# OSU-NLP-Group/saev

Measured on AMD Instinct MI355X. Metric: activations/sec (train step), d_in=1024 x32 k=32, higher is better.
Workload: dtype f32 (encoder: fp16 MFMA first pass with a rigorous error margin, survivors recomputed exactly in fp32; all else fp32)

## Files before the change

include/saev_amd.h:

```cpp
#ifndef SAEV_AMD_H
#define SAEV_AMD_H

#include <stdint.h>

#ifdef __cplusplus
extern "C" {
#endif

#define SAEV_AMD_ABI_VERSION 12

typedef enum {
    SAEV_OK = 0,
    SAEV_INVALID_ARG = -1,
    SAEV_HIP_ERROR = -2,
    SAEV_UNSUPPORTED = -3,
    SAEV_NOT_BOUND = -4,
    SAEV_RCCL_ERROR = -5,
    SAEV_STALE_PARAMS = -6,
    SAEV_ROW_OVERFLOW = -7
} saev_status;

typedef struct {
    int32_t d_model;
    int32_t d_sae;
// ... 377 lines not shown
#define SAEV_L1_STATE_BETA 3
#define SAEV_L1_STATE_F 4
#define SAEV_L1_STATE_FY 5
#define SAEV_L1_STATE_KKT 6
#define SAEV_L1_STATE_OBJ 7
#define SAEV_L1_STATE_DONE 8
#define SAEV_L1_STATE_NEED_GRAD 9
#define SAEV_L1_STATE_CUR 10
#define SAEV_L1_STATE_PREV 11
#define SAEV_L1_STATE_NEXT 12
#define SAEV_L1_STATE_REJECTS 13
#define SAEV_L1_STATE_RESTARTS 14
typedef struct {
    int32_t struct_size;
    int32_t coef_rows;
    int64_t chunk_rows, n_chunks;
    int64_t col_blocks;
    int64_t total_bytes;
    int64_t off_err, off_state, off_w, off_z, off_g, off_part, off_r, off_loss, off_bp;
} saev_l1_logistic_layout;
int64_t saev_pool_images_range(void);
int saev_pool_images(const int64_t* indptr, const int32_t* indices, const float* data, int64_t nnz, int64_t n_images,
                     int64_t tokens_per_image, int64_t n_latents, int32_t agg, float* out, int32_t* err, void* stream);
int64_t saev_l1_logistic_workspace_bytes(int64_t n, int64_t S, int64_t K);
int saev_l1_logistic_layout_of(int64_t n, int64_t S, int64_t K, saev_l1_logistic_layout* out);
int saev_l1_logistic_init(const float* X, const int32_t* y, int64_t n, int64_t S, int64_t K, double C, double kkt_tol, void* workspace,
                          int64_t workspace_bytes, void* stream);
int saev_l1_logistic_iterate(const float* X, const int32_t* y, int64_t n, int64_t S, int64_t K, double C, double kkt_tol, int32_t n_iters,
                             void* workspace, int64_t workspace_bytes, void* stream);
int saev_l1_logistic_result(const float* X, const int32_t* y, int64_t n, int64_t S, int64_t K, double C, double kkt_tol, double* coef,
                            double* intercept, double* scalars, void* workspace, int64_t workspace_bytes, void* stream);
#define SAEV_COACT_JACCARD 0
#define SAEV_COACT_CONTAINMENT 1
#define SAEV_COACT_ERR_COLUMN 1
#define SAEV_COACT_ERR_VALUE 2
#define SAEV_COACT_ERR_INDPTR 3
int64_t saev_coactivation_chunk_rows(void);
int64_t saev_coactivation_window(void);
int64_t saev_coactivation_slots(void);
int64_t saev_coactivation_workspace_bytes(int64_t N, int64_t Sa, int64_t Sb, int64_t nnz_a, int64_t nnz_b);
int saev_coactivation(const int64_t* a_indptr, const int32_t* a_indices, const float* a_data, int64_t nnz_a, int64_t Sa,
                      const int64_t* b_indptr, const int32_t* b_indices, const float* b_data, int64_t nnz_b, int64_t Sb, int64_t N,
                      float thr_a, float thr_b, int32_t measure, int32_t top_m, int32_t* n_a, int32_t* n_b, int32_t* out_index,
                      int32_t* out_inter, int32_t* err, void* workspace, int64_t workspace_bytes, void* stream);
int saev_params_touched(saev_ctx* ctx);

const int32_t* saev_last_idx(saev_ctx* ctx);
const float* saev_last_val(saev_ctx* ctx);
const float* saev_last_x_hat(saev_ctx* ctx);

int saev_copy_last(saev_ctx* ctx, int32_t n_rows, int32_t* idx_out, float* val_out, float* x_hat_out, void* stream);

int saev_bound_state(saev_ctx* ctx, float* z, int64_t* launches, int64_t* repeats, float* mean_candidates, void* stream);

int saev_enable_kernel_timing(saev_ctx* ctx, int32_t enable);
float saev_last_encoder_ms(saev_ctx* ctx);

#ifdef __cplusplus
}
#endif
#endif
```

saev_amd/_lib.py:

```python

from __future__ import annotations

import ctypes as C
import os
import pathlib

_HERE = pathlib.Path(__file__).resolve().parent
LIB_PATH = pathlib.Path(os.environ.get("SAEV_AMD_LIB", _HERE / "libsaev_amd.so"))

ABI_VERSION = 12


class SaevCfg(C.Structure):
    _fields_ = [
        ("d_model", C.c_int32), ("d_sae", C.c_int32), ("top_k", C.c_int32), ("k_aux", C.c_int32),
        ("alpha", C.c_float), ("dead_threshold_tokens", C.c_int64),
        ("normalize_w_dec", C.c_int32), ("remove_parallel_grads", C.c_int32),
        ("max_batch", C.c_int32), ("encoder_mode", C.c_int32), ("aux_dead_cap", C.c_int32),
        ("shard_world", C.c_int32), ("bound_mode", C.c_int32), ("max_backward_rows", C.c_int32),
        ("activation", C.c_int32),
    ]


class SaevDebugCfg(C.Structure):
# ... 183 lines not shown
    "saev_kmeans_collapsed": (C.c_int, [P, C.c_int64, C.c_int64, C.c_float, P, C.c_int32, P, C.c_int64, P, P, P]),
    "saev_batch_stats_workspace_bytes": (C.c_int64, [C.c_int64, C.c_int64]),
    "saev_batch_stats": (C.c_int, [P, P, P, P, P, P, C.c_int64, C.c_int64, C.c_int64, C.c_int64, C.POINTER(SaevBatchAcc), P, C.c_int64, P]),
    "saev_row_norm_mean": (C.c_int, [P, C.c_int64, C.c_int64, P, P, C.c_int64, P]),
    "saev_latent_topk_workspace_bytes": (C.c_int64, [C.c_int64, C.c_int64]),
    "saev_latent_topk_update": (C.c_int, [P, P, P, C.c_int64, P, P, P, C.c_int64, P, C.c_int64, C.c_int64, C.c_int64,
                                          C.POINTER(SaevLatentTopKState), P, C.c_int64, P]),
    "saev_latent_hist_workspace_bytes": (C.c_int64, [C.c_int64, C.c_int64]),
    "saev_latent_hist_update": (C.c_int, [P, P, P, C.c_int64, P, P, P, C.c_int64, P, C.c_int64, C.c_int64, C.POINTER(SaevLatentHistState), P,
                                          C.c_int64, P]),
    "saev_latent_hist_locate": (C.c_int, [C.POINTER(SaevLatentHistState), C.POINTER(SaevLatentHistTargets), C.c_int64, P]),
    "saev_probe1d_workspace_bytes": (C.c_int64, [C.c_int64] * 4),
    "saev_probe1d_layout_of": (C.c_int, [C.c_int64] * 4 + [C.POINTER(SaevProbe1DLayout)]),
    "saev_probe1d_prepare": (C.c_int, [P, P, P, C.c_int64, C.c_int64, C.c_int64, C.c_int64, P, P, P, P, C.c_int64, P]),
    "saev_probe1d_stats": (C.c_int, [C.c_int64] * 4 + [P, P, P, P, C.c_int64, P]),
    "saev_probe1d_init": (C.c_int, [C.c_int64] * 4 + [C.POINTER(SaevProbe1DCfg), P, C.c_int64, P]),
    "saev_probe1d_update": (C.c_int, [C.c_int64] * 4 + [C.POINTER(SaevProbe1DCfg), P, P, P, P, C.c_int64, P]),
    "saev_probe1d_fit": (C.c_int, [C.c_int64] * 4 + [C.POINTER(SaevProbe1DCfg), P, P, P, P, C.c_int64, P]),
    "saev_probe1d_evaluate": (C.c_int, [C.c_int64] * 4 + [P, P, C.c_double, C.c_int32, P, P, P, P, P, P, C.c_int64, P]),
    "saev_latent_ap_workspace_bytes": (C.c_int64, [C.c_int64] * 4),
    "saev_latent_ap_layout_of": (C.c_int, [C.c_int64] * 4 + [C.POINTER(SaevLatentAPLayout)]),
    "saev_latent_ap": (C.c_int, [P, P, P, C.c_int64, C.c_int64, C.c_int64, C.c_int64, P, P, P, P, P, P, P, P, C.c_int64, P]),
    "saev_probe_ap": (C.c_int, [P, P, P, C.c_int64, C.c_int64, C.c_int64, C.c_int64, P, P, P, P, P, C.c_int32, P, P, P, P, C.c_int32, P, P, C.c_int64, P]),
    "saev_latent_auroc_workspace_bytes": (C.c_int64, [C.c_int64] * 5),
    "saev_latent_auroc": (C.c_int, [P, P, P, C.c_int64, C.c_int64, C.c_int64, C.c_int64, P, P, P, P, C.c_int64, P, P, P, P, P, P, P, P, P, P, C.c_int64, P]),
    "saev_pool_images_range": (C.c_int64, []),
    "saev_pool_images": (C.c_int, [P, P, P, C.c_int64, C.c_int64, C.c_int64, C.c_int64, C.c_int32, P, P, P]),
    "saev_l1_logistic_workspace_bytes": (C.c_int64, [C.c_int64] * 3),
    "saev_l1_logistic_layout_of": (C.c_int, [C.c_int64] * 3 + [C.POINTER(SaevL1LogisticLayout)]),
    "saev_l1_logistic_init": (C.c_int, [P, P, C.c_int64, C.c_int64, C.c_int64, C.c_double, C.c_double, P, C.c_int64, P]),
    "saev_l1_logistic_iterate": (C.c_int, [P, P, C.c_int64, C.c_int64, C.c_int64, C.c_double, C.c_double, C.c_int32, P, C.c_int64, P]),
    "saev_l1_logistic_result": (C.c_int, [P, P, C.c_int64, C.c_int64, C.c_int64, C.c_double, C.c_double, P, P, P, P, C.c_int64, P]),
    "saev_coactivation_chunk_rows": (C.c_int64, []),
    "saev_coactivation_window": (C.c_int64, []),
    "saev_coactivation_slots": (C.c_int64, []),
    "saev_coactivation_workspace_bytes": (C.c_int64, [C.c_int64] * 5),
    "saev_coactivation": (C.c_int, [P, P, P, C.c_int64, C.c_int64, P, P, P, C.c_int64, C.c_int64, C.c_int64, C.c_float, C.c_float, C.c_int32,
                                    C.c_int32, P, P, P, P, P, P, C.c_int64, P]),
    "saev_edit_plan_bytes": (C.c_int64, [C.c_int64, C.c_int64]),
    "saev_edit_plan_build": (C.c_int, [C.POINTER(SaevEdit), C.c_int64, C.c_int64, C.c_int64, P, C.c_int64, P]),
    "saev_intervene_rows": (C.c_int, [P, C.c_int64, C.c_int64, P, C.c_int64, P, P, P, C.c_int64, P, C.c_int64, C.c_int64, P, P, P, P, P]),
    "saev_class_fire_counts": (C.c_int, [P, P, P, C.c_int64, C.c_int64, P, P, C.c_int64, C.c_int64, C.POINTER(C.c_float), C.c_int32, P, P, P, P]),
    "saev_class_fire_f1": (C.c_int, [P, P, P, C.c_int64, C.c_int64, C.c_int32, P, P, P, P]),
    "saev_comm_unique_id": (C.c_int, [P]),
    "saev_comm_init": (C.c_int, [P, P, C.c_int32, C.c_int32]),
    "saev_comm_world": (C.c_int, [P]),
    "saev_comm_destroy": (C.c_int, [P]),
    "saev_train_step_dp": (C.c_int, [P, P, C.c_int32, C.c_float, C.c_float, C.c_int64, P]),
    "saev_last_idx": (P, [P]),
    "saev_last_val": (P, [P]),
    "saev_last_x_hat": (P, [P]),
    "saev_copy_last": (C.c_int, [P, C.c_int32, P, P, P, P]),
    "saev_bound_state": (C.c_int, [P, C.POINTER(C.c_float), C.POINTER(C.c_int64), C.POINTER(C.c_int64), C.POINTER(C.c_float), P]),
    "saev_enable_kernel_timing": (C.c_int, [P, C.c_int32]),
    "saev_last_encoder_ms": (C.c_float, [P]),
}

EXPORTED_SYMBOLS = tuple(_SIGNATURES)

_lib = None


def load() -> C.CDLL:
    global _lib
    if _lib is None:
        if not LIB_PATH.exists():
            raise SaevError(
                f"{LIB_PATH} not found: build the HIP extension first (`make` in the repo root or "
                "`python -c 'import __graft_entry__ as g; g.build()'`). There is no CPU fallback."
            )
        import torch

        lib = C.CDLL(str(LIB_PATH))
        for name, (res, args) in _SIGNATURES.items():
            fn = getattr(lib, name)
            fn.restype = res
            fn.argtypes = args
        got = lib.saev_abi_version()
        if got != ABI_VERSION:
            raise SaevError(f"libsaev_amd.so ABI version {got} != expected {ABI_VERSION}")
        _lib = lib
    return _lib


def check(lib: C.CDLL, ctx, rc: int, what: str) -> None:
    if rc != 0:
        msg = lib.saev_last_error(ctx)
        raise SaevError(f"{what} failed (status {rc}): {msg.decode() if msg else '?'}")
```

saev_amd/csrc/ctx.h:

```cpp
#pragma once
#include <hip/hip_runtime.h>

#include <algorithm>
#include <cmath>
#include <cstdio>
#include <cstdlib>
#include <cstring>
#include <string>
#include <vector>

#include "kernels.h"

constexpr int AUX_KSPLIT_MAX = 16;
constexpr int CAND_CAP = 4096;
constexpr int CAND_STRIDE = CAND_CAP + 256;
constexpr int TIMING_RING = 512;
constexpr int DEAD_LAG = 4;
constexpr int DEAD_RING = 16;
enum { AUX_NONE = 0, AUX_SMALL_DEVICE = 1, AUX_SMALL_HOST = 2, AUX_DENSE = 3 };

struct saev_ctx {
    saev_cfg cfg{};
    saev_debug_cfg dbg{};
    int device = 0;
// ... 64 lines not shown
    bool fused_forward = false;
    bool g_rows_valid = true;
    bool fwd_slices = false;
    bool fwd_step = false;
    float* rs_part = nullptr;
    float* xS_c = nullptr;
    int2 *pv = nullptr, *pv2 = nullptr;
    int32_t *plat = nullptr, *cut_lat = nullptr, *cut_list = nullptr;
    int32_t* lat_unused = nullptr;
    bool fused_step = false;
    bool unused_valid = false;
    int P = 1;
    int32_t cuts[MAX_PREFIXES] = {0};
    float* G = nullptr;
    float* GS = nullptr;
    int P_cap = 0;
    int n_dead_host = 0, k_use_host = 0;
    int64_t tokens_seen = 0;
    bool tracker_dirty = false;
    int nd_cap = 0;
    DeadRecord* rec_host = nullptr;
    DeadRecord* rec_dev = nullptr;
    hipEvent_t dead_ev[DEAD_RING];
    bool dead_ev_created = false;
    int64_t dead_steps = 0;
    int64_t rec_valid_from = 1;
    int aux_route = AUX_NONE;
    int64_t n_readbacks = 0;
    std::vector<void*> aux_allocs;
    int32_t* dead_list = nullptr;
    float *Wenc_dead = nullptr, *Wdec_dead = nullptr, *H_dead = nullptr, *A_dead = nullptr, *dWd = nullptr, *dWe = nullptr,
          *dbe = nullptr, *aux_partials = nullptr, *WencT_dead = nullptr, *aux_small_part = nullptr, *aux_small_part2 = nullptr, *aux_small_partbe = nullptr;
    bool aux_dev_count = false;
    bool aux_small = false;
    int aux_mfma_bound = 0;
    int aux_ndp = AUX_SMALL_MAX;
    int aux_mfma_cap = AUX_SMALL_MAX;
    bool aux_mfma = false;
    bool aux_fused = false;
    bool aux_all = false;
    uint8_t* A_mask = nullptr;
    _Float16 *aux_ws1 = nullptr, *aux_ws2 = nullptr, *aux_xsA = nullptr, *aux_xsg = nullptr, *aux_kA = nullptr, *aux_kD = nullptr, *aux_kX = nullptr;
    bool aux_both = false;
    float* aux_parts = nullptr;
    int aux_kpad = 0;
    float *bias_dead = nullptr, *zero_bias = nullptr, *aux_scales = nullptr;
    float* aux_sync = nullptr;
    int aux_Dp2 = 0;
    float *row_margin = nullptr, *wnorm_scratch = nullptr, *surv_val = nullptr;
    int32_t *surv_idx = nullptr, *surv_cnt = nullptr, *surv_rng = nullptr;
    int rs_lat_range = 0, rs_n_ranges = 0;
    int32_t* tau_max = nullptr;
    float* heur_state = nullptr;
    float *f16r_scales = nullptr, *mu = nullptr, *xnorm = nullptr, *b_shift = nullptr, *dot_part = nullptr, *xabs_part = nullptr,
          *sq_part = nullptr, *wmax_prev = nullptr;
    bool wmax_known = false;
    bool mu_ready = false;
    bool stream_ok = false;
    float *WeS = nullptr;
    float *xn_part = nullptr, *amax_part = nullptr, *cmax_part = nullptr;
    float* b_seen = nullptr;
    int32_t *stale_host = nullptr, *stale_dev = nullptr;
    uint32_t* wchk = nullptr;
    float *mu_keep = nullptr, *xside_keep = nullptr;
    bool fwd_streamed = false;
    bool fwd_moves_mu = false;
    int64_t fwd_mu_serial = -1;
    bool borrow_streamed = false;
    bool follow_stream = false;
    bool wchk_valid = false;
    bool fwd_reused_wimg = false;
    uint32_t stale_salt = 0;
    int scale_par = 0;
    bool prep_valid = false;
    bool wimg_fresh = false;
    int64_t mu_serial = 0, wimg_mu_serial = -1;
    bool wimg_bf16_fresh = false;
    bool stream_step = false;
    bool stats_pending = false, stats_lists = false;
    bool aux_stats_pending = false;
    bool dead_list_ready = false;
    bool train_fused = false;
    const float* gather_pool = nullptr;
    const int64_t* gather_rows = nullptr;
    float *upper_c = nullptr, *mu_c = nullptr, *xnorm_c = nullptr, *xabs_c = nullptr;
    _Float16* xs_c = nullptr;
    saev_ctx* leader = nullptr;
    void* comm = nullptr;
    int comm_rank = 0, comm_world = 0;
    std::vector<saev_ctx*> followers;
    const float* xprep_x = nullptr;
    int xprep_n = 0;
    int64_t xprep_serial = 0;
    int64_t leader_serial_seen = 0;
    _Float16 *xs = nullptr, *ws = nullptr;
    int Dp = 0, S_pad = 0, MB_pad = 0;
    int max_work = 0, max_part = 0;
    float* upper = nullptr;
    saev_step_stats* stats = nullptr;
    double* stats_scratch = nullptr;
    int* tickets = nullptr;
    const float *ov_x = nullptr, *ov_g = nullptr, *ov_val = nullptr;
    const int32_t* ov_idx = nullptr;
    int ov_n = 0;
    float* db_aux = nullptr;
    bool trust_grads = false;
// ... 115 lines not shown
```

saev_amd/csrc/ctx.hip:

```cpp
#include "ctx.h"

int muon_cfg_check(const saev_muon_cfg& m, std::string* why) {
    if (m.ns_steps < 0 || m.ns_steps >= 100) { *why = "ns_steps must be in [0, 100)"; return SAEV_INVALID_ARG; }
    if (m.adjust_lr < 0 || m.adjust_lr > 2) { *why = "adjust_lr must be 0 (original), 1 (match_rms_adamw) or 2 (none)"; return SAEV_INVALID_ARG; }
    if (!(m.momentum >= 0.f) || !(m.weight_decay >= 0.f)) { *why = "momentum and weight_decay must be >= 0"; return SAEV_INVALID_ARG; }
    return SAEV_OK;
}

extern "C" {

int saev_abi_version(void) { return SAEV_AMD_ABI_VERSION; }

int saev_layout(const saev_cfg* cfg, saev_layout_t* out) {
    if (!cfg || !out || cfg->d_model <= 0 || cfg->d_sae <= 0) return SAEV_INVALID_ARG;
    const int64_t S = cfg->d_sae, D = cfg->d_model, N = std::max(1, cfg->shard_world);
    out->chunk_a = (S + 1 + N - 1) / N * D;
    out->chunk_b = ((D * S + S + N - 1) / N + 3) / 4 * 4;
    out->off_W_dec = 0;
    out->off_b_dec = S * D;
    out->off_W_enc = N * out->chunk_a;
    out->off_b_enc = out->off_W_enc + D * S;
    out->n_total = N * out->chunk_a + N * out->chunk_b;
    return SAEV_OK;
}
// ... 92 lines not shown
    A(cand_cnt, MB); A(gmax, (size_t)64 * c->gmax_stride); A(cand_idx, MB * CAND_STRIDE); A(cand_val, MB * CAND_STRIDE);
    A(h_dense, MB * S);
    A(idx, MB * K); A(val, MB * K);
    if (KA > 0) { A(aux_idx, MB * KA); A(aux_val, MB * KA); A(g_aux, MB * D); A(dead_list, S); }
    A(x_hat, MB * D); A(g, MB * D);
    A(rowstats, MB);
    c->bitmap_words = (int)(((MBB + 31) / 32 + 7) / 8 * 8);
    A(bitmap, S * c->bitmap_words);
    A(grp_prefix, S * (c->bitmap_words / 8));
    A(scan_totals, ((S + 1023) / 1024) * 4);
    A(counts, S); A(starts, S + 1); A(pairs, MBB * K); A(dval_pairs, MBB * (size_t)cfg->top_k);
    {
        const long max_pairs = MBB * K;
        c->max_work = (int)(S + (max_pairs + DW_CHUNK - 1) / DW_CHUNK);
        c->max_part = (int)(2 * ((max_pairs + DW_CHUNK - 1) / DW_CHUNK) + 2);
    }
    A(chunk_starts, S + 1); A(part_starts, S); A(work_latent, c->max_work);
    A(dW_encT, S * D); A(partials, (size_t)c->max_part * 2 * D); A(db_partials, c->max_part); A(row_proj, S); A(enc_sq, S);
    {
        const bool rows_only = c->dbg.dw_route == 1;
        c->dws_ok = !rows_only && !btk && D % DWS_SLICE == 0 && (uint64_t)S * D * 4ull < (1ull << 32) && MBB < (1l << 24) &&
                    (uint64_t)MBB * K < (1ull << 31);
    }
    c->fwd_slices = !btk && c->cfg.encoder_mode == SAEV_ENCODER_F16R && c->dbg.fwd_route == 0 && D % RS_SLICE == 0 &&
                    (uint64_t)S * 128ull < (1ull << 32) - 256ull && fused_supported(c->cfg);
    if (c->fwd_slices) {
        A(rs_part, (size_t)(D / RS_SLICE) * MB * REFINE_CAP); A(surv_rng, MB * RS_MAX_RANGES);
        c->rs_lat_range = (int)std::max<long>(RS_LAT_RANGE, ((S + RS_MAX_RANGES - 1) / RS_MAX_RANGES + 255) / 256 * 256);
        c->rs_n_ranges = (int)((S + c->rs_lat_range - 1) / c->rs_lat_range);
    }
    if (c->fwd_slices && !c->dws_ok) A(xS, MBB * D);
    if (c->dws_ok) {
        A(gS, MBB * D); A(xS, MBB * D); A(dvp, (size_t)(D / DWS_SLICE) * MBB * K);
        if (c->dbg.dw_route != 2 && decode_forms_dval((int)D, (int)K)) A(dval_rows, MB * K);
        A(pv, MBB * K); A(pv2, MBB * K); A(plat, MBB * K); A(cut_lat, (MBB * K + DWS_RUN - 1) / DWS_RUN); A(cut_list, 4 * (1 + (MBB * K + DWS_RUN - 1) / DWS_RUN)); A(lat_unused, S);
        if (c->dval_rows != nullptr && c->dbg.fin_route == 0) { A(wn2, S); A(sq_wave, (size_t)2 * dw_slices_waves((int)D, (int)(MBB * K))); }
    }
    A(colsum_partials, ((MBB + 63) / 64) * D);
    A(sumsq_partials, 2 * 1024 + (S + 3) / 4 + 8 + transpose_blocks((int)S, (int)D)); A(sumsq_total, 1);
    if (c->cfg.encoder_mode != SAEV_ENCODER_F32 || KA > 0 || c->relu_train) {
        c->Dp = (int)((D + 31) / 32 * 32);
        c->S_pad = (int)((S + 255) / 256 * 256);
        c->MB_pad = (int)((MB + 255) / 256 * 256);
        A(zero_bias, std::max(S, D)); A(aux_scales, 16); A(aux_sync, absmax_parts_max((int)MB));
    }
    if (c->cfg.encoder_mode != SAEV_ENCODER_F32) {
        A(xs, (size_t)c->MB_pad * 2 * c->Dp);
        A(ws, (size_t)c->S_pad * 2 * c->Dp);
        A(row_margin, MB); A(wnorm_scratch, std::max((S + 3) / 4, 3 * ((S + 255) / 256))); A(f16r_scales, 16); A(mu, D); A(xnorm, 2 * MB); A(b_shift, S);
        A(xabs_part, (MB + 3) / 4);
        if (c->cfg.encoder_mode == SAEV_ENCODER_F16R) { A(dot_part, (size_t)2 * (c->Dp / 32) * c->S_pad); A(sq_part, (size_t)2 * (c->Dp / 32) * c->S_pad); A(wmax_prev, 1); }
        if (c->cfg.encoder_mode == SAEV_ENCODER_F16R) { A(surv_idx, MB * REFINE_CAP); A(surv_val, MB * REFINE_CAP); A(surv_cnt, MB); }
    }
    c->stream_ok = c->fwd_slices && c->cfg.bound_mode == 0 && c->dbg.prep_route == 0 && D % 32 == 0 && c->Dp == (int)D;
    if (c->stream_ok) {
        A(WeS, S * D); A(xn_part, (size_t)(D / 32) * c->MB_pad * 2);
        A(amax_part, (size_t)(c->MB_pad / 256) * (D / 32)); A(cmax_part, (size_t)(c->MB_pad / 256) * (D / 32)); A(b_seen, S);
        A(mu_keep, D); A(xside_keep, 4);
    }
    if (c->stream_ok || c->cfg.encoder_mode == SAEV_ENCODER_BF16) A(wchk, (size_t)2 * ((S + 255) / 256) * ((D + 31) / 32));
    A(toks, S); A(fired, S); A(dead, S); A(flags, 16); A(upper, 1); A(stats, 1);
    A(tau_max, MB); A(heur_state, 8); A(stats_scratch, STATS_SCRATCH_DOUBLES); A(tickets, 8); A(db_aux, D);
    if (btk) { A(btk_ws, btk_workspace_words((int)MB)); A(row_nnz, MB); A(btk_over, 1); A(threshold_own, 1); }
#undef A
    if (rc == SAEV_OK && c->relu_train) rc = relu_train_alloc(c);
    if (rc != SAEV_OK) {
        for (void* p : c->allocs) hipFree(p);
        delete c;
        return rc;
    }
    hipMemset(c->toks, 0, S * sizeof(int64_t));
    hipMemset(c->fired, 0, S * sizeof(int32_t));
    hipMemset(c->dead, 0, S * sizeof(int32_t));
    hipMemset(c->flags, 0, 16 * sizeof(int32_t));
    if (btk) {
        hipMemset(c->threshold_own, 0, sizeof(float));
        hipMemset(c->btk_ws, 0, BTK_ST_WORDS * sizeof(uint32_t));
        hipMemset(c->btk_over, 0, sizeof(int32_t));
        c->threshold = c->threshold_own;
    }
    if (c->stream_ok || c->cfg.encoder_mode == SAEV_ENCODER_BF16) {
        void* hp = nullptr;
        if (hipHostMalloc(&hp, 64, hipHostMallocMapped) == hipSuccess &&
            hipHostGetDevicePointer(reinterpret_cast<void**>(&c->stale_dev), hp, 0) == hipSuccess) {
            c->stale_host = static_cast<int32_t*>(hp);
            c->stale_host[0] = 0; c->stale_host[1] = 0;
        } else {
            if (hp) hipHostFree(hp);
            c->stale_host = nullptr; c->stale_dev = nullptr;
        }
    }
    hipMemset(c->scan_totals, 0, ((S + 1023) / 1024) * 4 * sizeof(int32_t));
    hipMemset(c->stats, 0, sizeof(saev_step_stats));
    hipMemset(c->stats_scratch, 0, STATS_SCRATCH_DOUBLES * sizeof(double));
    hipMemset(c->tickets, 0, 8 * sizeof(int));
    {
        const float init[8] = {2.6f, 0.f, 0.f, 0.f, 0.f, 0.f, 0.f, 0.f};
        hipMemcpy(c->heur_state, init, sizeof(init), hipMemcpyHostToDevice);
    }
    hipMemset(c->rowstats, 0, MB * sizeof(RowStats));
    if (c->xs) hipMemset(c->xs, 0, (size_t)c->MB_pad * 2 * c->Dp * sizeof(_Float16));
    if (c->zero_bias) hipMemset(c->zero_bias, 0, std::max(S, D) * sizeof(float));
    if (c->f16r_scales) hipMemset(c->f16r_scales, 0, 16 * sizeof(float));
    if (KA > 0) {
        const int s4 = (int)((S + 3) / 4 * 4);
        const int want = cfg->aux_dead_cap > 0 ? cfg->aux_dead_cap : std::max(4096, 8 * (int)KA);
        const int cap = std::min((want + 3) / 4 * 4, s4);
        rc = alloc_aux_buffers(c, cap);
        if (rc == SAEV_OK) {
            void* h = nullptr;
            if (hipHostMalloc(&h, DEAD_RING * sizeof(DeadRecord), hipHostMallocMapped) != hipSuccess ||
                hipHostGetDevicePointer(reinterpret_cast<void**>(&c->rec_dev), h, 0) != hipSuccess) {
                rc = SAEV_HIP_ERROR;
            } else {
                c->rec_host = static_cast<DeadRecord*>(h);
                std::memset(h, 0, DEAD_RING * sizeof(DeadRecord));
                for (int i = 0; i < DEAD_RING && rc == SAEV_OK; ++i)
                    if (hipEventCreateWithFlags(&c->dead_ev[i], hipEventDisableTiming) != hipSuccess) rc = SAEV_HIP_ERROR;
                c->dead_ev_created = rc == SAEV_OK;
            }
        }
        if (rc != SAEV_OK) {
            for (void* q : c->allocs) hipFree(q);
            for (void* q : c->aux_allocs) hipFree(q);
            if (c->rec_host) hipHostFree(c->rec_host);
            delete c;
            return rc;
        }
    }
    hipDeviceSynchronize();
    *out = c;
    return SAEV_OK;
}

extern "C" {

static void detach_follower(saev_ctx* c) {
    c->leader = nullptr;
    centre_owner_changed(c);
    c->borrow_streamed = false;
    c->follow_stream = false;
}

static void unlink_from_leader(saev_ctx* c) {
    if (c->leader != nullptr) {
        auto& f = c->leader->followers;
        f.erase(std::remove(f.begin(), f.end(), c), f.end());
        detach_follower(c);
    }
}

// ... 133 lines not shown

int saev_copy_last_row_nnz(saev_ctx* c, int32_t n_rows, int32_t* row_nnz_out, void* stream) {
    if (!c) return SAEV_INVALID_ARG;
    REQUIRE(c, c->btk, SAEV_UNSUPPORTED, "saev_copy_last_row_nnz: the context is not a BatchTopK context");
    REQUIRE(c, c->n_last > 0 && n_rows == c->n_last && row_nnz_out, SAEV_INVALID_ARG,
            "saev_copy_last_row_nnz: n_rows differs from the batch of the last forward (or none has run)");
    HIPCHK(c, hipMemcpyAsync(row_nnz_out, c->row_nnz, (size_t)n_rows * sizeof(int32_t), hipMemcpyDeviceToDevice, (hipStream_t)stream));
    return SAEV_OK;
}

int saev_bind_threshold(saev_ctx* c, float* threshold) {
    if (!c) return SAEV_INVALID_ARG;
    REQUIRE(c, c->btk, SAEV_UNSUPPORTED, "saev_bind_threshold: the context is not a BatchTopK context");
    c->threshold = threshold != nullptr ? threshold : c->threshold_own;
    return SAEV_OK;
}
float* saev_threshold_device(saev_ctx* c) { return c ? c->threshold : nullptr; }
int32_t saev_row_cap(const saev_ctx* c) { return c && c->btk ? c->cfg.top_k : 0; }
int32_t saev_row_overflow_need(const saev_ctx* c) { return c ? c->btk_need : 0; }

int saev_batch_topk_state(saev_ctx* c, float* cut, int64_t* n_above, int64_t* tie_quota, int64_t* n_ties, void* stream) {
    if (!c) return SAEV_INVALID_ARG;
    REQUIRE(c, c->btk, SAEV_UNSUPPORTED, "saev_batch_topk_state: the context is not a BatchTopK context");
    uint32_t h[BTK_ST_WORDS];
    hipStream_t s = (hipStream_t)stream;
    HIPCHK(c, hipMemcpyAsync(h, c->btk_ws, sizeof(h), hipMemcpyDeviceToHost, s));
    HIPCHK(c, hipStreamSynchronize(s));
    if (cut) std::memcpy(cut, &h[BTK_ST_CUT], sizeof(float));
    if (n_above) *n_above = h[BTK_ST_ABOVE];
    if (tie_quota) *tie_quota = h[BTK_ST_RANK];
    if (n_ties) *n_ties = h[BTK_ST_TIES];
    return SAEV_OK;
}

int64_t* saev_toks_since_active(saev_ctx* c) { return c ? c->toks : nullptr; }
int32_t* saev_fired_flags(saev_ctx* c) { return c ? c->fired : nullptr; }
const saev_step_stats* saev_stats_device(saev_ctx* c) { return c ? c->stats : nullptr; }
const int32_t* saev_last_idx(saev_ctx* c) { return c ? c->idx : nullptr; }
const float* saev_last_val(saev_ctx* c) { return c ? c->val : nullptr; }
const float* saev_last_x_hat(saev_ctx* c) { return c ? c->x_hat : nullptr; }

int saev_read_stats(saev_ctx* c, saev_step_stats* out_host, void* stream) {
    if (!c || !out_host) return SAEV_INVALID_ARG;
    hipStream_t s = (hipStream_t)stream;
    HIPCHK(c, hipMemcpyAsync(out_host, c->stats, sizeof(saev_step_stats), hipMemcpyDeviceToHost, s));
    HIPCHK(c, hipStreamSynchronize(s));
    return SAEV_OK;
}

int saev_bound_state(saev_ctx* c, float* z, int64_t* launches, int64_t* repeats, float* mean_candidates, void* stream) {
    if (!c) return SAEV_INVALID_ARG;
    float h[4] = {0.f, 0.f, 0.f, 0.f};
    hipStream_t s = (hipStream_t)stream;
    HIPCHK(c, hipMemcpyAsync(h, c->heur_state, sizeof(h), hipMemcpyDeviceToHost, s));
    HIPCHK(c, hipStreamSynchronize(s));
    if (z) *z = h[0];
    if (repeats) *repeats = (int64_t)h[1];
    if (launches) *launches = (int64_t)h[2];
    if (mean_candidates) *mean_candidates = h[3];
    return SAEV_OK;
}

int saev_enable_kernel_timing(saev_ctx* c, int32_t enable) {
    if (!c) return SAEV_INVALID_ARG;
    if (enable && !c->ev_created) {
        for (int i = 0; i < TIMING_RING; ++i) {
            HIPCHK(c, hipEventCreate(&c->ev_start[i]));
            HIPCHK(c, hipEventCreate(&c->ev_stop[i]));
        }
        c->ev_created = true;
    }
    c->timing = enable != 0;
    c->ev_count = 0;
    return SAEV_OK;
}

float saev_last_encoder_ms(saev_ctx* c) {
    if (!c || !c->ev_created || c->ev_count == 0) return -1.f;
    const long n = std::min<long>(c->ev_count, TIMING_RING);
    double tot = 0;
    for (long i = 0; i < n; ++i) {
        float ms = 0.f;
        if (hipEventElapsedTime(&ms, c->ev_start[i], c->ev_stop[i]) != hipSuccess) return -1.f;
        tot += ms;
    }
    return (float)(tot / n);
}

int saev_params_touched(saev_ctx* c) {
    if (!c) return SAEV_INVALID_ARG;
    params_moved(c);
    return SAEV_OK;
}

void saev_muon_default_cfg(saev_muon_cfg* out) {
    if (!out) return;
    *out = saev_muon_cfg{0.95f, 0.1f, 3.4445f, -4.7750f, 2.0315f, 1e-7f, 1, 5, 0};
}

int64_t saev_muon_workspace_bytes(int64_t rows, int64_t cols) {
    if (rows <= 0 || cols <= 0 || rows > cols || cols > (int64_t)1 << 30) return -1;
    return (int64_t)muon_layout((int)rows, (int)cols).bytes;
}

int saev_muon_newton_schulz(const void* x_in, int64_t rows, int64_t cols, void* x_out, const saev_muon_cfg* cfg, int32_t normalize,
                            void* workspace, int64_t workspace_bytes, void* stream) {
    if (!x_in || !x_out || !workspace) return SAEV_INVALID_ARG;
    const int64_t need = saev_muon_workspace_bytes(rows, cols);
    if (need < 0 || workspace_bytes < need || ((uintptr_t)workspace & 255) != 0) return SAEV_INVALID_ARG;
    saev_muon_cfg m;
    saev_muon_default_cfg(&m);
    if (cfg) m = *cfg;
// ... 59 lines not shown
```

saev_amd/csrc/ctx_auxk.hip:

```cpp
#include "ctx.h"

int alloc_aux_buffers(saev_ctx* c, int cap) {
    const size_t MB = c->cfg.max_batch, D = c->cfg.d_model;
    const size_t capA = std::max(cap, AUX_SMALL_MAX);
    auto grab = [&](size_t bytes) -> void* {
        void* q = nullptr;
        if (hipMalloc(&q, bytes) != hipSuccess) return nullptr;
        c->aux_allocs.push_back(q);
        c->aux_bytes += bytes;
        return q;
    };
    c->Wenc_dead = (float*)grab(D * capA * 4);
    c->Wdec_dead = (float*)grab(capA * D * 4);
    c->H_dead = (float*)grab(MB * capA * 4);
    c->A_dead = (float*)grab(MB * capA * 4);
    c->A_mask = (uint8_t*)grab(MB * capA);
    c->dWd = (float*)grab(capA * D * 4);
    c->dWe = (float*)grab(capA * D * 4);
    c->dbe = (float*)grab(capA * 4);
    c->aux_partials = (float*)grab(((MB + 63) / 64) * capA * 4);
    const size_t mcap = (aux_mfma_supported((int)D) && capA >= (size_t)AUX_MFMA_MAX && c->cfg.max_backward_rows == 0 && c->dbg.aux_wide_route == 0)
                            ? (size_t)AUX_MFMA_MAX : (size_t)AUX_SMALL_MAX;
    c->aux_mfma_cap = (int)mcap;
    c->WencT_dead = (float*)grab(mcap * D * 4);
// ... 208 lines not shown
            HIPCHK(c, launch_colsum(c->g_aux, n, D, c->colsum_partials, c->grads + c->off_b_dec, 1, nd_dev, s));
        }
        return SAEV_OK;
    }
    {
        if (c->aux_both) {
            int ns, Kp;
            ksplit_shape(ndp, D, n, &ns, &Kp);
            HIPCHK(c, launch_split_both(c->g_aux, n, D, 1.0f, c->aux_scales + 4, c->aux_xsg, c->Dp, c->aux_kD, Kp, s));
        } else {
        HIPCHK(c, launch_split_rows(c->g_aux, n, D, c->Dp, c->aux_xsg, 0, s, 1.0f, c->aux_scales + 4));
        HIPCHK(c, launch_split_rows(c->Wdec_dead, ndp, D, c->Dp, c->aux_ws1, 0, s, 256.0f));
        }
        rc = dense_f16x3(c, c->aux_xsg, c->aux_ws1, c->zero_bias, n, c->Dp, ndp, 256.0f, dA, s, c->aux_scales + 4);
    }
    if (rc != SAEV_OK) return rc;
    if (!c->aux_all) HIPCHK(c, launch_mask_apply_absmax(dA, c->A_mask, (long)n * ndp, c->aux_sync, c->aux_scales + 10, s));
    else HIPCHK(c, launch_absmax_pow2(dA, (long)n * ndp, c->aux_sync, c->aux_scales + 10, s));
    {
        rc = ksplit_f16x3(c, c->A_dead, c->aux_scales + 2, ndp, c->g_aux, c->aux_scales + 4, D, n, c->dWd, s,
                          c->aux_both ? c->aux_kA : nullptr, c->aux_both ? c->aux_kD : nullptr);
        if (rc != SAEV_OK) return rc;
        if (c->cfg.encoder_mode == SAEV_ENCODER_F16X3) HIPCHK(c, launch_pow2_scale(c->upper_c, c->aux_scales + 6, s));
        rc = ksplit_f16x3(c, dA, c->aux_scales + 10, ndp, c->x_last, c->aux_scales + 6, D, n, c->dWe, s, nullptr,
                          c->aux_both ? c->aux_kX : nullptr);
        if (rc != SAEV_OK) return rc;
    }
    HIPCHK(c, launch_colsum(dA, n, ndp, c->aux_partials, c->dbe, 0, nullptr, s));
    HIPCHK(c, launch_colsum(c->g_aux, n, D, c->colsum_partials, c->ov_x != nullptr ? c->db_aux : c->grads + c->off_b_dec,
                            c->ov_x != nullptr ? 0 : 1, nullptr, s));
    return SAEV_OK;
}

extern "C" {

int saev_step_dead(saev_ctx* c, int64_t n_rows_global, void* stream) {
    if (!c) return SAEV_INVALID_ARG;
    REQUIRE(c, c->x_last && c->training_last, SAEV_INVALID_ARG, "saev_step_dead: no training forward in flight");
    hipStream_t s = (hipStream_t)stream;
    const int S = c->cfg.d_sae;
    const int64_t step = ++c->dead_steps;
    c->tokens_seen += n_rows_global;
    DeadArgs d{};
    d.toks = c->toks; d.fired = c->fired; d.dead = c->dead; d.S = S;
    d.add_tokens = n_rows_global; d.threshold = c->cfg.dead_threshold_tokens; d.k_aux = c->cfg.k_aux;
    d.n_dead = c->flags + 4; d.k_use = c->flags + 5; d.stats = c->stats; d.scratch = c->flags + 6;
    d.horizon_tokens = (int64_t)DEAD_LAG * n_rows_global;
    d.step = step; d.cum_tokens = c->tokens_seen;
    d.rec = c->rec_dev ? c->rec_dev + step % DEAD_RING : nullptr;
    c->dead_list_ready = false;
    if (c->stats_pending) {
        c->stats_pending = false;
        d.dead_list = c->cfg.k_aux > 0 ? c->dead_list : nullptr;
        HIPCHK(c, launch_stats_dead(c->rowstats, c->n_last, c->cfg.d_model, c->P_last, c->cfg.alpha, c->upper_c, c->flags + 2, c->stats,
                                    c->stats_scratch, c->stats_lists ? c->cand_cnt : nullptr, CAND_CAP, d, s));
        c->dead_list_ready = d.dead_list != nullptr;
    } else {
        HIPCHK(c, launch_dead_update(d, s));
    }
    c->n_dead_host = 0;
    c->k_use_host = 0;
    c->aux_route = AUX_NONE;
    c->aux_small = false;
    c->aux_dev_count = false;
    if (c->cfg.k_aux <= 0) return SAEV_OK;
    HIPCHK(c, hipEventRecord(c->dead_ev[step % DEAD_RING], s));
    if (!c->tracker_dirty && c->tokens_seen < c->cfg.dead_threshold_tokens) return SAEV_OK;
    const bool mfma_route = aux_mfma_supported(c->cfg.d_model) && c->dbg.aux_small_route == 0;
    const int small_default = mfma_route ? std::max((int)AUX_SMALL_MAX, c->aux_mfma_cap) : (int)AUX_SMALL_DEFAULT;
    const int small_cap = c->dbg.aux_small_max < 0 ? 0 : (c->dbg.aux_small_max == 0 ? small_default : std::min(c->dbg.aux_small_max, (int)AUX_SMALL_MAX));
    const int small_max = std::min(small_cap, c->cfg.k_aux);
    const int64_t s0 = step - DEAD_LAG;
    if (s0 >= c->rec_valid_from) {
        HIPCHK(c, hipEventSynchronize(c->dead_ev[s0 % DEAD_RING]));
        const volatile DeadRecord* r = c->rec_host + s0 % DEAD_RING;
        if (r->step == s0 && c->tokens_seen - r->cum_tokens <= r->horizon_tokens) {
            const int bound = r->n_near;
            if (bound == 0) return SAEV_OK;
            if (bound <= small_max && c->cfg.d_model <= 2048) {
                c->aux_route = AUX_SMALL_DEVICE;
                return auxk_small_forward(c, s, bound);
            }
            if ((bound + 3) / 4 * 4 <= c->nd_cap) {
                c->aux_route = AUX_DENSE;
                c->aux_dev_count = true;
                c->n_dead_host = bound;
                c->k_use_host = std::min(c->cfg.k_aux, bound);
                return auxk_forward(c, s);
            }
        }
    }
    int32_t host[2] = {0, 0};
    HIPCHK(c, hipMemcpyAsync(host, c->flags + 4, 2 * sizeof(int32_t), hipMemcpyDeviceToHost, s));
    HIPCHK(c, hipStreamSynchronize(s));
    c->n_readbacks++;
    c->n_dead_host = host[0];
    c->k_use_host = host[1];
    if (c->n_dead_host <= 0) return SAEV_OK;
    if ((c->n_dead_host + 3) / 4 * 4 > c->nd_cap && !(c->n_dead_host <= small_max && c->cfg.d_model <= 2048)) {
        const int s4 = (S + 3) / 4 * 4;
        const int cap = std::min(s4, std::max(2 * c->nd_cap, (2 * c->n_dead_host + 1023) / 1024 * 1024));
        for (void* q : c->aux_allocs) hipFree(q);
        c->aux_allocs.clear();
        c->aux_bytes = 0;
        c->nd_cap = 0;
        int rcg = alloc_aux_buffers(c, cap);
        if (rcg != SAEV_OK) {
            c->err = "AuxK: " + std::to_string(c->n_dead_host) + " dead latents exceed saev_cfg.aux_dead_cap and the buffers could not be grown to " +
// ... 16 lines not shown
```

saev_amd/csrc/ctx_forward.hip:

```cpp
#include "ctx.h"

extern "C" {


int saev_normalize_w_dec(saev_ctx* c, void* stream) {
    if (!c) return SAEV_INVALID_ARG;
    REQUIRE(c, c->params, SAEV_NOT_BOUND, "parameters not bound");
    if (!c->cfg.normalize_w_dec) return SAEV_OK;
    HIPCHK(c, launch_normalize_rows(c->params + c->off_W_dec, c->cfg.d_sae, c->cfg.d_model, (hipStream_t)stream));
    return SAEV_OK;
}

static bool bind_x_sources(saev_ctx* c, const float* x, int n, bool allow_borrow) {
    saev_ctx* l = c->leader;
    const bool borrow = allow_borrow && l != nullptr && l->xprep_x == x && l->xprep_n == n && l->xprep_serial != c->leader_serial_seen;
    saev_ctx* src = borrow ? l : c;
    c->upper_c = src->upper; c->mu_c = src->mu; c->xnorm_c = src->xnorm; c->xabs_c = src->xabs_part; c->xs_c = src->xs;
    c->borrow_streamed = borrow && l->fwd_streamed && l->mu_keep != nullptr;
    if (c->borrow_streamed) c->mu_c = l->mu_keep;
    c->fwd_step = c->fwd_slices && (src == c || src->fwd_slices);
    c->xS_c = c->fwd_step ? src->xS : nullptr;
    if (borrow) c->leader_serial_seen = l->xprep_serial;
    return borrow;
}
// ... 16 lines not shown
        if (!c->wmax_known) {
            { int rcw = wait_wenc(c, s); if (rcw != SAEV_OK) return rcw; }
            HIPCHK(c, launch_transpose(c->params + c->off_W_enc, c->dW_encT, D, S, s));
            HIPCHK(c, launch_wnorm_max(c->dW_encT, S, D, c->wnorm_scratch, c->wmax_prev, s));
            c->wmax_known = true;
        }
        if (!x_borrowed) {
            if (!c->mu_ready) { HIPCHK(c, launch_colsum(x, n, D, c->colsum_partials, c->mu, 0, nullptr, s, 0, 1.0f / (float)n)); c->mu_serial++; }
            HIPCHK(c, launch_center_stats(x, c->mu, n, D, c->xnorm, c->xabs_part, s, xmax_dev));
        }
        c->mu_ready = false;
        if (c->borrow_streamed)
            HIPCHK(c, launch_follower_scales(c->leader->xside_keep, c->wmax_prev, scl(c), pre_flag != nullptr ? pre_flag : c->flags, 0, s));
        else
        HIPCHK(c, launch_f16r_scales(c->xabs_c, (n + 3) / 4, c->wmax_prev, scl(c), s));
        float* const wt_out = (c->fwd_step && c->stream_ok) ? c->WeS : c->dW_encT;
        if (!x_borrowed && c->wenc_ready == nullptr) {
            HIPCHK(c, launch_split_f16r(x, n, D, c->Dp, c->xs, scl(c), c->mu, c->params + c->off_W_enc, S, c->S_pad, c->ws,
                                        reinterpret_cast<double*>(c->dot_part), c->sq_part, wt_out, s, c->fwd_step ? c->xS : nullptr,
                                        c->fwd_step ? 1 : 0));
        } else {
            if (!x_borrowed) HIPCHK(c, launch_split_rows(x, n, D, c->Dp, c->xs, 2, s, 1.0f, scl(c), c->mu, c->fwd_step ? c->xS : nullptr));
            { int rcw = wait_wenc(c, s); if (rcw != SAEV_OK) return rcw; }
            HIPCHK(c, launch_split_wT(c->params + c->off_W_enc, D, S, c->S_pad, c->Dp, 1.0f, c->ws, 2, s, scl(c) + 1,
                                      c->mu_c, reinterpret_cast<double*>(c->dot_part), c->sq_part, wt_out, c->fwd_step ? 1 : 0));
        }
        c->wimg_fresh = c->stream_ok && c->fwd_step && !x_borrowed && c->leader == nullptr;
        c->wimg_mu_serial = c->mu_serial;
        HIPCHK(c, launch_bias_finish(reinterpret_cast<const double*>(c->dot_part), c->sq_part, c->Dp, S, c->S_pad,
                                     scl(c) + 1, c->params + c->off_b_enc, c->b_shift, c->wnorm_scratch, s, c->b_seen));
        if (!defer_margins)
            HIPCHK(c, launch_row_margins(c->xnorm_c, n, D, c->wnorm_scratch, (S + 255) / 256, scl(c), pre_flag,
                                         c->wmax_prev, c->row_margin, s));
        return SAEV_OK;
    }
    if (!x_borrowed) HIPCHK(c, launch_split_rows(x, n, D, c->Dp, c->xs, bf ? 1 : 0, s));
    { int rcw = wait_wenc(c, s); if (rcw != SAEV_OK) return rcw; }
    c->fwd_reused_wimg = bf && c->wimg_bf16_fresh;
    if (!(bf && c->wimg_bf16_fresh))
        HIPCHK(c, launch_split_wT(c->params + c->off_W_enc, D, S, c->S_pad, c->Dp, bf ? 1.0f : 256.0f, c->ws, bf ? 1 : 0, s));
    if (bf && c->dbg.prep_route == 0 && c->Dp == D && D % 32 == 0) c->wimg_bf16_fresh = true;
    return SAEV_OK;
}

static int prepare_dense_scaled(saev_ctx* c, const float* x, int n, const float* absmax_dev, float* pair, hipStream_t s) {
    HIPCHK(c, launch_pow2_scale(absmax_dev, pair, s));
    HIPCHK(c, launch_split_rows(x, n, c->cfg.d_model, c->Dp, c->xs, 0, s, 1.0f, pair));
    { int rcw = wait_wenc(c, s); if (rcw != SAEV_OK) return rcw; }
    HIPCHK(c, launch_split_wT(c->params + c->off_W_enc, c->cfg.d_model, c->cfg.d_sae, c->S_pad, c->Dp, 256.0f, c->ws, 0, s));
    return SAEV_OK;
}

static int run_encoder(saev_ctx* c, const float* x, int n, int epi, float* h_out, const int32_t* flag, int when,
                       hipStream_t s, bool predicted = false, const float* x_scale = nullptr) {
    const bool f16r = c->cfg.encoder_mode == SAEV_ENCODER_F16R;
    if (c->cfg.encoder_mode != SAEV_ENCODER_F32 && !(f16r && epi == EPI_DENSE)) {
        const bool bf = c->cfg.encoder_mode == SAEV_ENCODER_BF16;
        EncodeF16Args a{};
        a.xs = c->xs_c; a.ws = c->ws;
        a.b_enc = f16r ? c->b_shift : c->params + c->off_b_enc;
        a.n_rows = n; a.Dp = c->Dp; a.S = c->cfg.d_sae; a.w_scale = (bf || f16r) ? 1.0f : 256.0f;
        a.scale_dev = f16r ? scl(c) : x_scale;
        a.arith = bf ? 1 : (f16r ? 2 : 0);
        a.row_margin = f16r ? c->row_margin : nullptr;
        a.s_splits = encoder_splits(n, a.S, encode_f16x3_tile_rows(), encode_f16x3_tile_latents(), 256);
        a.h_out = h_out;
        a.ngroups = f16_ngroups(c); a.top_k = c->cfg.top_k;
        a.gmax = c->gmax; a.gmax_stride = c->gmax_stride; a.cand_cnt = c->cand_cnt; a.cand_val = c->cand_val; a.cand_idx = c->cand_idx;
        a.cand_cap = CAND_CAP; a.cand_stride = CAND_STRIDE;
        a.enable_flag = flag; a.enable_when = when;
        if (predicted) { a.heur_z = c->heur_state; a.tau_max = c->tau_max; }
        a.refresh_first = 8;
        a.refresh_every = a.ngroups > 32 ? 1 : 2;
        HIPCHK(c, launch_encode_f16x3(a, epi, s));
        return SAEV_OK;
    }
    EncodeArgs a{};
    a.x = x;
    a.W_enc = c->params + c->off_W_enc;
    a.b_enc = c->params + c->off_b_enc;
    a.n_rows = n;
    a.D = c->cfg.d_model;
    a.S = c->cfg.d_sae;
    a.s_splits = encoder_splits(n, a.S, encode_gemm_tile_rows(), encode_gemm_tile_latents(), 512);
    a.h_out = h_out;
    a.ngroups = c->cfg.top_k <= 32 ? 32 : 64;
    a.gmax = c->gmax;
    a.gmax_stride = c->gmax_stride;
    a.cand_cnt = c->cand_cnt;
    a.cand_val = c->cand_val;
    a.cand_idx = c->cand_idx;
    a.cand_cap = CAND_CAP; a.cand_stride = CAND_STRIDE;
    a.enable_flag = flag;
    a.enable_when = when;
    HIPCHK(c, launch_encode_gemm(a, epi, s));
    return SAEV_OK;
}

int saev_encode_dense(saev_ctx* c, const float* x, int32_t n, float* h_out, void* stream) {
    if (!c) return SAEV_INVALID_ARG;
    REQUIRE(c, c->params, SAEV_NOT_BOUND, "parameters not bound");
    REQUIRE(c, x && h_out && n > 0, SAEV_INVALID_ARG, "saev_encode_dense: bad arguments");
    REQUIRE(c, n <= c->cfg.max_batch || c->cfg.encoder_mode == SAEV_ENCODER_F32, SAEV_INVALID_ARG,
            "saev_encode_dense: n_rows > max_batch");
    bind_x_sources(c, x, n, false);
    c->xprep_x = nullptr;
    if (c->relu_train && c->cfg.encoder_mode == SAEV_ENCODER_F16X3) {
        hipStream_t s = (hipStream_t)stream;
        HIPCHK(c, hipMemsetAsync(c->rt_scales + 8, 0, sizeof(float), s));
        HIPCHK(c, launch_absmax(x, (long)n * c->cfg.d_model, c->rt_scales + 8, s));
        int rc = prepare_dense_scaled(c, x, n, c->rt_scales + 8, c->rt_scales + 10, s);
        if (rc != SAEV_OK) return rc;
        return run_encoder(c, x, n, EPI_DENSE, h_out, nullptr, 0, s, false, c->rt_scales + 10);
    }
    if (c->cfg.encoder_mode != SAEV_ENCODER_F16R) {
        int rc = prepare_encoder(c, x, n, nullptr, (hipStream_t)stream);
        if (rc != SAEV_OK) return rc;
    }
    return run_encoder(c, x, n, EPI_DENSE, h_out, nullptr, 0, (hipStream_t)stream);
}

int saev_topk_dense(saev_ctx* c, const float* h, int32_t n, int32_t k, const int32_t* mask, int32_t* idx_out,
                    float* val_out, void* stream) {
    if (!c) return SAEV_INVALID_ARG;
    REQUIRE(c, h && idx_out && val_out && n > 0 && k > 0, SAEV_INVALID_ARG, "saev_topk_dense: bad arguments");
    REQUIRE(c, k <= c->cfg.d_sae, SAEV_INVALID_ARG, "saev_topk_dense: k > d_sae");
    SelectDenseArgs a{};
    a.h = h; a.n_rows = n; a.S = c->cfg.d_sae; a.k = k; a.mask = mask;
    a.idx_out = idx_out; a.val_out = val_out; a.out_stride = k;
    HIPCHK(c, launch_select_dense(a, (hipStream_t)stream));
    return SAEV_OK;
}

static int encode_topk_impl(saev_ctx* c, const float* x, int n, int32_t* idx_out, float* val_out,
                            const int32_t* pre_flag, hipStream_t s, const float* xmax_dev = nullptr, bool x_borrowed = false) {
    const int K = c->cfg.top_k;
    int32_t* need_dense = c->flags + 1;
    const bool f16r_mode = c->cfg.encoder_mode == SAEV_ENCODER_F16R;
    const bool predict_mode = fused_supported(c->cfg) && c->cfg.bound_mode != 0 && c->cfg.encoder_mode != SAEV_ENCODER_F32 &&
                              f16_ngroups(c) == 32;
    const bool one_launch_pre = fused_supported(c->cfg) && !predict_mode;
    if (c->follow_stream) {
        HIPCHK(c, launch_follower_scales(c->leader->xside_keep, c->wmax_prev, scl(c), const_cast<int32_t*>(pre_flag), 1, s));
    } else if (!c->stream_step) {
        int rc0 = prepare_encoder(c, x, n, const_cast<int32_t*>(pre_flag), s, xmax_dev, x_borrowed, one_launch_pre);
        if (rc0 != SAEV_OK) return rc0;
        rc0 = wait_wenc(c, s);
        if (rc0 != SAEV_OK) return rc0;
    }
    if (fused_supported(c->cfg)) {
        const int ng = c->cfg.encoder_mode == SAEV_ENCODER_F32 ? (c->cfg.top_k <= 32 ? 32 : 64) : f16_ngroups(c);
        const bool f16r = c->cfg.encoder_mode == SAEV_ENCODER_F16R;
        auto select_stage = [&](const int32_t* flag, int when, int32_t* bad, const int32_t* tau_max, int32_t* ovf = nullptr,
                                const int32_t* first_flag = nullptr) -> int {
            SelectCandArgs sc{};
            sc.cand_cnt = c->cand_cnt; sc.cand_val = c->cand_val; sc.cand_idx = c->cand_idx;
            sc.cand_cap = CAND_CAP; sc.cand_stride = CAND_STRIDE; sc.n_rows = n; sc.k = K;
            sc.idx_out = idx_out; sc.val_out = val_out; sc.out_stride = K;
            sc.enable_flag = first_flag ? first_flag : flag; sc.enable_when = when;
            sc.tau_max = tau_max; sc.invalid = bad; sc.ovf = ovf;
            if (f16r) {
                sc.row_margin = c->row_margin; sc.x = x; sc.W_encT = c->dW_encT; sc.b_enc = c->params + c->off_b_enc;
                sc.D = c->cfg.d_model; sc.refine_overflow = bad;
                sc.surv_idx = c->surv_idx; sc.surv_val = c->surv_val; sc.surv_cnt = c->surv_cnt;
                if (c->fwd_step) { sc.surv_rng = c->surv_rng; sc.lat_range = c->rs_lat_range; sc.n_ranges = c->rs_n_ranges; }
                HIPCHK(c, launch_select_cand(sc, s));
                sc.enable_flag = flag; sc.ovf = nullptr;
                if (c->fwd_step) {
                    RefineSlicesArgs rs{};
                    rs.surv_idx = c->surv_idx; rs.surv_cnt = c->surv_cnt; rs.surv_val = c->surv_val; rs.surv_rng = c->surv_rng;
                    rs.xS = c->xS_c; rs.WeS = c->stream_ok ? c->WeS : c->dW_encT; rs.b_enc = sc.b_enc; rs.part = c->rs_part;
                    rs.n_rows = n; rs.S = c->cfg.d_sae; rs.D = c->cfg.d_model;
                    rs.lat_range = c->rs_lat_range; rs.n_ranges = c->rs_n_ranges;
                    rs.enable_flag = flag; rs.enable_when = when;
                    HIPCHK(c, launch_refine_slices(rs, s));
                    sc.sum_part = c->rs_part; sc.sum_bias = sc.b_enc; sc.sum_n = c->cfg.d_model / RS_SLICE; sc.sum_plane = (size_t)n * REFINE_CAP;
                } else {
                    HIPCHK(c, launch_refine_exact(sc, s));
                }
                sc.row_margin = nullptr; sc.tau_max = nullptr;
                sc.cand_cnt = c->surv_cnt; sc.cand_val = c->surv_val; sc.cand_idx = c->surv_idx; sc.cand_cap = REFINE_CAP; sc.cand_stride = REFINE_CAP;
            }
            HIPCHK(c, launch_select_cand(sc, s));
            return SAEV_OK;
        };
        const bool predict = c->cfg.bound_mode != 0 && ng == 32 && c->cfg.encoder_mode != SAEV_ENCODER_F32;
        int32_t *bad1 = c->flags + 9, *run2 = c->flags + 10, *gate = c->flags + 11;
        if (predict) {
            HIPCHK(c, launch_heur_gate(c->heur_state, pre_flag, gate, s));
            HIPCHK(c, launch_encoder_init(c->cand_cnt, n, c->gmax, 0, s, c->tau_max));
            timing_begin(c, s);
            int rc = run_encoder(c, x, n, EPI_TOPK, nullptr, gate, 0, s, true);
            if (rc != SAEV_OK) return rc;
            timing_end(c, s);
            HIPCHK(c, launch_overflow_check(c->cand_cnt, n, CAND_CAP, gate, bad1, c->flags + 2, c->flags + 3, s, need_dense,
                                            nullptr, c->heur_state + 3, nullptr, pre_flag));
            rc = select_stage(bad1, 0, bad1, c->tau_max);
            if (rc != SAEV_OK) return rc;
            HIPCHK(c, launch_heur_update(c->heur_state, bad1, c->heur_state + 3, K, gate, s));
            HIPCHK(c, launch_encoder_init(c->cand_cnt, n, c->gmax, ng * c->gmax_stride, s, nullptr, bad1, 1));
            rc = run_encoder(c, x, n, EPI_TOPK, nullptr, bad1, 1, s);
            if (rc != SAEV_OK) return rc;
            HIPCHK(c, launch_overflow_check(c->cand_cnt, n, CAND_CAP, pre_flag, need_dense, c->flags + 2, c->flags + 3, s, need_dense,
                                            run2, nullptr, bad1));
            rc = select_stage(run2, 1, need_dense, nullptr);
            if (rc != SAEV_OK) return rc;
        } else {
            const int S_ = c->cfg.d_sae;
            if (c->stream_step) {
                const int D_ = c->cfg.d_model;
                XprepArgs xp{};
                xp.x = c->gather_pool != nullptr ? c->gather_pool : x; xp.rows = c->gather_rows; xp.x_out = c->gather_pool != nullptr ? const_cast<float*>(x) : nullptr;
                xp.n = n; xp.D = D_; xp.nks = D_ / 32; xp.n_pad = c->MB_pad; xp.scales = scl(c); xp.mu = c->mu; xp.xs = c->xs; xp.xS = c->xS;
                xp.xn_part = c->xn_part; xp.col_part = c->colsum_partials; xp.amax_part = c->amax_part; xp.cmax_part = c->cmax_part;
                xp.W_enc = c->params + c->off_W_enc; xp.WeS = c->WeS; xp.b_enc = c->params + c->off_b_enc; xp.b_seen = c->b_seen;
                xp.S = S_; xp.salt = ++c->stale_salt; xp.stale = c->flags + 12;
                if (!c->followers.empty()) { xp.mu_keep = c->mu_keep; xp.xside_keep = c->xside_keep; }
                HIPCHK(c, launch_xprep(xp, s));
                PreEncode2Args pe{};
                pe.cand_cnt = c->cand_cnt; pe.n_rows = n; pe.gmax = c->gmax; pe.n_gmax = ng * c->gmax_stride;
                pe.xn_part = c->xn_part; pe.nks = D_ / 32; pe.n_pad = c->MB_pad; pe.D = D_;
                pe.wg_part = c->wnorm_scratch; pe.n_part = (S_ + 255) / 256; pe.scales = scl(c); pe.scales_next = scl_next(c);
                pe.pre_flag = const_cast<int32_t*>(pre_flag); pe.wmax_prev = c->wmax_prev; pe.margin = c->row_margin; pe.xnorm = c->xnorm;
                pe.flags1 = c->flags + 1; pe.col_part = c->colsum_partials; pe.n_rowblk = (n + 255) / 256; pe.mu = c->mu;
                pe.inv_n = 1.0f / (float)n; pe.update_mu = c->train_fused ? 1 : 0;
                pe.amax_part = c->amax_part; pe.cmax_part = c->cmax_part; pe.n_img = ((n + 255) / 256) * (D_ / 32);
                pe.upper = c->upper; pe.stats = c->stats; pe.stale = c->flags + 12; pe.stale_host = c->stale_dev;
                pe.xside_keep = c->followers.empty() ? nullptr : c->xside_keep;
                HIPCHK(c, launch_pre_encode2(pe, s));
                if (c->train_fused) c->mu_serial++;
            } else
            HIPCHK(c, launch_pre_encode(c->cand_cnt, n, c->gmax, ng * c->gmax_stride, f16r_mode ? c->xnorm_c : nullptr, c->cfg.d_model,
                                        c->wnorm_scratch, (S_ + 255) / 256, f16r_mode ? scl(c) : nullptr, const_cast<int32_t*>(pre_flag),
                                        c->wmax_prev, c->row_margin, c->flags + 1, s));
            timing_begin(c, s);
            int rc = run_encoder(c, x, n, EPI_TOPK, nullptr, pre_flag, 0, s);
            if (rc != SAEV_OK) return rc;
            timing_end(c, s);
            rc = select_stage(need_dense, 0, need_dense, nullptr, c->flags + 1, pre_flag);
            if (rc != SAEV_OK) return rc;
        }
    } else {
        HIPCHK(c, launch_init_i32(need_dense, 1, 1, s));
        HIPCHK(c, hipMemsetAsync(c->flags + 2, 0, 2 * sizeof(int32_t), s));
        timing_begin(c, s);
        timing_end(c, s);
    }
    int rc = run_encoder(c, x, n, EPI_DENSE, c->h_dense, need_dense, 1, s);
    if (rc != SAEV_OK) return rc;
    SelectDenseArgs sd{};
    sd.h = c->h_dense; sd.n_rows = n; sd.S = c->cfg.d_sae; sd.k = K;
    sd.idx_out = idx_out; sd.val_out = val_out; sd.out_stride = K;
    sd.enable_flag = need_dense; sd.enable_when = 1;
    if (fused_supported(c->cfg)) sd.walk_grid = 4 * 256;
    HIPCHK(c, launch_select_dense(sd, s));
    return SAEV_OK;
}

int saev_encode_topk(saev_ctx* c, const float* x, int32_t n, int32_t* idx_out, float* val_out, void* stream) {
    if (!c) return SAEV_INVALID_ARG;
    REQUIRE(c, c->cfg.activation == SAEV_ACT_TOPK, SAEV_UNSUPPORTED,
            "saev_encode_topk: a TopK context only (ReLU: saev_encode_relu, BatchTopK: saev_encode_batch_topk)");
    REQUIRE(c, c->params, SAEV_NOT_BOUND, "parameters not bound");
    REQUIRE(c, x && idx_out && val_out && n > 0 && n <= c->cfg.max_batch, SAEV_INVALID_ARG,
            "saev_encode_topk: bad arguments (n_rows must be in 1..max_batch)");
    hipStream_t s = (hipStream_t)stream;
    HIPCHK(c, hipMemsetAsync(c->flags, 0, sizeof(int32_t), s));
    bind_x_sources(c, x, n, false);
    c->xprep_x = nullptr;
    c->stream_step = false;
    c->follow_stream = false;
    return encode_topk_impl(c, x, n, idx_out, val_out, c->flags, s);
}

int saev_scatter_dense(saev_ctx* c, const int32_t* idx, const float* val, int32_t n, int32_t k, float* f_out,
                       void* stream) {
    if (!c) return SAEV_INVALID_ARG;
    REQUIRE(c, idx && val && f_out && n > 0 && k > 0, SAEV_INVALID_ARG, "saev_scatter_dense: bad arguments");
    HIPCHK(c, launch_scatter_dense(idx, val, n, k, k, c->cfg.d_sae, f_out, (hipStream_t)stream));
    return SAEV_OK;
}

int saev_decode_sparse(saev_ctx* c, const int32_t* idx, const float* val, int32_t n, int32_t k,
                       const int64_t* prefixes_host, int32_t n_prefixes, float* x_hats_out, void* stream) {
    if (!c) return SAEV_INVALID_ARG;
    REQUIRE(c, c->params, SAEV_NOT_BOUND, "parameters not bound");
    REQUIRE(c, idx && val && x_hats_out && n > 0 && k > 0, SAEV_INVALID_ARG, "saev_decode_sparse: bad arguments");
    const int S = c->cfg.d_sae, D = c->cfg.d_model;
    int64_t single = S;
    if (!prefixes_host) { prefixes_host = &single; n_prefixes = 1; }
    REQUIRE(c, n_prefixes >= 1 && prefixes_host[n_prefixes - 1] == S && prefixes_host[0] >= 1, SAEV_INVALID_ARG,
            "prefixes must end at d_sae and start at >= 1");
    for (int p = 1; p < n_prefixes; ++p)
        REQUIRE(c, prefixes_host[p] > prefixes_host[p - 1], SAEV_INVALID_ARG, "prefixes must be strictly increasing");
    REQUIRE(c, n <= c->cfg.max_batch || n_prefixes == 1, SAEV_INVALID_ARG, "n_rows > max_batch");
    hipStream_t s = (hipStream_t)stream;
    for (int p = 0; p < n_prefixes; ++p) {
        DecodeArgs a{};
        a.x = nullptr;
        a.idx = idx; a.val = val; a.code_stride = k; a.k = k;
        a.W_dec = c->params + c->off_W_dec; a.b_dec = c->params + c->off_b_dec;
        a.n_rows = n; a.D = D; a.S = S; a.idx_limit = (int)prefixes_host[p];
        a.x_hat = (n_prefixes == 1) ? x_hats_out : c->g;
        HIPCHK(c, launch_decode(a, s));
        if (n_prefixes > 1)
            HIPCHK(c, hipMemcpy2DAsync(x_hats_out + (size_t)p * D, (size_t)n_prefixes * D * sizeof(float), c->g,
                                       (size_t)D * sizeof(float), (size_t)D * sizeof(float), n,
                                       hipMemcpyDeviceToDevice, s));
    }
    return SAEV_OK;
}


namespace {
int btk_codes(saev_ctx* c, const float* h, int n, int training, int32_t* row_nnz_out, int32_t* idx_out, float* val_out,
              int32_t* overflow_out, hipStream_t s) {
    BtkArgs a{};
    a.h = h; a.n_rows = n; a.S = c->cfg.d_sae; a.top_k = c->btk_k; a.row_cap = c->cfg.top_k; a.training = training ? 1 : 0;
    a.update_threshold = a.training; a.momentum = c->btk_momentum; a.threshold = c->threshold;
    a.idx_out = idx_out; a.val_out = val_out; a.row_nnz_out = row_nnz_out; a.overflow = overflow_out;
    a.ws = c->btk_ws; a.max_rows = c->cfg.max_batch; a.list_cap = c->btk_list_cap;
    HIPCHK(c, launch_batch_topk(a, s));
    return SAEV_OK;
}
// ... 111 lines not shown
    if (!c) return SAEV_INVALID_ARG;
    REQUIRE(c, pool && rows && out && n > 0, SAEV_INVALID_ARG, "saev_gather_rows: bad arguments");
    HIPCHK(c, launch_gather_rows(pool, rows, n, c->cfg.d_model, out, (hipStream_t)stream));
    return SAEV_OK;
}


int saev_step_forward(saev_ctx* c, const float* x, int32_t n, int64_t n_rows_global, int32_t training,
                      void* stream) {
    if (!c) return SAEV_INVALID_ARG;
    if (c->relu_train) return relu_train_forward(c, x, n, n_rows_global, training, (hipStream_t)stream);
    REQUIRE(c, c->cfg.activation != SAEV_ACT_RELU, SAEV_UNSUPPORTED, "saev_step_forward: a ReLU context runs the forward entries only");
    REQUIRE(c, c->params, SAEV_NOT_BOUND, "parameters not bound");
    REQUIRE(c, x && n > 0 && n <= c->cfg.max_batch, SAEV_INVALID_ARG,
            "saev_step_forward: n_rows must be in 1..max_batch");
    REQUIRE(c, ((uintptr_t)x % 16) == 0, SAEV_INVALID_ARG, "x must be 16-byte aligned");
    REQUIRE(c, n_rows_global >= n, SAEV_INVALID_ARG, "n_rows_global < n_rows");
    hipStream_t s = (hipStream_t)stream;
    const int S = c->cfg.d_sae, D = c->cfg.d_model, K = c->cfg.top_k;
    c->x_last = x;
    c->n_last = n;
    c->training_last = training;
    c->ov_x = nullptr; c->ov_n = 0;
    c->unused_valid = false;
    hipEvent_t wdec_ev = c->wdec_ready;
    c->wdec_ready = nullptr;
    const bool btk = c->btk;
    const bool borrowed = bind_x_sources(c, x, n, !btk);
    if (c->stale_host != nullptr && reinterpret_cast<volatile int32_t*>(c->stale_host)[1] != 0) {
        const int n_tiles = reinterpret_cast<volatile int32_t*>(c->stale_host)[1];
        reinterpret_cast<volatile int32_t*>(c->stale_host)[1] = 0;
        c->wimg_fresh = false; c->wimg_bf16_fresh = false; c->wn2_fresh = false;
        c->err = "W_enc was written outside the library without saev_params_touched (" + std::to_string(n_tiles) +
                 " 32 x 256 tiles changed between two optimizer steps): a recent step encoded with operand images of the OLD values. "
                 "Announce such writes (saev_params_touched / SaeEngine.params_touched) or make them through torch in-place "
                 "operations on the parameter tensors; the context prepares from scratch from here on";
        return SAEV_STALE_PARAMS;
    }
    if (c->stale_host != nullptr && *reinterpret_cast<volatile int32_t*>(c->stale_host) != 0) {
        *reinterpret_cast<volatile int32_t*>(c->stale_host) = 0;
        c->wimg_fresh = false;
        c->wn2_fresh = false;
    }
    c->stream_step = c->stream_ok && c->prep_valid && c->wimg_fresh && c->wimg_mu_serial == c->mu_serial && c->leader == nullptr &&
                     c->wenc_ready == nullptr && c->fwd_step && (c->followers.empty() || c->dbg.group_route == 0);
    if (!borrowed) {
        c->fwd_streamed = c->stream_step;
        c->fwd_moves_mu = c->stream_step && c->train_fused;
        c->fwd_mu_serial = c->mu_serial;
    }
    c->follow_stream = borrowed && c->borrow_streamed && c->stream_ok && c->wimg_fresh && c->wimg_mu_serial == c->leader->fwd_mu_serial &&
                       c->wenc_ready == nullptr && c->fwd_step && c->cfg.encoder_mode == SAEV_ENCODER_F16R;
    c->fwd_reused_wimg = c->stream_step || c->follow_stream;
    if (c->gather_pool != nullptr && !c->stream_step)
        HIPCHK(c, launch_gather_rows(c->gather_pool, c->gather_rows, n, D, const_cast<float*>(x), s));
    if (c->stream_step) {
        c->xprep_x = nullptr;
    } else if (!borrowed && !btk && c->cfg.encoder_mode == SAEV_ENCODER_F16R) {
        c->xprep_x = nullptr;
        HIPCHK(c, launch_colsum_absmax(x, n, D, c->colsum_partials, c->mu, c->xabs_part, c->upper, s, 1.0f / (float)n, c->stats, c->flags));
        c->mu_ready = true;
        c->mu_serial++;
    } else {
        HIPCHK(c, launch_step_zero(c->stats, c->upper, c->flags, s));
        if (!borrowed) {
            c->xprep_x = nullptr;
            HIPCHK(c, launch_absmax(x, (long)n * D, c->upper, s));
        }
    }
    (void)n_rows_global;
    int rc;
    if (btk) {
        rc = encode_dense_h(c, x, n, s);
        if (rc == SAEV_OK) rc = btk_codes(c, c->h_dense, n, training, c->row_nnz, c->idx, c->val, c->btk_over, s);
        if (rc == SAEV_OK) {
            int32_t need = 0;
            HIPCHK(c, hipMemcpyAsync(&need, c->btk_over, sizeof(int32_t), hipMemcpyDeviceToHost, s));
            HIPCHK(c, hipStreamSynchronize(s));
            if (need > 0) {
                c->btk_need = need;
                c->x_last = nullptr; c->n_last = 0; c->training_last = 0;
                c->err = "BatchTopK: a row holds " + std::to_string(need) + " codes, the context's row_cap is " + std::to_string(K) +
                         " (create a context with a larger saev_batch_topk_cfg.row_cap and repeat the forward; the threshold has not moved)";
                return SAEV_ROW_OVERFLOW;
            }
        }
    } else {
        rc = encode_topk_impl(c, x, n, c->idx, c->val, c->flags, s, c->upper_c, borrowed);
    }
    if (rc != SAEV_OK) return rc;
    if (!borrowed) { c->xprep_x = x; c->xprep_n = n; c->xprep_serial++; }
    if (!borrowed && c->stream_ok && !c->stream_step && c->fwd_step) {
        HIPCHK(c, hipMemcpyAsync(scl(c) + 4, c->upper, sizeof(float), hipMemcpyDeviceToDevice, s));
        c->prep_valid = true;
    }
    if (wdec_ev != nullptr) HIPCHK(c, hipStreamWaitEvent(s, wdec_ev, 0));
    if (training) {
        c->wn2_fresh = false;
        if (c->cfg.normalize_w_dec) {
            HIPCHK(c, launch_normalize_rows(c->params + c->off_W_dec, S, D, s, c->wn2));
            c->wn2_fresh = c->wn2 != nullptr;
        }
    }

    DecodeArgs a{};
    a.x = x; a.idx = c->idx; a.val = c->val; a.code_stride = K; a.k = K;
    a.W_dec = c->params + c->off_W_dec; a.b_dec = c->params + c->off_b_dec;
    a.n_rows = n; a.D = D; a.S = S; a.idx_limit = S;
    a.upper = c->upper_c;
    a.gscale = 2.0f / ((float)n * (float)D * (float)c->P);
    a.training = training ? 1 : 0;
    a.g = c->g; a.x_hat = c->x_hat; a.fired = c->fired; a.rowstats = c->rowstats;
    c->dws_rows = 0;
    c->dval_fwd = false;
    if (training && c->dws_ok && (c->P == 1 || c->GS != nullptr)) { a.gS = c->P == 1 ? c->gS : c->GS; a.xS = c->fwd_step ? nullptr : c->xS; c->dws_rows = n; }
    if (c->dws_rows == n && c->dval_rows != nullptr && (c->P == 1 || decode_matry_forms_dval(D, K))) { a.dval_out = c->dval_rows; c->dval_fwd = true; }
    c->g_rows_valid = !(c->train_fused && training && c->P == 1 && c->dws_rows == n);
    if (!c->g_rows_valid) a.g = nullptr;
    c->bitmap_prefill_words = 0;
    if (training && c->dbg.csc_route == 0 && c->bitmap != nullptr && c->bitmap_clean && !c->last_backward_gathered) {
        const int words = ((n + 31) / 32 + 7) / 8 * 8;
        if (words <= c->bitmap_clean_words) {
            a.csc_bitmap = c->bitmap; a.csc_words = words;
            c->bitmap_prefill_words = words; c->bitmap_prefill_rows = n;
            c->bitmap_clean = false;
        }
    }
    if (c->P > 1) {
        MatryArgs m{};
        m.P = c->P;
        for (int p = 0; p < c->P; ++p) m.cuts[p] = c->cuts[p];
        m.G = c->G;
        m.g_rows_all = c->fused_forward ? 0 : 1;
        HIPCHK(c, launch_decode_matry(a, m, s));
    } else {
        HIPCHK(c, launch_decode(a, s));
    }
    c->P_last = c->P;
    for (int p = 0; p < c->P; ++p) c->cuts_last[p] = c->cuts[p];
    const bool lists = !btk && fused_supported(c->cfg) && !(c->cfg.bound_mode != 0 && c->cfg.encoder_mode != SAEV_ENCODER_F32 && f16_ngroups(c) == 32);
    c->stats_pending = false;
    if (c->train_fused && training) {
        c->stats_pending = true;
        c->stats_lists = lists;
        return SAEV_OK;
    }
    HIPCHK(c, launch_stats_reduce(c->rowstats, n, D, c->P, c->cfg.alpha, 0, c->upper_c, c->flags + 2, c->stats, s, nullptr, c->stats_scratch,
                                  lists ? c->cand_cnt : nullptr, CAND_CAP));
    return SAEV_OK;
}

}
```

saev_amd/csrc/gemm_encode_f16x3.hip:

```cpp
#include "common.h"
#include "kernels.h"

namespace {

typedef _Float16 half8 __attribute__((ext_vector_type(8)));

constexpr int HTS = 256;
constexpr int HTB = 256;
constexpr int HTHREADS = 512;
constexpr int NSLOTS = 4;

struct __attribute__((aligned(16))) KSlot {
    _Float16 a[HTS][32];
    _Float16 b[HTB][32];
};
struct __attribute__((aligned(16))) HSmem {
    union {
        KSlot slot[NSLOTS];
        struct {
            KSlot keep[2];
            int32_t slots32[2][32][HTB];
        } e32;
    };
    int32_t tau_key[HTB];
// ... 549 lines not shown
    const int l15 = lane & 15;
    const int kg = lane >> 4;

    const int Dp = a.Dp, S = a.S, B = a.n_rows;
    const int n_stiles = (S + HTS - 1) / HTS;
    int bb, sp;
    {
        const int id = blockIdx.x;
        const int nbb = (B + HTB - 1) / HTB;
        const int full = (nbb / 8) * 8 * a.s_splits;
        if (id < full) {
            const int xcd = id & 7, j = id >> 3;
            sp = j % a.s_splits;
            bb = (j / a.s_splits) * 8 + xcd;
        } else {
            const int r = id - full;
            bb = (nbb / 8) * 8 + r / a.s_splits;
            sp = r % a.s_splits;
        }
    }
    const int st_begin = (int)((long)n_stiles * sp / a.s_splits);
    const int st_end = (int)((long)n_stiles * (sp + 1) / a.s_splits);
    const int b0 = bb * HTB;

    const int nks = Dp / 32;
    const int rot = (bb & 7) % nks;
    auto kmap = [&](int t) { const int k = t + rot; return k >= nks ? k - nks : k; };

    const size_t img = (size_t)256 * 32;
    const int blk_imgs = a.blk_imgs > 0 ? a.blk_imgs : nks;
    const _Float16* x_imgs = a.xs + (size_t)bb * blk_imgs * img;
    const uint32_t lane_off = (uint32_t)lane * 16u;
    const uint32_t lds_w = (uint32_t)(size_t)(__attribute__((address_space(3))) char*)&sm.slot[0].a[wid * 32][0];
    auto stage_kstep = [&](int slot, int s0, int ks) {
        const char* wsrc = reinterpret_cast<const char*>(a.ws + ((size_t)(s0 / HTS) * blk_imgs + ks) * img) + wid * 2048;
        const char* xsrc = reinterpret_cast<const char*>(x_imgs + (size_t)ks * img) + wid * 2048;
        const uint32_t lds_a = lds_w + (uint32_t)slot * (uint32_t)sizeof(KSlot);
        asm volatile(
            "s_mov_b32 m0, %0\n\ts_nop 0\n\t"
            "global_load_lds_dwordx4 %2, %3" SAEV_ENC_W_POLICY "\n\tglobal_load_lds_dwordx4 %2, %3 offset:1024" SAEV_ENC_W_POLICY "\n\t"
            "s_mov_b32 m0, %1\n\ts_nop 0\n\t"
            "global_load_lds_dwordx4 %2, %4" SAEV_ENC_X_POLICY "\n\tglobal_load_lds_dwordx4 %2, %4 offset:1024" SAEV_ENC_X_POLICY
            ::"s"(lds_a), "s"(lds_a + (uint32_t)sizeof(_Float16) * HTS * 32), "v"(lane_off), "s"(wsrc), "s"(xsrc)
            : "memory");
    };

    const int arow0 = ws * 128 + l15;
    const int brow0 = wb * 64 + l15;
    const int coff = 8 * (kg ^ ((4 - (l15 >> 2)) & 3));

    if (st_begin < st_end) {
        stage_kstep(0, st_begin * HTS, kmap(0));
        if (nks > 1) stage_kstep(1, st_begin * HTS, kmap(1));
    }

    for (int st = st_begin; st < st_end; ++st) {
        const int s0 = st * HTS;
        f32x4 acc[8][4];
#pragma unroll
        for (int i = 0; i < 8; ++i)
#pragma unroll
            for (int j = 0; j < 4; ++j) acc[i][j] = f32x4{0.f, 0.f, 0.f, 0.f};

        float* const bias_t = sm.bias[st & 1];
        if (tid < HTS) bias_t[tid] = (s0 + tid < S) ? a.b_enc[s0 + tid] : NEG_INF;
        asm volatile("s_waitcnt vmcnt(0)" ::: "memory");
        __syncthreads();
        if (nks > 2) stage_kstep(2, s0, kmap(2));
        const char* const w_tile = reinterpret_cast<const char*>(a.ws + (size_t)(s0 / HTS) * blk_imgs * img) + wid * 2048;
        const char* const x_blk = reinterpret_cast<const char*>(x_imgs) + wid * 2048;
        const uint32_t run_bytes = (uint32_t)nks * (uint32_t)(img * sizeof(_Float16));
        uint32_t koff = (uint32_t)kmap(nks > 3 ? 3 : 0) * (uint32_t)(img * sizeof(_Float16));
        auto stage_next = [&](int slot) {
            const uint32_t lds_a = lds_w + (uint32_t)slot * (uint32_t)sizeof(KSlot);
            asm volatile(
                "s_mov_b32 m0, %0\n\ts_nop 0\n\t"
                "global_load_lds_dwordx4 %2, %3" SAEV_ENC_W_POLICY "\n\tglobal_load_lds_dwordx4 %2, %3 offset:1024" SAEV_ENC_W_POLICY "\n\t"
                "s_mov_b32 m0, %1\n\ts_nop 0\n\t"
                "global_load_lds_dwordx4 %2, %4" SAEV_ENC_X_POLICY "\n\tglobal_load_lds_dwordx4 %2, %4 offset:1024" SAEV_ENC_X_POLICY
                ::"s"(lds_a), "s"(lds_a + (uint32_t)sizeof(_Float16) * HTS * 32), "v"(lane_off), "s"(w_tile + koff), "s"(x_blk + koff)
                : "memory");
            koff += (uint32_t)(img * sizeof(_Float16));
            koff = koff == run_bytes ? 0u : koff;
        };

        auto kstep = [&](int t, auto WAIT_, auto SLOT_) {
            constexpr int WAIT = decltype(WAIT_)::value;
            constexpr int SLOT = decltype(SLOT_)::value;
            if constexpr (WAIT == 8) stage_next(SLOT >= 0 ? (SLOT + 3) & 3 : (t + 3) & 3);
            const KSlot& cs = sm.slot[SLOT >= 0 ? SLOT : t & 3];
            half8 fa[3], fb[4];
            auto load_a = [&](int set, int sb) { fa[set] = *reinterpret_cast<const half8*>(&cs.a[arow0 + 16 * sb][coff]); };
#pragma unroll
            for (int jb = 0; jb < 4; ++jb) fb[jb] = *reinterpret_cast<const half8*>(&cs.b[brow0 + 16 * jb][coff]);
            load_a(0, 0);
            load_a(1, 1);
            static_for<8>([&](auto G) {
                constexpr int sb = decltype(G)::value;
                constexpr int as = sb % 3;
                constexpr int j0 = (sb & 1) ? 3 : 0, j1 = (sb & 1) ? 2 : 1, j2 = (sb & 1) ? 1 : 2, j3 = (sb & 1) ? 0 : 3;
                acc[sb][j0] = mfma16<AR>(fa[as], fb[j0], acc[sb][j0]);
                __builtin_amdgcn_sched_barrier(0);
                if constexpr (sb + 2 < 8) load_a((sb + 2) % 3, sb + 2);
                __builtin_amdgcn_sched_barrier(0);
                acc[sb][j1] = mfma16<AR>(fa[as], fb[j1], acc[sb][j1]);
                acc[sb][j2] = mfma16<AR>(fa[as], fb[j2], acc[sb][j2]);
// ... 71 lines not shown
                }
                __syncthreads();
                {
                    int32_t old[32];
#pragma unroll
                    for (int i = 0; i < 32; ++i) {
                        old[i] = __hip_atomic_load(GPTR(i), __ATOMIC_RELAXED, __HIP_MEMORY_SCOPE_AGENT);
                    }
                    short2v mp[16];
                    uint32_t improved = 0;
#pragma unroll
                    for (int j = 0; j < 16; ++j) {
                        const int gp = 16 * tpart + j;
                        const short2v w0 = __builtin_bit_cast(short2v, sm.e32.slots32[0][gp][trow]);
                        const short2v w1 = __builtin_bit_cast(short2v, sm.e32.slots32[1][gp][trow]);
                        const short2v wm = __builtin_elementwise_max(w0, w1);
                        const short2v o = __builtin_bit_cast(
                            short2v, __builtin_amdgcn_perm((uint32_t)old[2 * j + 1], (uint32_t)old[2 * j], 0x07060302u));
                        mp[j] = __builtin_elementwise_max(wm, o);
                        improved |= __builtin_bit_cast(uint32_t, mp[j]) ^ __builtin_bit_cast(uint32_t, o);
                    }
                    if (share && improved != 0) {
#pragma unroll
                        for (int j = 0; j < 16; ++j) {
                            const int32_t a0 = (int32_t)mp[j][0], a1 = (int32_t)mp[j][1];
                            if (a0 > (old[2 * j] >> 16)) atomicMax(GPTR(2 * j), a0 << 16);
                            if (a1 > (old[2 * j + 1] >> 16)) atomicMax(GPTR(2 * j + 1), a1 << 16);
                        }
                    }
                    short2v mn = mp[0], mx = mp[0];
#pragma unroll
                    for (int j = 1; j < 16; ++j) { mn = __builtin_elementwise_min(mn, mp[j]); mx = __builtin_elementwise_max(mx, mp[j]); }
                    int32_t lo = min((int32_t)mn[0], (int32_t)mn[1]), hi = max((int32_t)mx[0], (int32_t)mx[1]);
                    lo = min(lo, __shfl_xor(lo, 32, 64));
                    hi = max(hi, __shfl_xor(hi, 32, 64));
                    const int K = a.top_k;
#pragma unroll 1
                    for (int it = 0; it < 4 && lo < hi && K < 64; ++it) {
                        const int32_t mid = lo + ((hi - lo + 1) >> 1);
                        const short2v midp = {(short)mid, (short)mid};
                        uint32_t lt = 0;
#pragma unroll
                        for (int j = 0; j < 16; ++j)
                            lt += (__builtin_bit_cast(uint32_t, __builtin_elementwise_sub_sat(mp[j], midp)) >> 15) & 0x00010001u;
                        int c = 32 - (int)((lt & 0xffffu) + (lt >> 16));
                        c += __shfl_xor(c, 32, 64);
                        if (c >= K) lo = mid; else hi = mid - 1;
                    }
                    if (tpart == 0) sm.tau_key[trow] = (int32_t)((uint32_t)lo << 16);
                }
#undef GPTR
                __syncthreads();
            }
        } else if (refresh) {
#pragma unroll
            for (int jb = 0; jb < 4; ++jb) {
                const int bl_ = wb * 64 + jb * 16 + l15;
#pragma unroll
                for (int p = 0; p < 2; ++p)
#pragma unroll
                    for (int e = 0; e < 4; ++e) {
                        const float m = fmaxf(fmaxf(acc[p][jb][e], acc[p + 2][jb][e]), fmaxf(acc[p + 4][jb][e], acc[p + 6][jb][e]));
                        sm.e32.slots32[ws][p * 16 + 4 * kg + e][bl_] = f2key(m);
                    }
            }
            __syncthreads();
            if (tid < HTB) sm.tau_key[tid] = INT32_MAX;
            __syncthreads();
            {
                const int row = tid % HTB;
                const int part = __builtin_amdgcn_readfirstlane(tid / HTB);
                constexpr int GPT = 16;
                const int b = b0 + row;
                const bool share = b < B;
                const uint32_t boff = (uint32_t)b * 4u;
                int32_t m = INT32_MAX;
                int32_t old[GPT];
#pragma unroll
                for (int i = 0; i < GPT; ++i) {
                    old[i] = INT32_MIN;
                    if (share)
                        old[i] = __hip_atomic_load(
                            reinterpret_cast<int32_t*>(reinterpret_cast<char*>(a.gmax + (size_t)(part * GPT + i) * a.gmax_stride) + boff),
                            __ATOMIC_RELAXED, __HIP_MEMORY_SCOPE_AGENT);
                }
#pragma unroll
                for (int i = 0; i < GPT; ++i) {
                    const int g = part * GPT + i;
                    const int32_t v = max(sm.e32.slots32[0][g][row], sm.e32.slots32[1][g][row]);
                    if (share && v > old[i])
                        atomicMax(reinterpret_cast<int32_t*>(reinterpret_cast<char*>(a.gmax + (size_t)g * a.gmax_stride) + boff), v);
                    m = min(m, max(v, old[i]));
                }
                atomicMin(&sm.tau_key[row], m);
            }
            __syncthreads();
        }
        if (NG == 32 && st == st_begin && a.top_k <= HTS / 4) {
            if (tid < HTB) { sm.ref[0][tid] = INT32_MIN; sm.ref[1][tid] = 0; sm.ref[2][tid] = 0; sm.ref[3][tid] = 0; }
            __syncthreads();
#pragma unroll
            for (int jb = 0; jb < 4; ++jb) {
                float m = NEG_INF;
#pragma unroll
                for (int sb = 0; sb < 8; ++sb)
#pragma unroll
                    for (int e = 0; e < 4; ++e) m = fmaxf(m, acc[sb][jb][e]);
                atomicMax(&sm.ref[0][wb * 64 + jb * 16 + l15], f2key(m));
            }
            __syncthreads();
            float tg[4][3];
#pragma unroll
            for (int jb = 0; jb < 4; ++jb) {
                const int row = wb * 64 + jb * 16 + l15;
                const float t0 = key2f(sm.tau_key[row]), M = key2f(sm.ref[0][row]);
                const bool usable = t0 > -3.0e38f && M > t0;
                const float span = usable ? (M - t0) : 0.f;
                tg[jb][0] = t0 + 0.25f * span; tg[jb][1] = t0 + 0.40f * span; tg[jb][2] = t0 + 0.55f * span;
                int c0 = 0, c1 = 0, c2 = 0;
#pragma unroll
                for (int sb = 0; sb < 8; ++sb)
#pragma unroll
                    for (int e = 0; e < 4; ++e) {
                        const float v = acc[sb][jb][e];
                        c0 += (v >= tg[jb][0]) ? 1 : 0; c1 += (v >= tg[jb][1]) ? 1 : 0; c2 += (v >= tg[jb][2]) ? 1 : 0;
                    }
                if (usable) { atomicAdd(&sm.ref[1][row], c0); atomicAdd(&sm.ref[2][row], c1); atomicAdd(&sm.ref[3][row], c2); }
            }
            __syncthreads();
            if (ws == 0 && kg == 0) {
#pragma unroll
                for (int jb = 0; jb < 4; ++jb) {
                    const int row = wb * 64 + jb * 16 + l15;
                    float best = key2f(sm.tau_key[row]);
                    if (sm.ref[1][row] >= a.top_k) best = fmaxf(best, tg[jb][0]);
                    if (sm.ref[2][row] >= a.top_k) best = fmaxf(best, tg[jb][1]);
                    if (sm.ref[3][row] >= a.top_k) best = fmaxf(best, tg[jb][2]);
                    sm.tau_key[row] = f2key(best);
                }
            }
            __syncthreads();
        }
        typedef unsigned u32x2 __attribute__((ext_vector_type(2)));
        uint32_t hit[4];
        int pos[4], rowtot[4], base[4];
#pragma unroll
        for (int jb = 0; jb < 4; ++jb) {
            const int b = b0 + wb * 64 + jb * 16 + l15;
            float tau = fmaxf(key2f(sm.tau_key[wb * 64 + jb * 16 + l15]), -3.0e38f);
            if (a.row_margin != nullptr) tau -= (b < B) ? a.row_margin[b] : 0.f;
            uint32_t m = 0;
#pragma unroll
            for (int sb = 0; sb < 8; ++sb)
#pragma unroll
                for (int e = 0; e < 4; ++e)
                    asm("v_cmp_ge_f32 vcc, %1, %2\n\tv_addc_co_u32 %0, vcc, %0, %0, vcc" : "+v"(m) : "v"(acc[sb][jb][e]), "v"(tau) : "vcc");
            m = (b < B) ? m : 0u;
            const int n = __builtin_popcount(m);
            const u32x2 r = __builtin_amdgcn_permlane16_swap((unsigned)n, (unsigned)n, false, false);
            const unsigned pair = r[0] + r[1];
            const u32x2 q = __builtin_amdgcn_permlane32_swap(pair, pair, false, false);
            rowtot[jb] = (int)(q[0] + q[1]);
            pos[jb] = (int)(((kg & 1) ? r[0] : 0u) + ((kg & 2) ? q[0] : 0u));
            base[jb] = 0;
            if (kg == 0 && rowtot[jb] > 0) base[jb] = atomicAdd(&a.cand_cnt[b], rowtot[jb]);
            hit[jb] = m;
        }
        asm volatile("s_waitcnt vmcnt(0)" ::: "memory");
        asm volatile("" : "+v"(base[0]), "+v"(base[1]), "+v"(base[2]), "+v"(base[3]));
        float* const park = reinterpret_cast<float*>(&sm.e32.slots32[0][0][0]) + wid * 2048 + lane * 4;
        const int lat0 = s0 + ws * 128 + 4 * kg;
#pragma unroll
        for (int jb = 0; jb < 4; ++jb) {
            const u32x2 h = __builtin_amdgcn_permlane32_swap((unsigned)base[jb], (unsigned)base[jb], false, false);
            const u32x2 f = __builtin_amdgcn_permlane16_swap(h[0], h[0], false, false);
            const int row_base = (int)f[0];
            uint32_t mm = (row_base + rowtot[jb] <= a.cand_cap) ? hit[jb] : 0u;
            if (__ballot(mm != 0u) == 0ull) continue;
            if (mm != 0u) {
#pragma unroll
                for (int sb = 0; sb < 8; ++sb) *reinterpret_cast<f32x4*>(park + 256 * sb) = acc[sb][jb];
            }
            uint32_t off = ((uint32_t)(b0 + wb * 64 + jb * 16 + l15) * (uint32_t)a.cand_stride + (uint32_t)(row_base + pos[jb])) * 4u;
            int i0 = 0;
            while (mm != 0u) {
                const int p = __builtin_clz(mm);
                const int i = i0 + p;
                mm = (mm << p) << 1;
                i0 = i + 1;
                const int c = i >> 2, e = i & 3;
                const float v = park[256 * c + e];
                *reinterpret_cast<float*>(reinterpret_cast<char*>(a.cand_val) + off) = v;
                *reinterpret_cast<int32_t*>(reinterpret_cast<char*>(a.cand_idx) + off) = lat0 + 16 * c + e;
                off += 4u;
            }
        }
        if (!prefetched && st + 1 < st_end) {
            __syncthreads();
            stage_kstep(0, s0 + HTS, kmap(0));
            if (nks > 1) stage_kstep(1, s0 + HTS, kmap(1));
        }
    }
}

}

hipError_t launch_encode_f16x3(const EncodeF16Args& a, int epi, hipStream_t stream) {
    const int n_bblocks = (a.n_rows + HTB - 1) / HTB;
    dim3 grid(n_bblocks * a.s_splits, (epi == EPI_DENSE && a.n_batches > 1) ? a.n_batches : 1), block(HTHREADS);
    const size_t smem = sizeof(HSmem);
    static bool attr_set = false;
    if (!attr_set) {
        const void* fns[12] = {reinterpret_cast<const void*>(&encode_m16_kernel<1>),
                              reinterpret_cast<const void*>(&encode_m16_kernel<2>),
                              reinterpret_cast<const void*>(&encode_m16_kernel<1, 64>),
                              reinterpret_cast<const void*>(&encode_m16_kernel<2, 64>),
                              reinterpret_cast<const void*>(&encode_f16x3_kernel<EPI_TOPK, 32, 0, true>),
                              reinterpret_cast<const void*>(&encode_f16x3_kernel<EPI_TOPK, 32, 1, true>),
                              reinterpret_cast<const void*>(&encode_f16x3_kernel<EPI_TOPK, 32, 2, true>),
                              reinterpret_cast<const void*>(&encode_f16x3_kernel<EPI_DENSE, 32, 0>),
                              reinterpret_cast<const void*>(&encode_f16x3_kernel<EPI_TOPK, 32, 0>),
                              reinterpret_cast<const void*>(&encode_f16x3_kernel<EPI_TOPK, 64, 0>),
                              reinterpret_cast<const void*>(&encode_f16x3_kernel<EPI_DENSE, 32, 1>),
                              reinterpret_cast<const void*>(&encode_f16x3_kernel<EPI_DENSE, 32, 2>)};
        for (const void* f : fns) {
            hipError_t e = hipFuncSetAttribute(f, hipFuncAttributeMaxDynamicSharedMemorySize, (int)smem);
            if (e != hipSuccess) return e;
        }
        attr_set = true;
    }
#define LAUNCH_ENC(...) hipLaunchKernelGGL((encode_f16x3_kernel<__VA_ARGS__>), grid, block, smem, stream, a)
#define LAUNCH_M16(...) hipLaunchKernelGGL((encode_m16_kernel<__VA_ARGS__>), grid, block, smem, stream, a)
    if (epi == EPI_DENSE) {
        if (a.arith == 1) LAUNCH_ENC(EPI_DENSE, 32, 1);
        else if (a.arith == 2) LAUNCH_ENC(EPI_DENSE, 32, 2);
        else LAUNCH_ENC(EPI_DENSE, 32, 0);
    } else if (a.ngroups <= 32 && a.heur_z != nullptr) {
        if (a.arith == 1) LAUNCH_ENC(EPI_TOPK, 32, 1, true);
        else if (a.arith == 2) LAUNCH_ENC(EPI_TOPK, 32, 2, true);
        else LAUNCH_ENC(EPI_TOPK, 32, 0, true);
    } else if (a.ngroups <= 32) {
        if (a.arith == 1) LAUNCH_M16(1);
        else if (a.arith == 2) LAUNCH_M16(2);
        else LAUNCH_ENC(EPI_TOPK, 32, 0);
    } else {
        if (a.arith == 1) LAUNCH_M16(1, 64);
        else if (a.arith == 2) LAUNCH_M16(2, 64);
        else LAUNCH_ENC(EPI_TOPK, 64, 0);
    }
#undef LAUNCH_M16
#undef LAUNCH_ENC
    return hipGetLastError();
}

int encode_f16x3_tile_rows() { return HTB; }
int encode_f16x3_tile_latents() { return HTS; }
```

saev_amd/csrc/kernels.h:

```cpp
#pragma once
#include <hip/hip_runtime.h>
#include <stdint.h>

#include <string>

#include "../../include/saev_amd.h"

enum { EPI_DENSE = 0, EPI_TOPK = 1 };

struct EncodeArgs {
    const float* x;
    const float* W_enc;
    const float* b_enc;
    int n_rows, D, S;
    int s_splits;
    float* h_out;
    int ngroups;
    int32_t* gmax;
    int gmax_stride;
    int32_t* cand_cnt;
    float* cand_val;
    int32_t* cand_idx;
    int cand_cap;
    int cand_stride;
    const int32_t* enable_flag;
    int enable_when;
};

size_t encode_gemm_smem_bytes();
hipError_t launch_encode_gemm(const EncodeArgs& a, int epi, hipStream_t stream);
int encode_gemm_tile_rows();
int encode_gemm_tile_latents();

struct SelectDenseArgs {
    const float* h;
    int n_rows, S;
    int k;
    const int32_t* k_dev;
    const int32_t* mask;
    int32_t* idx_out;
    float* val_out;
    int out_stride;
    const int32_t* enable_flag;
    int enable_when;
    int walk_grid;
};
hipError_t launch_select_dense(const SelectDenseArgs& a, hipStream_t stream);

struct SelectCandArgs {
    const int32_t* cand_cnt;
    const float* cand_val;
    const int32_t* cand_idx;
    int cand_cap, cand_stride, n_rows, k;
    int32_t* idx_out;
    float* val_out;
    int out_stride;
    const int32_t* enable_flag;
    int enable_when;
    const float* row_margin;
    const float* x;
    const float* W_encT;
    const float* b_enc;
    int D;
    int32_t* surv_idx;
    float* surv_val;
    int32_t* surv_cnt;
    int32_t* refine_overflow;
    const int32_t* tau_max;
    int32_t* invalid;
    int32_t* ovf;
    int32_t* surv_rng;
    int lat_range, n_ranges;
    const float* sum_part;
    const float* sum_bias;
    int sum_n;
    size_t sum_plane;
};
hipError_t launch_refine_exact(const SelectCandArgs& a, hipStream_t stream);
constexpr int REFINE_CAP = 512;
constexpr int RS_SLICE = 32;
constexpr int RS_ROWS_MAX = 8;
constexpr int RS_LAT_RANGE = 32768;
constexpr int RS_MAX_RANGES = 8;
struct RefineSlicesArgs {
    const int32_t* surv_idx; const int32_t* surv_cnt; float* surv_val; const int32_t* surv_rng;
    const float* xS; const float* WeS; const float* b_enc; float* part;
    int n_rows, S, D, lat_range, n_ranges;
    const int32_t* enable_flag; int enable_when;
};
hipError_t launch_refine_slices(const RefineSlicesArgs& a, hipStream_t stream);
hipError_t launch_select_cand(const SelectCandArgs& a, hipStream_t stream);
hipError_t launch_init_i32(int32_t* p, int32_t v, int n, hipStream_t stream);
hipError_t launch_encoder_init(int32_t* cand_cnt, int n_rows, int32_t* gmax, int n_gmax, hipStream_t stream,
                               int32_t* tau_max = nullptr, const int32_t* enable_flag = nullptr, int enable_when = 0);
hipError_t launch_pre_encode(int32_t* cand_cnt, int n_rows, int32_t* gmax, int n_gmax, const float* xnorm, int D,
                             const float* wg_part, int n_part, const float* scales, int32_t* pre_flag, float* wmax_prev,
                             float* margin, int32_t* flags1, hipStream_t stream);
hipError_t launch_heur_gate(float* state, const int32_t* pre_flag, int32_t* gate, hipStream_t stream);
hipError_t launch_heur_update(float* state, const int32_t* bad, const float* cand_mean, int k, const int32_t* gate,
                              hipStream_t stream);
hipError_t launch_step_zero(saev_step_stats* stats, float* upper, int32_t* flag0, hipStream_t stream);
hipError_t launch_wnorm_max(const float* W_encT, int S, int D, float* wg_scratch, float* wmax, hipStream_t stream);
hipError_t launch_f16r_scales(const float* xmax_part, int n_part, const float* wmax, float* scales, hipStream_t stream);
hipError_t launch_pow2_scale(const float* absmax, float* pair, hipStream_t stream);
hipError_t launch_center_stats(const float* x, const float* mu, int n, int D, float* xnorm, float* wg_absmax,
                               hipStream_t stream, const float* xmax = nullptr);
hipError_t launch_row_margins(const float* xnorm, int n, int D, const float* wg_part, int n_part, const float* scales,
                              int32_t* pre_flag, float* wmax_prev, float* margin, hipStream_t stream);
hipError_t launch_overflow_check(const int32_t* cand_cnt, int n_rows, int cap, const int32_t* pre_flag,
                                 int32_t* need_dense, int32_t* n_overflow, int32_t* cand_max, hipStream_t stream,
                                 int32_t* dense_out = nullptr, int32_t* run_out = nullptr, float* cand_mean = nullptr,
                                 const int32_t* enable_flag = nullptr, const int32_t* dense_src = nullptr);

struct __attribute__((aligned(8))) RowStats {
    float sse_scaled;
    float l0;
    float l1;
    float aux_sse;
    double sse64;
    double sumsq64;
};

struct DecodeArgs {
    const float* x;
    const int32_t* idx;
    const float* val;
    int code_stride, k;
    const float* W_dec;
    const float* b_dec;
// ... 143 lines not shown
    float* p; const float* g; float* m; float* v;
    long n;
    float lr, beta1, beta2, eps, bc1, bc2_sqrt;
    float omb1, omb2;
    float grad_scale;
    float max_norm;
    const double* sumsq;
    saev_step_stats* stats;
};
hipError_t launch_adam(const AdamArgs& a, hipStream_t stream);
hipError_t launch_adam_rows(const AdamArgs& a, const float2* row_proj, int S, int D, hipStream_t stream);
hipError_t launch_sumsq_final_ex(const double* partials, int nb, const float2* row_proj, int n_rows, const float* e1, long n1,
                                 const float* e2, long n2, double* total, double* blk_part, int* ticket, hipStream_t stream,
                                 const float* enc_sq = nullptr,
                                 const float* plain = nullptr, long n_plain = 0);
struct AdamImageArgs {
    _Float16* ws; float* WeS; double* dot_part; float* sq_part;
    const float* mu; const float* wmax_prev; float* scales_next;
    int nks, S_pad;
    int mode;
    uint32_t* chk; int32_t* late; int verify;
    const int32_t* early;
};
hipError_t launch_adam_fused(const AdamArgs& a, const float2* row_proj, const float* gT, int S, int D, long off_b_dec, long n_b_dec,
                             long off_W_enc, long off_b_enc, long n_b_enc, hipStream_t stream, const int32_t* lat_unused = nullptr,
                             const AdamImageArgs* img = nullptr);
constexpr int SUMSQ_EX_BLOCKS = 32;

struct DeadRecord {
    int64_t step;
    int64_t cum_tokens;
    int64_t horizon_tokens;
    int32_t n_dead;
    int32_t n_near;
};

struct DeadArgs {
    int64_t* toks;
    int32_t* fired;
    int32_t* dead;
    int S;
    int64_t add_tokens, threshold;
    int k_aux;
    int32_t* n_dead;
    int32_t* k_use;
    saev_step_stats* stats;
    int32_t* scratch;
    int64_t horizon_tokens;
    int64_t step, cum_tokens;
    DeadRecord* rec;
    int32_t* dead_list;
};
hipError_t launch_dead_update(const DeadArgs& a, hipStream_t stream);
hipError_t launch_stats_dead(const RowStats* rs, int n_rows, int D, int P, float alpha, const float* upper, const int32_t* n_overflow,
                             saev_step_stats* stats, double* scratch, const int32_t* cand_cnt, int cand_cap, const DeadArgs& d,
                             hipStream_t stream);
hipError_t launch_absmax(const float* x, long n, float* out_zeroed, hipStream_t stream);
hipError_t launch_gather_rows(const float* pool, const int64_t* rows, int n_rows, int D, float* out, hipStream_t stream);
hipError_t launch_scatter_dense(const int32_t* idx, const float* val, int n_rows, int k, int stride, int S, float* f,
                                hipStream_t stream);
hipError_t launch_stats_reduce(const RowStats* rs, int n_rows, int D, int P, float alpha, int with_aux, const float* upper,
                               const int32_t* n_overflow_and_max, saev_step_stats* stats, hipStream_t stream,
                               const int32_t* n_dead_dev, double* scratch,
                               const int32_t* cand_cnt = nullptr, int cand_cap = 0);
constexpr int STATS_SCRATCH_DOUBLES = 16 * 8 + 1;

struct EncodeF16Args {
    const _Float16* xs;
    const _Float16* ws;
    const float* b_enc;
    int n_rows, Dp, S;
    float w_scale;
    int arith;
    const float* row_margin;
    const float* scale_dev;
    const float* scale_dev_b;
    int s_splits;
    float* h_out;
    int ngroups;
    int top_k;
    int32_t* gmax;
    int gmax_stride;
    int32_t* cand_cnt;
    float* cand_val;
    int32_t* cand_idx;
    int cand_cap, cand_stride;
    const int32_t* enable_flag;
    int enable_when;
    const float* heur_z;
    int32_t* tau_max;
    int refresh_first, refresh_every;
    int n_batches;
    int blk_imgs;
    long out_bstride;
};
hipError_t launch_encode_f16x3(const EncodeF16Args& a, int epi, hipStream_t stream);
int encode_f16x3_tile_rows();
int encode_f16x3_tile_latents();
hipError_t launch_split_rows(const float* x, int n, int D, int Dp, void* xs, int mode, hipStream_t stream, float scale = 1.0f,
                             const float* scale_dev = nullptr,
                             const float* mu = nullptr,
                             float* xS = nullptr);
hipError_t launch_split_wT(const float* W, int D, int S, int S_pad, int Dp, float scale, void* ws, int mode,
                           hipStream_t stream, const float* scale_dev = nullptr,
                           const float* mu = nullptr, double* dot_part = nullptr, float* sq_part = nullptr,
                           float* W_T = nullptr,
                           int wt_slices = 0);
struct XprepArgs {
    const float* x;
    const int64_t* rows;
    float* x_out;
    int n, D, nks, n_pad;
    const float* scales;
    const float* mu;
    _Float16* xs;
    float* xS;
    float* xn_part;
    float* col_part;
    float* amax_part;
    float* cmax_part;
    const float* W_enc; const float* WeS; const float* b_enc; const float* b_seen;
    int S; uint32_t salt; int32_t* stale;
    float* mu_keep; float* xside_keep;
};
hipError_t launch_xprep(const XprepArgs& a, hipStream_t stream);
struct PreEncode2Args {
    int32_t* cand_cnt; int n_rows;
    int32_t* gmax; int n_gmax;
    const float* xn_part; int nks, n_pad, D;
    const float* wg_part; int n_part;
    const float* scales;
    float* scales_next;
    int32_t* pre_flag;
    float* wmax_prev;
    float* margin;
    float* xnorm;
    int32_t* flags1;
    const float* col_part; int n_rowblk;
    float* mu; float inv_n; int update_mu;
    const float* amax_part; const float* cmax_part; int n_img;
    float* upper;
    int32_t* stale; int32_t* stale_host;
    float* xside_keep;
    saev_step_stats* stats;
    int nb_rows;
};
hipError_t launch_pre_encode2(PreEncode2Args a, hipStream_t stream);
hipError_t launch_follower_scales(const float* xside, const float* wmax, float* scales, int32_t* pre_flag, int keep_w, hipStream_t stream);
hipError_t launch_split_both(const float* M, int R, int C, float scale, const float* scale_dev, void* rf, int kp_r, void* tf, int kp_t,
                             hipStream_t stream);
hipError_t launch_split_f16r(const float* x, int n, int D, int Dp, void* xs, const float* scales, const float* mu, const float* W,
                             int S, int S_pad, void* ws, double* dot_part, float* sq_part, float* W_T, hipStream_t stream,
                             float* xS = nullptr, int wt_slices = 0);
hipError_t launch_bias_finish(const double* dot_part, const float* sq_part, int Dp, int S, int S_pad, const float* w_scale,
                              const float* b_enc, float* b_shift, float* wg_part, hipStream_t stream, float* b_seen = nullptr);
hipError_t launch_max_reduce(const float* v, int n, float* out, hipStream_t stream);

hipError_t launch_dead_compact(const int32_t* dead, int S, int32_t* list, hipStream_t s,
                               const int32_t* n_dead_dev = nullptr);
hipError_t launch_gather_dead(const float* W_enc, const float* W_dec, const int32_t* dl, int nd, int ndp, int D, int S,
                              float* Wenc_dead, float* Wdec_dead, hipStream_t s,
                              const int32_t* nd_dev = nullptr);
hipError_t launch_dead_bias_vec(const float* b_enc, const int32_t* dl, int nd, int ndp, float* out, hipStream_t s,
                                bool pad_zero = false,
                                const int32_t* nd_dev = nullptr);
hipError_t launch_aux_scatter(const int32_t* idx, const float* val, int n_rows, int k, int stride, int ndp, float* A,
                              uint8_t* mask, hipStream_t s, const int32_t* k_dev = nullptr);
hipError_t launch_aux_resid(float* E, const float* x, const float* x_hat, const float* b_dec, int n_rows, int D,
                            float gscale, RowStats* rowstats, hipStream_t s, const int32_t* nd_dev = nullptr, float* part = nullptr,
                            float* pair = nullptr);
int absmax_parts_max(int n_rows_cap);
hipError_t launch_absmax_pow2(const float* x, long n, float* part, float* pair, hipStream_t s);
hipError_t launch_mask_apply_absmax(float* dA, const uint8_t* mask, long n, float* part, float* pair, hipStream_t s);
bool aux_select_supported(int ndp);
hipError_t launch_aux_select(const float* H, int n_rows, int ndp, int k, const int32_t* k_dev, float* A, uint8_t* mask, float* part,
                             float* pair, hipStream_t s);
hipError_t launch_mask_apply(float* dA, const uint8_t* mask, long n, hipStream_t s);
constexpr int AUX_SMALL_MAX = 64;
constexpr int AUX_SMALL_DEFAULT = 40;
hipError_t launch_gather_dead_small(const float* W_enc, const float* W_dec, const int32_t* dl, const int32_t* nd_dev, int D,
                                    int S, float* WencT_dead, float* Wdec_dead, hipStream_t s, int cap = AUX_SMALL_MAX);
hipError_t launch_aux_small_fwd(const float* x, const float* x_hat, const float* WencT_dead, const float* Wdec_dead,
                                const float* b_enc, const float* b_dec, const int32_t* dl, int n_rows, int D,
                                const int32_t* nd_dev, float gscale, float* A, float* dA, float* g_aux, RowStats* rowstats,
                                hipStream_t s);
hipError_t launch_aux_small_wsum(const float* part, int n_blk, int D, const int32_t* nd_dev, float* dWd, float* dWe, hipStream_t s,
                                 int ndp = AUX_SMALL_MAX);
constexpr int AUX_FUSED_MAX = 8;
constexpr int AUX_FUSED_ROWS = 32;
#ifndef AUX_FUSED_PF8
#define AUX_FUSED_PF8 1
#endif
#ifndef AUX_FUSED_PF4
#define AUX_FUSED_PF4 1
#endif
bool aux_fused_supported(int D);
constexpr int AUX_MFMA_MAX = 128;
// ... 186 lines not shown
```

saev_amd/csrc/select.hip:

```cpp
#include "common.h"
#include "kernels.h"

namespace {

constexpr int SD_THREADS = 256;

__device__ __forceinline__ int block_excl_scan_256(int v, int* lds_wave_tot, int& total) {
    const int lane = threadIdx.x & 63, w = threadIdx.x >> 6;
    int incl = v;
#pragma unroll
    for (int o = 1; o < 64; o <<= 1) {
        int n = __shfl_up(incl, o, 64);
        if (lane >= o) incl += n;
    }
    if (lane == 63) lds_wave_tot[w] = incl;
    __syncthreads();
    int base = 0, tot = 0;
#pragma unroll
    for (int i = 0; i < 4; ++i) {
        const int t = lds_wave_tot[i];
        if (i < w) base += t;
        tot += t;
    }
    total = tot;
// ... 164 lines not shown

    uint32_t key[EPL];
    int32_t idx[EPL];
#pragma unroll
    for (int e = 0; e < EPL; ++e) {
        const int p = e * 64 + lane;
        if (p < n) { key[e] = f2ukey(cv[p]); idx[e] = ci[p]; }
        else { key[e] = 0u; idx[e] = 0x7fffffff; }
    }
    auto kth_largest = [&]() {
        uint32_t t = 0;
        for (int bit = 31; bit >= 0; --bit) {
            const uint32_t trial = t | (1u << bit);
            int c = 0;
#pragma unroll
            for (int e = 0; e < EPL; ++e) c += __popcll(__ballot(key[e] >= trial));
            if (c == k) {
                uint32_t m = 0xffffffffu;
#pragma unroll
                for (int e = 0; e < EPL; ++e) m = min(m, key[e] >= trial ? key[e] : 0xffffffffu);
#pragma unroll
                for (int o = 32; o > 0; o >>= 1) m = min(m, (uint32_t)__shfl_xor((int)m, o, 64));
                return m;
            }
            if (c > k) t = trial;
        }
        return t;
    };
    uint32_t T = kth_largest();
    if (a.tau_max != nullptr && lane == 0 && (n < a.k || ukey2f(T) < key2f(a.tau_max[row]))) *a.invalid = 1;
    if (a.row_margin != nullptr) {
        const uint32_t key_lo = f2ukey(ukey2f(T) - a.row_margin[row]);
        int32_t* so = a.surv_idx + (size_t)row * REFINE_CAP;
        int base = 0;
        const int n_rng = a.surv_rng != nullptr ? a.n_ranges : 1;
        for (int r = 0; r < n_rng; ++r) {
            const int32_t lo = r * a.lat_range, hi = (r == n_rng - 1) ? 0x7ffffffe : lo + a.lat_range;
#pragma unroll
            for (int e = 0; e < EPL; ++e) {
                const bool sv = key[e] >= key_lo && idx[e] >= lo && idx[e] <= hi - (r == n_rng - 1 ? 0 : 1);
                const unsigned long long m = __ballot(sv);
                const int pos = base + __popcll(m & ((1ull << lane) - 1ull));
                if (sv && pos < REFINE_CAP) so[pos] = idx[e];
                base += __popcll(m);
            }
            if (a.surv_rng != nullptr && lane == 0) a.surv_rng[(size_t)row * RS_MAX_RANGES + r] = min(base, REFINE_CAP);
        }
        if (lane == 0) {
            a.surv_cnt[row] = min(base, REFINE_CAP);
            if (base > REFINE_CAP) *a.refine_overflow = 1;
        }
        return;
    }
    int cgt = 0, ceq = 0;
#pragma unroll
    for (int e = 0; e < EPL; ++e) { cgt += __popcll(__ballot(key[e] > T)); ceq += __popcll(__ballot(key[e] == T)); }
    const int need = k - cgt;
    int32_t idx_cut = 0x7fffffff;
    if (ceq > need) {
        int32_t X = 0;
        for (int bit = 30; bit >= 0; --bit) {
            const int32_t trial = X | (1 << bit);
            int c = 0;
#pragma unroll
            for (int e = 0; e < EPL; ++e) c += __popcll(__ballot(key[e] == T && idx[e] < trial));
            if (c < need) X = trial;
        }
        idx_cut = X;
    }
    s_idx[w][lane] = 0x7fffffff;
    s_val[w][lane] = 0.f;
    int base = 0;
#pragma unroll
    for (int e = 0; e < EPL; ++e) {
        const bool sel = (key[e] > T) || (key[e] == T && idx[e] <= idx_cut);
        const unsigned long long m = __ballot(sel);
        const int pos = base + __popcll(m & ((1ull << lane) - 1ull));
        if (sel && pos < 64) { s_idx[w][pos] = idx[e]; s_val[w][pos] = ukey2f(key[e]); }
        base += __popcll(m);
    }
    sort_by_idx_and_store(a, row, k, s_idx[w][lane], s_val[w][lane], lane);
}

__device__ __forceinline__ int stream_count(const float* cv, const int32_t* ci, int n, uint32_t lo_key, int mode, uint32_t T,
                                            int32_t idx_lt, int lane) {
    int c = 0;
    for (int p0 = 0; p0 < n; p0 += 64) {
        const int p = p0 + lane;
        bool hit = false;
        if (p < n) {
            const uint32_t key = f2ukey(cv[p]);
            hit = mode == 0 ? key >= lo_key : mode == 1 ? key > T : mode == 2 ? key == T : (key == T && ci[p] < idx_lt);
        }
        c += __popcll(__ballot(hit));
    }
    return c;
}
__device__ __forceinline__ uint32_t stream_kth_largest(const float* cv, const int32_t* ci, int n, int k, int lane) {
    uint32_t t = 0;
    for (int bit = 31; bit >= 0; --bit) {
        const uint32_t trial = t | (1u << bit);
        const int c = stream_count(cv, ci, n, trial, 0, 0u, 0, lane);
        if (c == k) {
            uint32_t m = 0xffffffffu;
            for (int p = lane; p < n; p += 64) { const uint32_t key = f2ukey(cv[p]); if (key >= trial) m = min(m, key); }
#pragma unroll
            for (int o = 32; o > 0; o >>= 1) m = min(m, (uint32_t)__shfl_xor((int)m, o, 64));
            return m;
        }
        if (c > k) t = trial;
    }
    return t;
}
__device__ __forceinline__ int stream_survivors(const SelectCandArgs& a, int row, int n, const float* cv, const int32_t* ci,
                                                int32_t* out, uint32_t* T_out) {
    const int lane = threadIdx.x & 63;
    const uint32_t T = stream_kth_largest(cv, ci, n, min(a.k, n), lane);
    *T_out = T;
    const uint32_t key_lo = f2ukey(ukey2f(T) - a.row_margin[row]);
    int base = 0;
    const int n_rng = a.surv_rng != nullptr ? a.n_ranges : 1;
    for (int r = 0; r < n_rng; ++r) {
        const int32_t lo = r * a.lat_range, hi = (r == n_rng - 1) ? 0x7ffffffe : lo + a.lat_range - 1;
        for (int p0 = 0; p0 < n; p0 += 64) {
            const int p = p0 + lane;
            bool sv = p < n && f2ukey(cv[p]) >= key_lo;
            if (sv && n_rng > 1) { const int32_t i = ci[p]; sv = i >= lo && i <= hi; }
            const unsigned long long m = __ballot(sv);
            const int pos = base + __popcll(m & ((1ull << lane) - 1ull));
            if (sv && pos < REFINE_CAP) out[pos] = ci[p];
            base += __popcll(m);
        }
        if (a.surv_rng != nullptr && lane == 0) a.surv_rng[(size_t)row * RS_MAX_RANGES + r] = min(base, REFINE_CAP);
    }
    return base;
}
__device__ __forceinline__ void select_cand_row_stream(const SelectCandArgs& a, int row, int n, int32_t (&s_idx)[4][64],
                                                       float (&s_val)[4][64], const float* cv, const int32_t* ci) {
    const int lane = threadIdx.x & 63, w = threadIdx.x >> 6;
    const int k = min(a.k, n);
    if (a.row_margin != nullptr) {
        uint32_t T;
        const int base = stream_survivors(a, row, n, cv, ci, a.surv_idx + (size_t)row * REFINE_CAP, &T);
        if (a.tau_max != nullptr && lane == 0 && (n < a.k || ukey2f(T) < key2f(a.tau_max[row]))) *a.invalid = 1;
        if (lane == 0) {
            a.surv_cnt[row] = min(base, REFINE_CAP);
            if (base > REFINE_CAP) *a.refine_overflow = 1;
        }
        return;
    }
    const uint32_t T = stream_kth_largest(cv, ci, n, k, lane);
    if (a.tau_max != nullptr && lane == 0 && (n < a.k || ukey2f(T) < key2f(a.tau_max[row]))) *a.invalid = 1;
    const int cgt = stream_count(cv, ci, n, 0u, 1, T, 0, lane), ceq = stream_count(cv, ci, n, 0u, 2, T, 0, lane);
    const int need = k - cgt;
    int32_t idx_cut = 0x7fffffff;
    if (ceq > need) {
        int32_t X = 0;
        for (int bit = 30; bit >= 0; --bit) {
            const int32_t trial = X | (1 << bit);
            if (stream_count(cv, ci, n, 0u, 3, T, trial, lane) < need) X = trial;
        }
        idx_cut = X;
    }
    s_idx[w][lane] = 0x7fffffff;
    s_val[w][lane] = 0.f;
    int base = 0;
    for (int p0 = 0; p0 < n; p0 += 64) {
        const int p = p0 + lane;
        uint32_t key = 0u;
        int32_t idx = 0x7fffffff;
        if (p < n) { key = f2ukey(cv[p]); idx = ci[p]; }
        const bool sel = p < n && ((key > T) || (key == T && idx <= idx_cut));
        const unsigned long long m = __ballot(sel);
        const int pos = base + __popcll(m & ((1ull << lane) - 1ull));
        if (sel && pos < 64) { s_idx[w][pos] = idx; s_val[w][pos] = ukey2f(key); }
        base += __popcll(m);
    }
    sort_by_idx_and_store(a, row, k, s_idx[w][lane], s_val[w][lane], lane);
}

__device__ __forceinline__ void select_small_row(const SelectCandArgs& a, int row, int n, const float* cv, const int32_t* ci) {
    const int lane = threadIdx.x & 63;
    const int k = min(a.k, n);
    uint32_t key = 0u;
    int32_t idx = 0x7fffffff;
    if (lane < n) {
        key = f2ukey(cv[lane]);
        idx = ci[lane];
    }
#pragma unroll
    for (int size = 2; size <= 64; size <<= 1) {
#pragma unroll
        for (int stride = size >> 1; stride > 0; stride >>= 1) {
            const uint32_t o_key = __shfl_xor(key, stride, 64);
            const int32_t o_idx = __shfl_xor(idx, stride, 64);
            const bool other_first = (o_key > key) || (o_key == key && o_idx < idx);
            const bool up = ((lane & size) == 0);
            const bool lower = ((lane & stride) == 0);
            const bool take_other = (lower == up) ? other_first : !other_first;
            if (take_other) { key = o_key; idx = o_idx; }
        }
    }
    if (a.tau_max != nullptr) {
        const float kth = ukey2f(__shfl(key, max(k - 1, 0), 64));
        if (lane == 0 && (n < a.k || kth < key2f(a.tau_max[row]))) *a.invalid = 1;
    }
    const bool win = lane < k;
    sort_by_idx_and_store(a, row, k, win ? idx : 0x7fffffff, win ? ukey2f(key) : 0.f, lane);
}

template <bool BIG>
__global__ __launch_bounds__(256) void select_cand_kernel(SelectCandArgs a) {
    if (a.enable_flag != nullptr && (*a.enable_flag != 0) != (a.enable_when != 0)) return;
    __shared__ int32_t s_idx[4][64];
    __shared__ float s_val[4][64];
    const int row = blockIdx.x * 4 + (threadIdx.x >> 6);
    if (row >= a.n_rows) return;
    const int cnt = a.cand_cnt[row];
    if (a.ovf != nullptr && (threadIdx.x & 63) == 0 && cnt > a.cand_cap) atomicOr(&a.ovf[0], 1);
    if (a.ovf != nullptr && a.row_margin != nullptr && (threadIdx.x & 63) == 0 && !(a.row_margin[row] < 3.0e38f)) atomicOr(&a.ovf[0], 1);
    const int n = min(cnt, a.cand_cap);
    const float* cv = a.cand_val + (size_t)row * a.cand_stride;
    const int32_t* ci = a.cand_idx + (size_t)row * a.cand_stride;
    __shared__ float l_sum[4][REFINE_CAP];
    if (a.sum_part != nullptr) {
        float* const lv = l_sum[threadIdx.x >> 6];
        for (int j = threadIdx.x & 63; j < n; j += 64) {
            const size_t o = (size_t)row * a.cand_stride + j;
            float sv = 0.f;
            int c = 0;
            for (; c + 8 <= a.sum_n; c += 8) {
                float v[8];
#pragma unroll
                for (int u = 0; u < 8; ++u) v[u] = a.sum_part[(size_t)(c + u) * a.sum_plane + o];
#pragma unroll
                for (int u = 0; u < 8; ++u) sv += v[u];
            }
            for (; c < a.sum_n; ++c) sv += a.sum_part[(size_t)c * a.sum_plane + o];
            lv[j] = sv + a.sum_bias[ci[j]];
        }
        __asm__ volatile("" ::: "memory");
        cv = lv;
    }
    if (n <= 64 && a.row_margin == nullptr) select_small_row(a, row, n, cv, ci);
    else if (n <= 512) select_cand_row<8>(a, row, n, s_idx, s_val, cv, ci);
    else if (n <= 1024) select_cand_row<16>(a, row, n, s_idx, s_val, cv, ci);
    else if (n <= 2048) select_cand_row<32>(a, row, n, s_idx, s_val, cv, ci);
    else if constexpr (BIG) select_cand_row<64>(a, row, n, s_idx, s_val, cv, ci);
    else select_cand_row_stream(a, row, n, s_idx, s_val, cv, ci);
}

__global__ void init_i32_kernel(int32_t* p, int32_t v, int n) {
    const int i = blockIdx.x * blockDim.x + threadIdx.x;
    if (i < n) p[i] = v;
}

__global__ void encoder_init_kernel(int32_t* cand_cnt, int n_rows, int32_t* gmax, int n_gmax, int32_t* tau_max,
                                    const int32_t* enable_flag, int enable_when) {
    if (enable_flag != nullptr && (*enable_flag != 0) != (enable_when != 0)) return;
    const int i = blockIdx.x * blockDim.x + threadIdx.x;
    if (i < n_rows) cand_cnt[i] = 0;
    if (i < n_gmax) gmax[i] = INT32_MIN;
    if (tau_max != nullptr && i < n_rows) tau_max[i] = INT32_MIN;
}
__global__ void step_zero_kernel(saev_step_stats* stats, float* upper, int32_t* flag0) {
    if (threadIdx.x == 0) {
        *stats = saev_step_stats{};
        *upper = 0.f;
        *flag0 = 0;
    }
}

template <int NV>
__global__ __launch_bounds__(256) void refine_exact_kernel(SelectCandArgs a) {
    if (a.enable_flag != nullptr && (*a.enable_flag != 0) != (a.enable_when != 0)) return;
    const int lane = threadIdx.x & 63;
    const int row = blockIdx.x * 4 + (threadIdx.x >> 6);
    if (row >= a.n_rows) return;
    const int ns = a.surv_cnt[row];
    const int D4 = a.D >> 2;
    f32x4 xv[NV];
    const f32x4* xr = reinterpret_cast<const f32x4*>(a.x + (size_t)row * a.D);
#pragma unroll
    for (int n = 0; n < NV; ++n) xv[n] = (lane + 64 * n < D4) ? xr[lane + 64 * n] : f32x4{0.f, 0.f, 0.f, 0.f};
    const int32_t* si = a.surv_idx + (size_t)row * REFINE_CAP;
    float* sv = a.surv_val + (size_t)row * REFINE_CAP;
    for (int j0 = 0; j0 < ns; j0 += 8) {
        const int32_t my = si[min(j0 + (lane & 7), ns - 1)];
        float p[8];
#pragma unroll
        for (int t = 0; t < 8; ++t) {
            const int32_t li = __shfl(my, t, 64);
            const f32x4* wr = reinterpret_cast<const f32x4*>(a.W_encT + (size_t)li * a.D);
            float acc = 0.f;
#pragma unroll
            for (int n = 0; n < NV; ++n) {
                if (lane + 64 * n < D4) {
                    const f32x4 wv = wr[lane + 64 * n];
                    acc += xv[n][0] * wv[0] + xv[n][1] * wv[1] + xv[n][2] * wv[2] + xv[n][3] * wv[3];
                }
            }
            p[t] = acc;
        }
        const float r = wave_reduce_scatter8(p, lane);
        if ((lane & 7) == 0) {
            const int t = lane >> 3;
            if (j0 + t < ns) sv[j0 + t] = r + a.b_enc[si[j0 + t]];
        }
    }
}

typedef int i32x4 __attribute__((ext_vector_type(4)));
__device__ __forceinline__ f32x4 rs_buf_load16(__amdgpu_buffer_rsrc_t r, uint32_t voff) {
    const i32x4 v = __builtin_amdgcn_raw_buffer_load_b128(r, voff, 0, 0);
    return f32x4{__int_as_float(v[0]), __int_as_float(v[1]), __int_as_float(v[2]), __int_as_float(v[3])};
}
__device__ __forceinline__ float group8_reduce_scatter(float (&p)[8], int li) {
// ... 178 lines not shown
    const float t = wmax * w_scale;
    return t < 60000.0f && (t >= 2048.0f || wmax == 0.f);
}
__global__ __launch_bounds__(256) void row_margin_kernel(const float* xnorm, int n, int D, const float* wg_part, int n_part,
                                                         const float* scales, int32_t* pre_flag, float* wmax_prev,
                                                         float* margin) {
    __shared__ float sh[3][4];
    float bm = 0.f, wm = 0.f, dm = 0.f;
    for (int i = threadIdx.x; i < n_part; i += 256) { bm = fmaxf(bm, wg_part[i]); wm = fmaxf(wm, wg_part[n_part + i]); dm = fmaxf(dm, wg_part[2 * n_part + i]); }
    bm = wave_max(bm); wm = wave_max(wm); dm = wave_max(dm);
    if ((threadIdx.x & 63) == 0) { sh[0][threadIdx.x >> 6] = bm; sh[1][threadIdx.x >> 6] = wm; sh[2][threadIdx.x >> 6] = dm; }
    __syncthreads();
    const float bmax = fmaxf(fmaxf(sh[0][0], sh[0][1]), fmaxf(sh[0][2], sh[0][3]));
    const float wmax = fmaxf(fmaxf(sh[1][0], sh[1][1]), fmaxf(sh[1][2], sh[1][3]));
    const float dwmax = fmaxf(fmaxf(sh[2][0], sh[2][1]), fmaxf(sh[2][2], sh[2][3]));
    if (blockIdx.x == 0 && threadIdx.x == 0) {
        if (!f16r_scale_ok(wmax, scales[1])) *pre_flag = 1;
        *wmax_prev = wmax;
    }
    const int r = blockIdx.x * 256 + threadIdx.x;
    if (r >= n) return;
    margin[r] = f16r_margin(xnorm[2 * r], xnorm[2 * r + 1], wmax, dwmax, bmax, D, scales[0]);
}
__global__ __launch_bounds__(256) void pre_encode_kernel(int32_t* cand_cnt, int n_rows, int32_t* gmax, int n_gmax,
                                                         const float* xnorm, int D, const float* wg_part, int n_part,
                                                         const float* scales, int32_t* pre_flag, float* wmax_prev,
                                                         float* margin, int32_t* flags1) {
    const int i = blockIdx.x * 256 + threadIdx.x;
    if (i < n_rows) cand_cnt[i] = 0;
    if (i < n_gmax) gmax[i] = INT32_MIN;
    if (xnorm == nullptr) {
        if (i == 0) { flags1[0] = (pre_flag != nullptr && *pre_flag != 0) ? 1 : 0; flags1[1] = 0; flags1[2] = 0; }
        return;
    }
    if ((int)blockIdx.x * 256 >= n_rows && blockIdx.x != 0) return;
    __shared__ float sh[3][4];
    float bm = 0.f, wm = 0.f, dm = 0.f;
    for (int j = threadIdx.x; j < n_part; j += 256) { bm = fmaxf(bm, wg_part[j]); wm = fmaxf(wm, wg_part[n_part + j]); dm = fmaxf(dm, wg_part[2 * n_part + j]); }
    bm = wave_max(bm); wm = wave_max(wm); dm = wave_max(dm);
    if ((threadIdx.x & 63) == 0) { sh[0][threadIdx.x >> 6] = bm; sh[1][threadIdx.x >> 6] = wm; sh[2][threadIdx.x >> 6] = dm; }
    __syncthreads();
    const float bmax = fmaxf(fmaxf(sh[0][0], sh[0][1]), fmaxf(sh[0][2], sh[0][3]));
    const float wmax = fmaxf(fmaxf(sh[1][0], sh[1][1]), fmaxf(sh[1][2], sh[1][3]));
    const float dwmax = fmaxf(fmaxf(sh[2][0], sh[2][1]), fmaxf(sh[2][2], sh[2][3]));
    if (i == 0) {
        int pre = *pre_flag != 0 ? 1 : 0;
        if (!f16r_scale_ok(wmax, scales[1])) { pre = 1; *pre_flag = 1; }
        *wmax_prev = wmax;
        flags1[0] = pre; flags1[1] = 0; flags1[2] = 0;
    }
    if (i >= n_rows) return;
    margin[i] = f16r_margin(xnorm[2 * i], xnorm[2 * i + 1], wmax, dwmax, bmax, D, scales[0]);
}
__global__ __launch_bounds__(256) void pre_encode2_kernel(PreEncode2Args a) {
    __shared__ float sh[5][4];
    const int i = blockIdx.x * 256 + threadIdx.x;
    if ((int)blockIdx.x >= a.nb_rows) {
        const int d = ((int)blockIdx.x - a.nb_rows) * 256 + threadIdx.x;
        if (d >= a.D || !a.update_mu) return;
        float t = 0.f;
        int b = 0;
        for (; b + 8 <= a.n_rowblk; b += 8) {
            float v[8];
#pragma unroll
            for (int u = 0; u < 8; ++u) v[u] = a.col_part[(size_t)(b + u) * a.D + d];
#pragma unroll
            for (int u = 0; u < 8; ++u) t += v[u];
        }
        for (; b < a.n_rowblk; ++b) t += a.col_part[(size_t)b * a.D + d];
        t *= a.inv_n;
        if (t - t == 0.f) a.mu[d] = t;
        return;
    }
    if (i < a.n_rows) a.cand_cnt[i] = 0;
    if (i < a.n_gmax) a.gmax[i] = INT32_MIN;
    float bm = 0.f, wm = 0.f, dm = 0.f, am = 0.f, cm = 0.f;
    for (int j = threadIdx.x; j < a.n_part; j += 256) { bm = fmaxf(bm, a.wg_part[j]); wm = fmaxf(wm, a.wg_part[a.n_part + j]); dm = fmaxf(dm, a.wg_part[2 * a.n_part + j]); }
    if (blockIdx.x == 0)
        for (int j = threadIdx.x; j < a.n_img; j += 256) { am = fmaxf(am, a.amax_part[j]); cm = fmaxf(cm, a.cmax_part[j]); }
    bm = wave_max(bm); wm = wave_max(wm); dm = wave_max(dm); am = wave_max(am); cm = wave_max(cm);
    if ((threadIdx.x & 63) == 0) { const int w = threadIdx.x >> 6; sh[0][w] = bm; sh[1][w] = wm; sh[2][w] = dm; sh[3][w] = am; sh[4][w] = cm; }
    __syncthreads();
    const float bmax = fmaxf(fmaxf(sh[0][0], sh[0][1]), fmaxf(sh[0][2], sh[0][3]));
    const float wmax = fmaxf(fmaxf(sh[1][0], sh[1][1]), fmaxf(sh[1][2], sh[1][3]));
    const float dwmax = fmaxf(fmaxf(sh[2][0], sh[2][1]), fmaxf(sh[2][2], sh[2][3]));
    const float x_scale = a.scales[0];
    if (i == 0) {
        const float amax = fmaxf(fmaxf(sh[3][0], sh[3][1]), fmaxf(sh[3][2], sh[3][3]));
        const float cmax = fmaxf(fmaxf(sh[4][0], sh[4][1]), fmaxf(sh[4][2], sh[4][3]));
        int pre = 0;
        if (!f16r_scale_ok(wmax, a.scales[1])) pre = 1;
        if (!(cmax * x_scale < 60000.0f)) pre = 1;
        if (a.xside_keep != nullptr && !(cmax * x_scale < 60000.0f)) a.xside_keep[1] = 1.0f;
        if (a.stale != nullptr) {
            const bool caught = *a.stale != 0;
            if (caught) {
                pre = 1;
                *a.stale = 0;
                if (a.stale_host != nullptr) *a.stale_host = 1;
            }
            a.stale[1] = caught ? 1 : 0;
        }
        *a.pre_flag = pre;
        *a.wmax_prev = wmax;
        a.flags1[0] = pre; a.flags1[1] = 0; a.flags1[2] = 0;
        *a.upper = amax;
        *a.stats = saev_step_stats{};
        const float xs_next = (cmax > 0.f && cmax < 3.0e38f) ? exp2f(13.0f - floorf(log2f(cmax))) : x_scale;
        a.scales_next[0] = xs_next;
        a.scales_next[2] = xs_next;
        a.scales_next[4] = (amax > 0.f && amax < 3.0e38f) ? amax : a.scales[4];
    }
    if (i >= a.n_rows) return;
    const float up = a.scales[4];
    const float back = (up > 0.f && up < 3.0e38f) ? up : 1.0f;
    float s2 = 0.f, d2 = 0.f;
    int ks = 0;
    for (; ks + 8 <= a.nks; ks += 8) {
        float2 t[8];
#pragma unroll
        for (int u = 0; u < 8; ++u) t[u] = reinterpret_cast<const float2*>(a.xn_part)[(size_t)(ks + u) * a.n_pad + i];
#pragma unroll
        for (int u = 0; u < 8; ++u) { s2 += t[u].x; d2 += t[u].y; }
    }
    for (; ks < a.nks; ++ks) {
        const float2 t = reinterpret_cast<const float2*>(a.xn_part)[(size_t)ks * a.n_pad + i];
        s2 += t.x; d2 += t.y;
    }
    const float xn = back * sqrtf(s2) * 1.000001f, xd = back * sqrtf(d2) * 1.000002f;
    if (a.xnorm != nullptr) { a.xnorm[2 * i] = xn; a.xnorm[2 * i + 1] = xd; }
    a.margin[i] = f16r_margin(xn, xd, wmax, dwmax, bmax, a.D, x_scale);
}
__global__ void follower_scales_kernel(const float* xside, const float* wmax, float* scales, int32_t* pre_flag, int keep_w) {
    if (threadIdx.x != 0) return;
    scales[0] = xside[0];
    scales[2] = xside[0];
    scales[3] = 1.0f;
    if (!keep_w) {
        const float wm = *wmax;
        scales[1] = (wm > 0.f && wm < 3.0e38f) ? exp2f(13.0f - floorf(log2f(wm))) : 1.0f;
    }
    if (xside[1] != 0.f) *pre_flag = 1;
}
__global__ void pow2_scale_kernel(const float* absmax, float* pair) {
    if (threadIdx.x == 0) {
        const float m = *absmax;
        pair[0] = (m > 0.f && m < 3.0e38f) ? exp2f(13.0f - floorf(log2f(m))) : 1.0f;
        pair[1] = 1.0f;
    }
}
__global__ __launch_bounds__(256) void f16r_scales_kernel(const float* xmax_part, int n_part, const float* wmax, float* scales) {
    __shared__ float sh[4];
    float m = 0.f;
    for (int i = threadIdx.x; i < n_part; i += 256) m = fmaxf(m, xmax_part[i]);
    m = wave_max(m);
    if ((threadIdx.x & 63) == 0) sh[threadIdx.x >> 6] = m;
    __syncthreads();
    if (threadIdx.x == 0) {
        const float xm = fmaxf(fmaxf(sh[0], sh[1]), fmaxf(sh[2], sh[3])), wm = *wmax;
        scales[0] = (xm > 0.f && xm < 3.0e38f) ? exp2f(13.0f - floorf(log2f(xm))) : 1.0f;
        scales[1] = (wm > 0.f && wm < 3.0e38f) ? exp2f(13.0f - floorf(log2f(wm))) : 1.0f;
        scales[2] = scales[0];
        scales[3] = 1.0f;
    }
}

__global__ void overflow_check_kernel(const int32_t* cand_cnt, int n_rows, int cap, const int32_t* pre_flag,
                                      int32_t* bad_out, int32_t* n_overflow, int32_t* cand_max, int32_t* dense_out,
                                      int32_t* run_out, float* cand_mean, const int32_t* enable_flag,
                                      const int32_t* dense_src) {
    if (enable_flag != nullptr && *enable_flag == 0) {
        if (threadIdx.x == 0 && run_out != nullptr) *run_out = 0;
        return;
    }
    __shared__ int sh, shmax, shsum;
    if (threadIdx.x == 0) { sh = 0; shmax = 0; shsum = 0; }
    __syncthreads();
    int c = 0, m = 0, t = 0;
    for (int i = threadIdx.x; i < n_rows; i += blockDim.x) { const int v = cand_cnt[i]; c += (v > cap); m = max(m, v); t += min(v, cap); }
    c = wave_sum_i(c);
    t = wave_sum_i(t);
#pragma unroll
    for (int o = 32; o > 0; o >>= 1) m = max(m, __shfl_xor(m, o, 64));
    if ((threadIdx.x & 63) == 0) { if (c) atomicAdd(&sh, c); atomicMax(&shmax, m); atomicAdd(&shsum, t); }
// ... 9 lines not shown
        } else {
            const int dense = (*dense_out != 0 || sh > 0) ? 1 : 0;
            *dense_out = dense;
            *run_out = dense ? 0 : 1;
        }
    }
}

__global__ void heur_gate_kernel(float* state, const int32_t* pre_flag, int32_t* gate) {
    if (threadIdx.x != 0) return;
    int g = (pre_flag != nullptr && *pre_flag != 0) ? 1 : 0;
    if (state[5] > 0.f) { state[5] -= 1.f; g = 1; }
    *gate = g;
}
__global__ void heur_update_kernel(float* state, const int32_t* bad, const float* cand_mean, int k, const int32_t* gate) {
    if (threadIdx.x != 0 || *gate != 0) return;
    float z = state[0];
    state[2] += 1.f;
    if (*bad != 0) {
        z -= 0.3f;
        state[1] += 1.f;
        state[4] += 1.f;
        if (state[4] >= 3.f) { state[4] = 0.f; state[5] = 256.f; z = 1.5f; }
    } else {
        state[4] = 0.f;
        if (*cand_mean > 3.f * (float)k) z += 0.002f;
    }
    state[0] = fminf(fmaxf(z, 0.5f), 3.5f);
}

}

hipError_t launch_select_dense(const SelectDenseArgs& a, hipStream_t stream) {
    if (a.n_rows <= 0) return hipSuccess;
    const int grid = (a.walk_grid > 0 && a.walk_grid < a.n_rows) ? a.walk_grid : a.n_rows;
    hipLaunchKernelGGL(select_dense_kernel, dim3(grid), dim3(SD_THREADS), 0, stream, a);
    return hipGetLastError();
}

hipError_t launch_select_cand(const SelectCandArgs& a, hipStream_t stream) {
    if (a.n_rows <= 0) return hipSuccess;
    if (a.cand_cap > 4096 || (a.sum_part != nullptr && a.cand_cap > REFINE_CAP)) return hipErrorInvalidValue;
    if (a.k > 32) hipLaunchKernelGGL(select_cand_kernel<true>, dim3((a.n_rows + 3) / 4), dim3(256), 0, stream, a);
    else hipLaunchKernelGGL(select_cand_kernel<false>, dim3((a.n_rows + 3) / 4), dim3(256), 0, stream, a);
    return hipGetLastError();
}

hipError_t launch_init_i32(int32_t* p, int32_t v, int n, hipStream_t stream) {
    if (n <= 0) return hipSuccess;
    hipLaunchKernelGGL(init_i32_kernel, dim3((n + 255) / 256), dim3(256), 0, stream, p, v, n);
    return hipGetLastError();
}

hipError_t launch_encoder_init(int32_t* cand_cnt, int n_rows, int32_t* gmax, int n_gmax, hipStream_t stream, int32_t* tau_max,
                               const int32_t* enable_flag, int enable_when) {
    const int n = n_rows > n_gmax ? n_rows : n_gmax;
    if (n <= 0) return hipSuccess;
    hipLaunchKernelGGL(encoder_init_kernel, dim3((n + 255) / 256), dim3(256), 0, stream, cand_cnt, n_rows, gmax, n_gmax, tau_max,
                       enable_flag, enable_when);
    return hipGetLastError();
}
hipError_t launch_pre_encode(int32_t* cand_cnt, int n_rows, int32_t* gmax, int n_gmax, const float* xnorm, int D,
                             const float* wg_part, int n_part, const float* scales, int32_t* pre_flag, float* wmax_prev,
                             float* margin, int32_t* flags1, hipStream_t stream) {
    const int n = std::max(1, n_rows > n_gmax ? n_rows : n_gmax);
    hipLaunchKernelGGL(pre_encode_kernel, dim3((n + 255) / 256), dim3(256), 0, stream, cand_cnt, n_rows, gmax, n_gmax, xnorm, D,
                       wg_part, n_part, scales, pre_flag, wmax_prev, margin, flags1);
    return hipGetLastError();
}
hipError_t launch_follower_scales(const float* xside, const float* wmax, float* scales, int32_t* pre_flag, int keep_w, hipStream_t stream) {
    hipLaunchKernelGGL(follower_scales_kernel, dim3(1), dim3(64), 0, stream, xside, wmax, scales, pre_flag, keep_w);
    return hipGetLastError();
}
hipError_t launch_pre_encode2(PreEncode2Args a, hipStream_t stream) {
    a.nb_rows = (std::max(1, std::max(a.n_rows, a.n_gmax)) + 255) / 256;
    hipLaunchKernelGGL(pre_encode2_kernel, dim3(a.nb_rows + (a.D + 255) / 256), dim3(256), 0, stream, a);
    return hipGetLastError();
}
hipError_t launch_heur_gate(float* state, const int32_t* pre_flag, int32_t* gate, hipStream_t stream) {
    hipLaunchKernelGGL(heur_gate_kernel, dim3(1), dim3(64), 0, stream, state, pre_flag, gate);
    return hipGetLastError();
}
hipError_t launch_heur_update(float* state, const int32_t* bad, const float* cand_mean, int k, const int32_t* gate,
                              hipStream_t stream) {
    hipLaunchKernelGGL(heur_update_kernel, dim3(1), dim3(64), 0, stream, state, bad, cand_mean, k, gate);
    return hipGetLastError();
}
hipError_t launch_step_zero(saev_step_stats* stats, float* upper, int32_t* flag0, hipStream_t stream) {
    hipLaunchKernelGGL(step_zero_kernel, dim3(1), dim3(64), 0, stream, stats, upper, flag0);
    return hipGetLastError();
}

hipError_t launch_wnorm_max(const float* W_encT, int S, int D, float* wg_scratch, float* wmax, hipStream_t stream) {
    const int nwg = (S + 3) / 4;
    hipLaunchKernelGGL(rownorm_wgmax_kernel, dim3(nwg), dim3(256), 0, stream, W_encT, S, D, wg_scratch);
    hipLaunchKernelGGL(max_reduce_kernel, dim3(1), dim3(1024), 0, stream, wg_scratch, nwg, wmax);
    return hipGetLastError();
}
hipError_t launch_f16r_scales(const float* xmax_part, int n_part, const float* wmax, float* scales, hipStream_t stream) {
    hipLaunchKernelGGL(f16r_scales_kernel, dim3(1), dim3(256), 0, stream, xmax_part, n_part, wmax, scales);
    return hipGetLastError();
}
hipError_t launch_pow2_scale(const float* absmax, float* pair, hipStream_t stream) {
    hipLaunchKernelGGL(pow2_scale_kernel, dim3(1), dim3(64), 0, stream, absmax, pair);
    return hipGetLastError();
}
// ... 49 lines not shown
```

saev_amd/csrc/tail.hip:

```cpp
#include "common.h"
#include "kernels.h"

namespace {

template <int NV>
__global__ __launch_bounds__(256) void normalize_rows_kernel(float* W, int S, int D, float* wn2) {
    const int lane = threadIdx.x & 63;
    const int i = blockIdx.x * 4 + (threadIdx.x >> 6);
    if (i >= S) return;
    const int D4 = D >> 2;
    f32x4* r = reinterpret_cast<f32x4*>(W + (size_t)i * D);
    f32x4 v[NV];
    float ss = 0.f;
#pragma unroll
    for (int n = 0; n < NV; ++n) {
        const int q = lane + 64 * n;
        v[n] = (q < D4) ? r[q] : f32x4{0.f, 0.f, 0.f, 0.f};
        ss += v[n][0] * v[n][0] + v[n][1] * v[n][1] + v[n][2] * v[n][2] + v[n][3] * v[n][3];
    }
    ss = wave_sum(ss);
    const float nrm = sqrtf(ss);
    float s2 = 0.f;
#pragma unroll
    for (int n = 0; n < NV; ++n) {
// ... 492 lines not shown
            last_n = t;
        }
    }
    if (a.dead_list == nullptr) return;
    __syncthreads();
    if (last_n > 0) dead_compact_block(a.dead, a.S, a.dead_list, wave_tot);
}
__global__ __launch_bounds__(256) void dead_update_kernel(DeadArgs a) {
    a.dead_list = nullptr;
    dead_update_body(a, blockIdx.x, gridDim.x);
}

__global__ __launch_bounds__(256) void absmax_kernel(const float* x, long n, float* out) {
    const long n4 = n >> 2;
    float m = 0.f;
    for (long q = (long)blockIdx.x * 256 + threadIdx.x; q < n4; q += (long)gridDim.x * 256) {
        const f32x4 v = reinterpret_cast<const f32x4*>(x)[q];
        m = fmaxf(fmaxf(fmaxf(m, fabsf(v[0])), fabsf(v[1])), fmaxf(fabsf(v[2]), fabsf(v[3])));
    }
    if (blockIdx.x == 0)
        for (long i = (n4 << 2) + threadIdx.x; i < n; i += 256) m = fmaxf(m, fabsf(x[i]));
    m = wave_max(m);
    __shared__ float shm[4];
    if ((threadIdx.x & 63) == 0) shm[threadIdx.x >> 6] = m;
    __syncthreads();
    if (threadIdx.x == 0)
        atomicMax(reinterpret_cast<unsigned int*>(out),
                  __float_as_uint(fmaxf(fmaxf(shm[0], shm[1]), fmaxf(shm[2], shm[3]))));
}

__global__ __launch_bounds__(256) void gather_rows_kernel(const float* pool, const int64_t* rows, int n_rows, int D,
                                                          float* out) {
    const int lane = threadIdx.x & 63;
    const int r = blockIdx.x * 4 + (threadIdx.x >> 6);
    if (r >= n_rows) return;
    const f32x4* src = reinterpret_cast<const f32x4*>(pool + (size_t)rows[r] * D);
    f32x4* dst = reinterpret_cast<f32x4*>(out + (size_t)r * D);
    for (int q = lane; q < (D >> 2); q += 64) dst[q] = src[q];
}

__global__ __launch_bounds__(256) void scatter_dense_kernel(const int32_t* idx, const float* val, int n_rows, int k,
                                                            int stride, int S, float* f) {
    const long p = (long)blockIdx.x * 256 + threadIdx.x;
    if (p >= (long)n_rows * k) return;
    const int b = (int)(p / k), j = (int)(p % k);
    const int32_t i = idx[(size_t)b * stride + j];
    if (i >= 0 && i < S) f[(size_t)b * S + i] = val[(size_t)b * stride + j];
}

struct StatsArgs {
    const RowStats* rs; int n_rows, D, P; float alpha; int with_aux; const float* upper; const int32_t* n_overflow;
    saev_step_stats* stats; const int32_t* n_dead_dev; double* scratch; const int32_t* cand_cnt; int cand_cap;
};
__device__ __forceinline__ void stats_reduce_body(const StatsArgs& A, int bid, int n_blocks) {
    const RowStats* rs = A.rs; const int n_rows = A.n_rows, D = A.D, P = A.P; const float alpha = A.alpha; const int with_aux = A.with_aux;
    const float* upper = A.upper; const int32_t* n_overflow = A.n_overflow; saev_step_stats* stats = A.stats;
    const int32_t* n_dead_dev = A.n_dead_dev; double* scratch = A.scratch; const int32_t* cand_cnt = A.cand_cnt; const int cand_cap = A.cand_cap;
    if (with_aux == 2 && *n_dead_dev <= 0) return;
    constexpr int NS = 8;
    __shared__ double sh[16][NS];
    __shared__ int last;
    double s[NS] = {0, 0, 0, 0, 0, 0, 0, 0};
    const int per = (n_rows + n_blocks - 1) / n_blocks;
    const int r0 = bid * per, r1 = min(n_rows, r0 + per);
    for (int r = r0 + threadIdx.x; r < r1; r += 1024) {
        const RowStats v = rs[r];
        s[0] += v.sse_scaled; s[1] += v.l0; s[2] += v.l1; s[3] += with_aux ? v.aux_sse : 0.f;
        s[4] += v.sse64; s[5] += v.sumsq64;
        if (cand_cnt != nullptr) {
            const int c = cand_cnt[r];
            s[6] += c > cand_cap ? 1.0 : 0.0;
            s[7] = fmax(s[7], (double)c);
        }
    }
#pragma unroll
    for (int i = 0; i < 7; ++i) s[i] = wave_sum_d(s[i]);
#pragma unroll
    for (int o = 32; o > 0; o >>= 1) s[7] = fmax(s[7], __shfl_xor(s[7], o, 64));
    if ((threadIdx.x & 63) == 0)
        for (int i = 0; i < NS; ++i) sh[threadIdx.x >> 6][i] = s[i];
    __syncthreads();
    int* ticket = reinterpret_cast<int*>(scratch + 16 * NS);
    if (threadIdx.x < NS) {
        const int i = threadIdx.x;
        double t = 0.0;
        for (int w = 0; w < 16; ++w) t = i < 7 ? t + sh[w][i] : fmax(t, sh[w][i]);
        __hip_atomic_store(&scratch[bid * NS + i], t, __ATOMIC_RELAXED, __HIP_MEMORY_SCOPE_AGENT);
    }
    asm volatile("s_waitcnt vmcnt(0)" ::: "memory");
    __syncthreads();
    if (threadIdx.x == 0) {
        __threadfence();
        last = (atomicAdd(ticket, 1) == n_blocks - 1) ? 1 : 0;
        if (last) __threadfence();
    }
    __syncthreads();
    if (!last) return;
    __shared__ double part[16][NS];
    if (threadIdx.x < 16 * NS) {
        const int b = threadIdx.x / NS, i = threadIdx.x % NS;
        part[b][i] = b < n_blocks ? __hip_atomic_load(&scratch[b * NS + i], __ATOMIC_RELAXED, __HIP_MEMORY_SCOPE_AGENT) : 0.0;
    }
    __syncthreads();
    if (threadIdx.x != 0) return;
    {
        double t[NS] = {0, 0, 0, 0, 0, 0, 0, 0};
        for (int b = 0; b < n_blocks; ++b) {
            for (int i = 0; i < 7; ++i) t[i] += part[b][i];
            t[7] = fmax(t[7], part[b][7]);
        }
        *ticket = 0;
        const double nd = (double)n_rows * (double)D;
        stats->mse = (float)(t[0] / (nd * (double)P));
        stats->l0 = (float)(t[1] / n_rows);
        stats->l1 = (float)(t[2] / n_rows);
        if (with_aux) stats->aux = (float)((double)alpha * t[3] / nd);
        stats->sse = t[4];
        stats->sum_sq = t[5];
        if (upper) stats->upper = *upper;
        if (n_overflow) { stats->n_overflow_rows = n_overflow[0]; stats->cand_max = n_overflow[1]; stats->dense_route = n_overflow[-1]; }
        if (cand_cnt != nullptr) { stats->n_overflow_rows = (int32_t)t[6]; stats->cand_max = (int32_t)t[7]; }
    }
}

template <typename F>
hipError_t dispatch_nv(int D, F&& f) {
    const int nv = (D / 4 + 63) / 64;
    switch (nv) {
        case 1: f(std::integral_constant<int, 1>()); break;
        case 2: f(std::integral_constant<int, 2>()); break;
        case 3: f(std::integral_constant<int, 3>()); break;
        case 4: f(std::integral_constant<int, 4>()); break;
        case 5: f(std::integral_constant<int, 5>()); break;
        case 6: f(std::integral_constant<int, 6>()); break;
        case 7: case 8: f(std::integral_constant<int, 8>()); break;
        case 9: case 10: case 11: case 12: f(std::integral_constant<int, 12>()); break;
        case 13: case 14: case 15: case 16: f(std::integral_constant<int, 16>()); break;
        default: return hipErrorInvalidValue;
    }
    return hipGetLastError();
}

__global__ __launch_bounds__(1024) void stats_reduce_kernel(StatsArgs A) { stats_reduce_body(A, blockIdx.x, gridDim.x); }
__global__ __launch_bounds__(1024) void stats_dead_kernel(StatsArgs A, int n_stat, DeadArgs d) {
    if ((int)blockIdx.x < n_stat) stats_reduce_body(A, blockIdx.x, n_stat);
    else dead_update_body(d, (int)blockIdx.x - n_stat, (int)gridDim.x - n_stat);
}

}

hipError_t launch_normalize_rows(float* W, int S, int D, hipStream_t stream, float* wn2) {
    return dispatch_nv(D, [&](auto nv) {
        hipLaunchKernelGGL(normalize_rows_kernel<decltype(nv)::value>, dim3((S + 3) / 4), dim3(256), 0, stream, W, S, D, wn2);
    });
}
hipError_t launch_rpg(float* gW, const float* W, int S, int D, hipStream_t stream, double* sq_partials, int project) {
    if (S <= 0) return hipSuccess;
    return dispatch_nv(D, [&](auto nv) {
        hipLaunchKernelGGL(rpg_kernel<decltype(nv)::value>, dim3((S + 3) / 4), dim3(256), 0, stream, gW, W, S, D, sq_partials,
                           project);
    });
}
int sumsq_blocks() { return SUMSQ_BLOCKS; }
hipError_t launch_sumsq_partials(const float* g, long n, double* partials, hipStream_t stream) {
    hipLaunchKernelGGL(sumsq_partial_kernel, dim3(SUMSQ_BLOCKS), dim3(256), 0, stream, g, n, partials);
    return hipGetLastError();
}
hipError_t launch_sumsq_final(const double* partials, int nb, double* total, hipStream_t stream) {
    hipLaunchKernelGGL(sumsq_final_kernel, dim3(1), dim3(1024), 0, stream, partials, nb, total);
    return hipGetLastError();
}
hipError_t launch_sumsq(const float* g, long n, double* partials, double* total, hipStream_t stream) {
    hipLaunchKernelGGL(sumsq_partial_kernel, dim3(SUMSQ_BLOCKS), dim3(256), 0, stream, g, n, partials);
    hipLaunchKernelGGL(sumsq_final_kernel, dim3(1), dim3(1024), 0, stream, partials, SUMSQ_BLOCKS, total);
    return hipGetLastError();
}
hipError_t launch_sumsq_final_ex(const double* partials, int nb, const float2* row_proj, int n_rows, const float* e1, long n1,
                                 const float* e2, long n2, double* total, double* blk_part, int* ticket, hipStream_t stream,
                                 const float* enc_sq, const float* plain, long n_plain) {
    hipLaunchKernelGGL(sumsq_final_ex_kernel, dim3(SUMSQ_EX_BLOCKS), dim3(1024), 0, stream, partials, nb, row_proj, n_rows, e1, n1, e2,
                       n2, total, blk_part, ticket, enc_sq, plain, n_plain);
    return hipGetLastError();
}
hipError_t launch_adam_rows(const AdamArgs& a, const float2* row_proj, int S, int D, hipStream_t stream) {
    if (S <= 0) return hipSuccess;
    return dispatch_nv(D, [&](auto nv) {
        hipLaunchKernelGGL(adam_rows_kernel<decltype(nv)::value>, dim3((S + 3) / 4), dim3(256), 0, stream, a, row_proj, S, D);
    });
}
hipError_t launch_adam_fused(const AdamArgs& a, const float2* row_proj, const float* gT, int S, int D, long off_b_dec, long n_b_dec,
                             long off_W_enc, long off_b_enc, long n_b_enc, hipStream_t stream, const int32_t* lat_unused,
                             const AdamImageArgs* img) {
    AdamFusedArgs f{};
    if (img != nullptr && D % 32 == 0) f.img = *img;
    f.a = a; f.row_proj = row_proj; f.gT = gT; f.S = S; f.D = D; f.lat_unused = lat_unused;
    f.off_b_dec = off_b_dec; f.n_b_dec = n_b_dec; f.off_W_enc = off_W_enc; f.off_b_enc = off_b_enc; f.n_b_enc = n_b_enc;
    f.nb_rows = (S + 3) / 4;
    f.tiles_s = (S + 255) / 256;
    f.nb_tiles = f.tiles_s * ((D + 31) / 32);
    const int nb_bias = 32;
    return dispatch_nv(D, [&](auto nv) {
        hipLaunchKernelGGL((adam_fused_kernel<decltype(nv)::value, 2>), dim3(f.nb_rows + f.nb_tiles + nb_bias), dim3(256), 0, stream, f);
    });
}
hipError_t launch_adam(const AdamArgs& a, hipStream_t stream) {
    const long n4 = a.n >> 2;
    const int blocks = (int)std::max<long>(1, std::min<long>((n4 + 1023) / 1024, 256 * 8));
    hipLaunchKernelGGL(adam_kernel, dim3(blocks), dim3(256), 0, stream, a);
    return hipGetLastError();
}
hipError_t launch_dead_update(const DeadArgs& a, hipStream_t stream) {
    hipLaunchKernelGGL(dead_update_kernel, dim3((a.S + 255) / 256), dim3(256), 0, stream, a);
    return hipGetLastError();
}
hipError_t launch_absmax(const float* x, long n, float* out_zeroed, hipStream_t stream) {
    const int blocks = (int)std::max<long>(1, std::min<long>(((n >> 2) + 255) / 256, 1024));
    hipLaunchKernelGGL(absmax_kernel, dim3(blocks), dim3(256), 0, stream, x, n, out_zeroed);
    return hipGetLastError();
}
hipError_t launch_gather_rows(const float* pool, const int64_t* rows, int n_rows, int D, float* out, hipStream_t stream) {
    if (n_rows <= 0) return hipSuccess;
    hipLaunchKernelGGL(gather_rows_kernel, dim3((n_rows + 3) / 4), dim3(256), 0, stream, pool, rows, n_rows, D, out);
    return hipGetLastError();
}
hipError_t launch_scatter_dense(const int32_t* idx, const float* val, int n_rows, int k, int stride, int S, float* f,
                                hipStream_t stream) {
    const long n = (long)n_rows * k;
    if (n <= 0) return hipSuccess;
    hipLaunchKernelGGL(scatter_dense_kernel, dim3((unsigned)((n + 255) / 256)), dim3(256), 0, stream, idx, val, n_rows, k,
                       stride, S, f);
    return hipGetLastError();
}
hipError_t launch_stats_reduce(const RowStats* rs, int n_rows, int D, int P, float alpha, int with_aux, const float* upper,
                               const int32_t* n_overflow, saev_step_stats* stats, hipStream_t stream,
                               const int32_t* n_dead_dev, double* scratch, const int32_t* cand_cnt, int cand_cap) {
    const int nb = std::max(1, std::min(16, (n_rows + 1023) / 1024));
    const StatsArgs A{rs, n_rows, D, P, alpha, with_aux, upper, n_overflow, stats, n_dead_dev, scratch, cand_cnt, cand_cap};
    hipLaunchKernelGGL(stats_reduce_kernel, dim3(nb), dim3(1024), 0, stream, A);
    return hipGetLastError();
}
hipError_t launch_stats_dead(const RowStats* rs, int n_rows, int D, int P, float alpha, const float* upper, const int32_t* n_overflow,
                             saev_step_stats* stats, double* scratch, const int32_t* cand_cnt, int cand_cap, const DeadArgs& d,
                             hipStream_t stream) {
    const int nb = std::max(1, std::min(16, (n_rows + 1023) / 1024));
    const StatsArgs A{rs, n_rows, D, P, alpha, 0, upper, n_overflow, stats, nullptr, scratch, cand_cnt, cand_cap};
    hipLaunchKernelGGL(stats_dead_kernel, dim3(nb + (d.S + 1023) / 1024), dim3(1024), 0, stream, A, nb, d);
    return hipGetLastError();
}
```

saev_amd/engine.py:

```python

from __future__ import annotations

import ctypes as C
import dataclasses
import math
import os

import torch

from . import _lib


DEFAULT_ENCODER = "f16r"


@dataclasses.dataclass(frozen=True)
class EngineConfig:
    d_model: int
    d_sae: int
    top_k: int = 32
    k_aux: int = 512
    alpha: float = 1.0 / 32.0
    dead_threshold_tokens: int = 10_000_000
    normalize_w_dec: bool = True
    remove_parallel_grads: bool = True
    max_batch: int = 16384
    aux_dead_cap: int = 0
    shard_world: int = 1
    max_backward_rows: int = 0
    bounds: str = dataclasses.field(default_factory=lambda: os.environ.get("SAEV_AMD_BOUNDS", "guaranteed"))
    encoder: str = dataclasses.field(default_factory=lambda: os.environ.get("SAEV_AMD_ENCODER", DEFAULT_ENCODER))
    dw_route: str = dataclasses.field(default_factory=lambda: os.environ.get("SAEV_AMD_DW", "slices"))
    fwd_route: str = dataclasses.field(default_factory=lambda: os.environ.get("SAEV_AMD_FWD", "default"))
    aux_small_max: int = dataclasses.field(default_factory=lambda: int(os.environ.get("SAEV_AMD_AUX_SMALL_MAX", "0")))
    csc_route: int = dataclasses.field(default_factory=lambda: int(os.environ.get("SAEV_AMD_CSC", "0")))
    fin_route: int = dataclasses.field(default_factory=lambda: int(os.environ.get("SAEV_AMD_FIN", "0")))
    prep_route: int = dataclasses.field(default_factory=lambda: int(os.environ.get("SAEV_AMD_PREP", "0")))
    aux_dense_route: int = dataclasses.field(default_factory=lambda: int(os.environ.get("SAEV_AMD_AUX_DENSE", "0")))
    aux_small_route: int = dataclasses.field(default_factory=lambda: int(os.environ.get("SAEV_AMD_AUX_SMALL", "0")))
    group_route: int = dataclasses.field(default_factory=lambda: int(os.environ.get("SAEV_AMD_GROUP", "0")))
    aux_split_route: int = dataclasses.field(default_factory=lambda: int(os.environ.get("SAEV_AMD_AUX_SPLIT", "0")))
    aux_wide_route: int = dataclasses.field(default_factory=lambda: int(os.environ.get("SAEV_AMD_AUX_WIDE", "0")))
    activation: str = "topk"
    row_cap: int = 0
    batch_momentum: float = 0.1
    select_list_cap: int = 0
    l1_coeff: float = 0.0


@dataclasses.dataclass(frozen=True)
class MuonConfig:

    weight_decay: float = 0.1
    momentum: float = 0.95
    nesterov: bool = True
    ns_coefficients: tuple[float, float, float] = (3.4445, -4.7750, 2.0315)
    eps: float = 1e-07
    ns_steps: int = 5
    adjust_lr_fn: str | None = None

    def c_struct(self) -> "_lib.SaevMuonCfg":
        adj = {None: 0, "original": 0, "match_rms_adamw": 1, "none": 2}
        if self.adjust_lr_fn not in adj:
            raise ValueError(f"adjust_lr_fn must be None, 'original' or 'match_rms_adamw', got {self.adjust_lr_fn!r}")
        a, b, c = self.ns_coefficients
        return _lib.SaevMuonCfg(momentum=self.momentum, weight_decay=self.weight_decay, a=a, b=b, c=c, eps=self.eps,
                                nesterov=int(self.nesterov), ns_steps=self.ns_steps, adjust_lr=adj[self.adjust_lr_fn])


def newton_schulz(x: torch.Tensor, muon: MuonConfig | None = None, *, normalize: bool = True) -> torch.Tensor:
    if x.ndim != 2 or not x.is_cuda:
        raise ValueError("newton_schulz takes a 2-D device matrix")
    lib = _lib.load()
    muon = muon or MuonConfig()
    tall = x.shape[0] > x.shape[1]
    xb = (x.t() if tall else x).to(torch.bfloat16).contiguous()
    rows, cols = xb.shape
    nbytes = int(lib.saev_muon_workspace_bytes(rows, cols))
    if nbytes < 0:
        raise _lib.SaevError(f"newton_schulz: unsupported shape {tuple(x.shape)}")
    ws = torch.empty(nbytes, device=x.device, dtype=torch.uint8)
    out = torch.empty_like(xb)
    cfg = muon.c_struct()
# ... 1318 lines not shown
@dataclasses.dataclass
class StepStats:
    mse: float
    aux: float
    l0: float
    l1: float
    grad_norm: float
    upper: float
    n_dead: int
    n_overflow_rows: int
    cand_max: int
    dense_route: int
    sse: float
    sum_sq: float

    @property
    def loss(self) -> float:
        return self.mse + self.aux


def flat_layout(cfg: EngineConfig) -> "_lib.SaevLayout":
    lay = _lib.SaevLayout()
    ccfg = _lib.SaevCfg(d_model=cfg.d_model, d_sae=cfg.d_sae, shard_world=cfg.shard_world)
    rc = _lib.load().saev_layout(C.byref(ccfg), C.byref(lay))
    if rc != 0:
        raise _lib.SaevError(f"saev_layout failed with status {rc} for {cfg}")
    return lay


def _ptr(t: torch.Tensor | None):
    return None if t is None else C.c_void_p(t.data_ptr())


def _stream():
    return C.c_void_p(torch.cuda.current_stream().cuda_stream)


class SaeEngine:
    def __init__(self, cfg: EngineConfig, device: torch.device | str | int = "cuda", *, with_optim: bool = True):
        if not torch.cuda.is_available():
            raise _lib.SaevError("saev_amd needs a HIP device (torch.cuda.is_available() is False); there is no CPU path")
        self.lib = _lib.load()
        self.cfg = cfg
        self.device = torch.device(device if not isinstance(device, int) else f"cuda:{device}")
        if self.device.index is None:
            self.device = torch.device("cuda", torch.cuda.current_device())
        S, D = cfg.d_sae, cfg.d_model
        lay = flat_layout(cfg)
        self.n_params = lay.n_total
        self.shard_world = cfg.shard_world
        self.chunk_a, self.chunk_b = lay.chunk_a, lay.chunk_b
        self.offsets = {"W_dec": lay.off_W_dec, "b_dec": lay.off_b_dec, "W_enc": lay.off_W_enc, "b_enc": lay.off_b_enc}
        self.shapes = {"W_dec": (S, D), "b_dec": (D,), "W_enc": (D, S), "b_enc": (S,)}
        if cfg.bounds not in ("guaranteed", "predicted"):
            raise ValueError(f"EngineConfig.bounds (SAEV_AMD_BOUNDS) must be 'guaranteed' or 'predicted', got {cfg.bounds!r}")
        if cfg.encoder not in ("f32", "f16x3", "bf16", "f16r"):
            raise ValueError(f"EngineConfig.encoder (SAEV_AMD_ENCODER) must be one of f32, f16x3, bf16, f16r, got {cfg.encoder!r}")
        if cfg.activation not in ("topk", "relu", "batch_topk", "relu_train"):
            raise ValueError(f"EngineConfig.activation must be 'topk', 'relu', 'batch_topk' or 'relu_train', got {cfg.activation!r}")
        if cfg.activation == "relu_train" and cfg.encoder == "bf16":
            raise NotImplementedError("the bf16 encoder is not available for ReLU SAEs: use f32, f16x3 or f16r")
        if cfg.activation == "relu_train" and (cfg.shard_world > 1 or cfg.max_backward_rows > cfg.max_batch):
            raise NotImplementedError("a ReLU training engine runs on one GPU (world > 1 is not on this path)")
        if cfg.activation == "relu_train" and not (cfg.l1_coeff >= 0.0 and math.isfinite(cfg.l1_coeff)):
            raise ValueError(f"EngineConfig.l1_coeff must be a finite number >= 0, got {cfg.l1_coeff!r}")
        if cfg.activation == "batch_topk" and cfg.encoder == "bf16":
            raise NotImplementedError("the bf16 encoder is not available for BatchTopK SAEs: use f32, f16x3 or f16r")
        if cfg.activation == "batch_topk" and (cfg.shard_world > 1 or cfg.max_backward_rows > cfg.max_batch):
            raise NotImplementedError("a BatchTopK engine runs on one GPU (a batch-wide top-k over ranks needs a distributed select)")
        if cfg.activation in ("relu", "relu_train") and cfg.k_aux != 0:
            raise ValueError("a ReLU engine has no auxiliary loss: k_aux must be 0")
        with torch.cuda.device(self.device):
            self.params = torch.zeros(self.n_params, device=self.device, dtype=torch.float32)
            self.grads = torch.zeros_like(self.params) if with_optim else None
            self.adam_m = torch.zeros_like(self.params) if with_optim else None
            self.adam_v = torch.zeros_like(self.params) if with_optim else None
            self.toks_since_active = torch.zeros(S, device=self.device, dtype=torch.int64)
            self.fired = torch.zeros(S, device=self.device, dtype=torch.int32)
            if cfg.dw_route not in ("slices", "rows", "slices_a") or cfg.fwd_route not in ("default", "rows"):
                raise ValueError(f"EngineConfig.dw_route must be 'slices', 'slices_a' or 'rows' and fwd_route 'default' or 'rows', got {cfg.dw_route!r} / {cfg.fwd_route!r}")
            self.sumsq = torch.zeros(1, device=self.device, dtype=torch.float64)
            self.threshold = torch.zeros((), device=self.device, dtype=torch.float32) if cfg.activation == "batch_topk" else None
            self.row_cap = 0
            self.row_regrows = 0
            self._w_enc_t = None
            self._prefixes = None
            self.ctx = None
            self._create_ctx()
            self._params_version = self._pversion()
        self.adam_steps = 0
        self._x_keepalive = None
        self._last_n = 0
        self.relu_row_cap = min(cfg.d_sae, 512)
        self.relu_second_launches = 0

    def _create_ctx(self) -> None:
        cfg, S, D = self.cfg, self.cfg.d_sae, self.cfg.d_model
        ccfg = _lib.SaevCfg(
            d_model=D, d_sae=S, top_k=cfg.top_k, k_aux=cfg.k_aux, alpha=cfg.alpha,
            dead_threshold_tokens=cfg.dead_threshold_tokens,
            normalize_w_dec=int(cfg.normalize_w_dec), remove_parallel_grads=int(cfg.remove_parallel_grads),
            max_batch=cfg.max_batch, encoder_mode={"f32": 0, "f16x3": 1, "bf16": 2, "f16r": 3}[cfg.encoder],
            aux_dead_cap=cfg.aux_dead_cap, shard_world=cfg.shard_world,
            bound_mode={"guaranteed": 0, "predicted": 1}[cfg.bounds], max_backward_rows=cfg.max_backward_rows,
            activation={"topk": _lib.ACT_TOPK, "relu": _lib.ACT_RELU, "batch_topk": _lib.ACT_BATCHTOPK, "relu_train": _lib.ACT_RELU}[cfg.activation],
        )
        dbg = _lib.SaevDebugCfg(
            struct_size=C.sizeof(_lib.SaevDebugCfg), dw_route={"slices": 0, "rows": 1, "slices_a": 2}[cfg.dw_route],
            aux_small_max=cfg.aux_small_max, fwd_route={"default": 0, "rows": 1}[cfg.fwd_route],
            csc_route=cfg.csc_route, fin_route=cfg.fin_route, prep_route=cfg.prep_route, aux_dense_route=cfg.aux_dense_route, aux_small_route=cfg.aux_small_route,
            group_route=cfg.group_route, aux_split_route=cfg.aux_split_route, aux_wide_route=cfg.aux_wide_route)
        ctx = C.c_void_p()
        if cfg.activation == "batch_topk":
            bt = _lib.SaevBatchTopKCfg(struct_size=C.sizeof(_lib.SaevBatchTopKCfg), row_cap=cfg.row_cap, batch_momentum=cfg.batch_momentum,
                                       list_cap=cfg.select_list_cap)
            rc = self.lib.saev_create_batch_topk(C.byref(ccfg), C.byref(dbg), C.byref(bt), self.device.index, C.byref(ctx))
        elif cfg.activation == "relu_train":
            rt = _lib.SaevReluTrainCfg(struct_size=C.sizeof(_lib.SaevReluTrainCfg), l1_coeff=float(cfg.l1_coeff))
            rc = self.lib.saev_create_relu_train(C.byref(ccfg), C.byref(dbg), C.byref(rt), self.device.index, C.byref(ctx))
        else:
            rc = self.lib.saev_create_ex(C.byref(ccfg), C.byref(dbg), self.device.index, C.byref(ctx))
        if rc != 0:
            raise _lib.SaevError(f"saev_create failed with status {rc} for {cfg}")
        self.ctx = ctx
        self._chk(self.lib.saev_bind(ctx, _ptr(self.params), _ptr(self.grads), _ptr(self.adam_m), _ptr(self.adam_v)), "saev_bind")
        self._chk(self.lib.saev_bind_tracker(ctx, _ptr(self.toks_since_active), _ptr(self.fired)), "saev_bind_tracker")
        self._chk(self.lib.saev_bind_sumsq(ctx, _ptr(self.sumsq)), "saev_bind_sumsq")
        if self._w_enc_t is not None:
            self._chk(self.lib.saev_bind_w_enc_t(ctx, _ptr(self._w_enc_t)), "saev_bind_w_enc_t")
        if self.threshold is not None:
            self._chk(self.lib.saev_bind_threshold(ctx, _ptr(self.threshold)), "saev_bind_threshold")
            self.row_cap = int(self.lib.saev_row_cap(ctx))
        if self._prefixes is not None:
            self.set_prefixes(self._prefixes)

    def _grow_rows(self, need: int) -> None:
        if need <= self.row_cap:
            raise _lib.SaevError(f"BatchTopK row overflow reported {need} codes for rows of {self.row_cap}")
        torch.cuda.synchronize(self.device)
        self.lib.saev_destroy(self.ctx)
        self.ctx = None
        self.cfg = dataclasses.replace(self.cfg, row_cap=min(self.cfg.d_sae, (need + 63) // 64 * 64))
        with torch.cuda.device(self.device):
            self._create_ctx()
        self.row_regrows += 1
        self._last_n = 0

    def _chk(self, rc, what):
        _lib.check(self.lib, self.ctx, rc, what)

    def _topk_only(self, what: str):
        if self.cfg.activation == "batch_topk":
            raise NotImplementedError(f"{what} is not available for a BatchTopK SAE (one GPU, the phases or train_step, encode_batch_topk)")
        if self.cfg.activation == "relu_train":
            raise NotImplementedError(f"{what} is not available for a ReLU training engine (one GPU, the phases in one piece or train_step, "
                                      "encode_relu)")
        if self.cfg.activation != "topk":
# ... 501 lines not shown
        return self.row_cap if self.cfg.activation == "batch_topk" else min(self.cfg.top_k, self.cfg.d_sae)

    def last_codes(self, n_rows: int, *, x_hat: bool = True, row_nnz: bool = False):
        if self.cfg.activation == "relu_train":
            return self._relu_last_rows(n_rows, x_hat, row_nnz)
        k = self._code_width()
        idx = torch.empty(n_rows, k, device=self.device, dtype=torch.int32)
        val = torch.empty(n_rows, k, device=self.device, dtype=torch.float32)
        x_hat = torch.empty(n_rows, self.cfg.d_model, device=self.device, dtype=torch.float32) if x_hat else None
        self._chk(self.lib.saev_copy_last(self.ctx, n_rows, _ptr(idx), _ptr(val), _ptr(x_hat), _stream()), "saev_copy_last")
        if not row_nnz:
            return idx, val, x_hat
        nnz = torch.empty(n_rows, device=self.device, dtype=torch.int32)
        self._chk(self.lib.saev_copy_last_row_nnz(self.ctx, n_rows, _ptr(nnz), _stream()), "saev_copy_last_row_nnz")
        return idx, val, x_hat, nnz

    def _relu_last_rows(self, n_rows: int, x_hat: bool, row_nnz: bool):
        S = self.cfg.d_sae
        cap = max(1, min(S, self.relu_row_cap))
        over = torch.empty(1, device=self.device, dtype=torch.int32)
        nnz = torch.empty(n_rows, device=self.device, dtype=torch.int32)
        for attempt in range(2):
            idx = torch.empty(n_rows, cap, device=self.device, dtype=torch.int32)
            val = torch.empty(n_rows, cap, device=self.device, dtype=torch.float32)
            self._chk(self.lib.saev_copy_last_rows(self.ctx, n_rows, cap, _ptr(nnz), _ptr(idx), _ptr(val), _ptr(over), _stream()),
                      "saev_copy_last_rows")
            need = int(over.item())
            if need == 0:
                break
            if attempt == 1:
                raise _lib.SaevError(f"saev_copy_last_rows overflowed a capacity of {cap} sized from its own count {need}")
            cap = need
            self.relu_second_launches += 1
            self.relu_row_cap = max(self.relu_row_cap, min(S, (need + 63) // 64 * 64))
        xh = None
        if x_hat:
            xh = torch.empty(n_rows, self.cfg.d_model, device=self.device, dtype=torch.float32)
            self._chk(self.lib.saev_copy_last(self.ctx, n_rows, None, None, _ptr(xh), _stream()), "saev_copy_last")
        return (idx, val, xh, nnz) if row_nnz else (idx, val, xh)

    def aux_route(self) -> int:
        return int(self.lib.saev_last_aux_route(self.ctx))

    def scratch_bytes(self, which: int = 0) -> int:
        return int(self.lib.saev_scratch_bytes(self.ctx, which))

    def dead_readbacks(self) -> int:
        return int(self.lib.saev_dead_readbacks(self.ctx))

    def bound_state(self) -> dict:
        z, mc = C.c_float(), C.c_float()
        n, r = C.c_int64(), C.c_int64()
        self._chk(self.lib.saev_bound_state(self.ctx, C.byref(z), C.byref(n), C.byref(r), C.byref(mc), _stream()), "saev_bound_state")
        return {"z": z.value, "launches": n.value, "repeats": r.value, "mean_candidates": mc.value}

    def enable_kernel_timing(self, on: bool = True):
        self._chk(self.lib.saev_enable_kernel_timing(self.ctx, int(on)), "saev_enable_kernel_timing")

    def encoder_ms(self) -> float:
        return float(self.lib.saev_last_encoder_ms(self.ctx))
```

Before: 6.307 million.

## Add norm-ratio bound mode that predicts per-row top-k threshold from input norm

Adds a new bound mode 'norm' (now the default). It keeps a per-row lower bound on the k-th activation, scaled by the row's input norm with an adaptive ratio rho. A controller inside the stats kernel maintains rho from the previous step's k-th values, and the encoder uses this per-row threshold to prune candidates instead of refreshing a running tau in shared memory. Rows whose bound fails are detected and re-encoded in a second pass, and the controller pauses after misses. This trades occasional repeat launches and extra controller state for fewer candidate survivors and less in-kernel threshold maintenance.

```diff
diff --git a/include/saev_amd.h b/include/saev_amd.h
--- a/include/saev_amd.h
+++ b/include/saev_amd.h
@@ -453,6 +453,7 @@
 int saev_copy_last(saev_ctx* ctx, int32_t n_rows, int32_t* idx_out, float* val_out, float* x_hat_out, void* stream);
 
 int saev_bound_state(saev_ctx* ctx, float* z, int64_t* launches, int64_t* repeats, float* mean_candidates, void* stream);
+int saev_bound_ratio(saev_ctx* ctx, float* rho_lo, int64_t* pause_left, void* stream);
 
 int saev_enable_kernel_timing(saev_ctx* ctx, int32_t enable);
 float saev_last_encoder_ms(saev_ctx* ctx);
diff --git a/saev_amd/_lib.py b/saev_amd/_lib.py
--- a/saev_amd/_lib.py
+++ b/saev_amd/_lib.py
@@ -259,6 +259,7 @@
     "saev_last_x_hat": (P, [P]),
     "saev_copy_last": (C.c_int, [P, C.c_int32, P, P, P, P]),
     "saev_bound_state": (C.c_int, [P, C.POINTER(C.c_float), C.POINTER(C.c_int64), C.POINTER(C.c_int64), C.POINTER(C.c_float), P]),
+    "saev_bound_ratio": (C.c_int, [P, C.POINTER(C.c_float), C.POINTER(C.c_int64), P]),
     "saev_enable_kernel_timing": (C.c_int, [P, C.c_int32]),
     "saev_last_encoder_ms": (C.c_float, [P]),
 }
diff --git a/saev_amd/csrc/ctx.h b/saev_amd/csrc/ctx.h
--- a/saev_amd/csrc/ctx.h
+++ b/saev_amd/csrc/ctx.h
@@ -140,6 +140,12 @@
     int rs_lat_range = 0, rs_n_ranges = 0;
     int32_t* tau_max = nullptr;
     float* heur_state = nullptr;
+    float *rho_state = nullptr, *rho_scratch = nullptr, *row_bound = nullptr, *kth_val = nullptr;
+    bool rho_valid = false;
+    int rho_n = 0;
+    int rho_step = 0;
+    int32_t rho_serial_seen = 0;
+    int rho_pause_left = 0;
     float *f16r_scales = nullptr, *mu = nullptr, *xnorm = nullptr, *b_shift = nullptr, *dot_part = nullptr, *xabs_part = nullptr,
           *sq_part = nullptr, *wmax_prev = nullptr;
     bool wmax_known = false;
diff --git a/saev_amd/csrc/ctx.hip b/saev_amd/csrc/ctx.hip
--- a/saev_amd/csrc/ctx.hip
+++ b/saev_amd/csrc/ctx.hip
@@ -168,11 +168,12 @@
         if (c->cfg.encoder_mode == SAEV_ENCODER_F16R) { A(dot_part, (size_t)2 * (c->Dp / 32) * c->S_pad); A(sq_part, (size_t)2 * (c->Dp / 32) * c->S_pad); A(wmax_prev, 1); }
         if (c->cfg.encoder_mode == SAEV_ENCODER_F16R) { A(surv_idx, MB * REFINE_CAP); A(surv_val, MB * REFINE_CAP); A(surv_cnt, MB); }
     }
-    c->stream_ok = c->fwd_slices && c->cfg.bound_mode == 0 && c->dbg.prep_route == 0 && D % 32 == 0 && c->Dp == (int)D;
+    c->stream_ok = c->fwd_slices && c->cfg.bound_mode != 1 && c->dbg.prep_route == 0 && D % 32 == 0 && c->Dp == (int)D;
     if (c->stream_ok) {
         A(WeS, S * D); A(xn_part, (size_t)(D / 32) * c->MB_pad * 2);
         A(amax_part, (size_t)(c->MB_pad / 256) * (D / 32)); A(cmax_part, (size_t)(c->MB_pad / 256) * (D / 32)); A(b_seen, S);
         A(mu_keep, D); A(xside_keep, 4);
+        if (c->cfg.bound_mode == 2) { A(rho_state, 16); A(rho_scratch, 32); A(row_bound, MB); A(kth_val, MB); }
     }
     if (c->stream_ok || c->cfg.encoder_mode == SAEV_ENCODER_BF16) A(wchk, (size_t)2 * ((S + 255) / 256) * ((D + 31) / 32));
     A(toks, S); A(fired, S); A(dead, S); A(flags, 16); A(upper, 1); A(stats, 1);
@@ -200,7 +201,7 @@
         if (hipHostMalloc(&hp, 64, hipHostMallocMapped) == hipSuccess &&
             hipHostGetDevicePointer(reinterpret_cast<void**>(&c->stale_dev), hp, 0) == hipSuccess) {
             c->stale_host = static_cast<int32_t*>(hp);
-            c->stale_host[0] = 0; c->stale_host[1] = 0;
+            for (int i = 0; i < 16; ++i) c->stale_host[i] = 0;
         } else {
             if (hp) hipHostFree(hp);
             c->stale_host = nullptr; c->stale_dev = nullptr;
@@ -213,6 +214,11 @@
     {
         const float init[8] = {2.6f, 0.f, 0.f, 0.f, 0.f, 0.f, 0.f, 0.f};
         hipMemcpy(c->heur_state, init, sizeof(init), hipMemcpyHostToDevice);
+    }
+    if (c->rho_state) {
+        const float init[16] = {0.9f, 0.f, 0.f, 0.f, 0.f, 0.f, __builtin_nanf(""), 0.f, 0.f, 0.f, 0.f, 0.f, 0.f, 0.f, 0.f, 0.f};
+        hipMemcpy(c->rho_state, init, sizeof(init), hipMemcpyHostToDevice);
+        hipMemset(c->rho_scratch, 0, 32 * sizeof(float));
     }
     hipMemset(c->rowstats, 0, MB * sizeof(RowStats));
     if (c->xs) hipMemset(c->xs, 0, (size_t)c->MB_pad * 2 * c->Dp * sizeof(_Float16));
@@ -452,12 +458,25 @@
     if (!c) return SAEV_INVALID_ARG;
     float h[4] = {0.f, 0.f, 0.f, 0.f};
     hipStream_t s = (hipStream_t)stream;
-    HIPCHK(c, hipMemcpyAsync(h, c->heur_state, sizeof(h), hipMemcpyDeviceToHost, s));
+    HIPCHK(c, hipMemcpyAsync(h, c->rho_state != nullptr ? c->rho_state : c->heur_state, sizeof(h), hipMemcpyDeviceToHost, s));
     HIPCHK(c, hipStreamSynchronize(s));
     if (z) *z = h[0];
     if (repeats) *repeats = (int64_t)h[1];
     if (launches) *launches = (int64_t)h[2];
     if (mean_candidates) *mean_candidates = h[3];
+    return SAEV_OK;
+}
+
+int saev_bound_ratio(saev_ctx* c, float* rho_lo, int64_t* pause_left, void* stream) {
+    if (!c) return SAEV_INVALID_ARG;
+    float h[8] = {0.f, 0.f, 0.f, 0.f, 0.f, 0.f, __builtin_nanf(""), 0.f};
+    hipStream_t s = (hipStream_t)stream;
+    if (c->rho_state != nullptr) {
+        HIPCHK(c, hipMemcpyAsync(h, c->rho_state, sizeof(h), hipMemcpyDeviceToHost, s));
+        HIPCHK(c, hipStreamSynchronize(s));
+    }
+    if (rho_lo) *rho_lo = h[6];
+    if (pause_left) *pause_left = (int64_t)h[5];
     return SAEV_OK;
 }
 
diff --git a/saev_amd/csrc/ctx_auxk.hip b/saev_amd/csrc/ctx_auxk.hip
--- a/saev_amd/csrc/ctx_auxk.hip
+++ b/saev_amd/csrc/ctx_auxk.hip
@@ -284,8 +284,13 @@
     if (c->stats_pending) {
         c->stats_pending = false;
         d.dead_list = c->cfg.k_aux > 0 ? c->dead_list : nullptr;
+        RhoArgs rho{};
+        if (c->rho_step != 0) {
+            rho.kth = c->kth_val; rho.xnorm = c->xnorm; rho.state = c->rho_state; rho.flags = c->flags; rho.scratch = c->rho_scratch;
+            rho.k = c->cfg.top_k; rho.host = c->stale_dev != nullptr ? c->stale_dev + 4 : nullptr;
+        }
         HIPCHK(c, launch_stats_dead(c->rowstats, c->n_last, c->cfg.d_model, c->P_last, c->cfg.alpha, c->upper_c, c->flags + 2, c->stats,
-                                    c->stats_scratch, c->stats_lists ? c->cand_cnt : nullptr, CAND_CAP, d, s));
+                                    c->stats_scratch, c->stats_lists ? c->cand_cnt : nullptr, CAND_CAP, d, s, c->rho_step != 0 ? &rho : nullptr));
         c->dead_list_ready = d.dead_list != nullptr;
     } else {
         HIPCHK(c, launch_dead_update(d, s));
diff --git a/saev_amd/csrc/ctx_forward.hip b/saev_amd/csrc/ctx_forward.hip
--- a/saev_amd/csrc/ctx_forward.hip
+++ b/saev_amd/csrc/ctx_forward.hip
@@ -92,7 +92,7 @@
 }
 
 static int run_encoder(saev_ctx* c, const float* x, int n, int epi, float* h_out, const int32_t* flag, int when,
-                       hipStream_t s, bool predicted = false, const float* x_scale = nullptr) {
+                       hipStream_t s, bool predicted = false, const float* x_scale = nullptr, bool norm_bounds = false) {
     const bool f16r = c->cfg.encoder_mode == SAEV_ENCODER_F16R;
     if (c->cfg.encoder_mode != SAEV_ENCODER_F32 && !(f16r && epi == EPI_DENSE)) {
         const bool bf = c->cfg.encoder_mode == SAEV_ENCODER_BF16;
@@ -110,6 +110,7 @@
         a.cand_cap = CAND_CAP; a.cand_stride = CAND_STRIDE;
         a.enable_flag = flag; a.enable_when = when;
         if (predicted) { a.heur_z = c->heur_state; a.tau_max = c->tau_max; }
+        if (norm_bounds) a.row_bound = c->row_bound;
         a.refresh_first = 8;
         a.refresh_every = a.ngroups > 32 ? 1 : 2;
         HIPCHK(c, launch_encode_f16x3(a, epi, s));
@@ -177,7 +178,7 @@
     const int K = c->cfg.top_k;
     int32_t* need_dense = c->flags + 1;
     const bool f16r_mode = c->cfg.encoder_mode == SAEV_ENCODER_F16R;
-    const bool predict_mode = fused_supported(c->cfg) && c->cfg.bound_mode != 0 && c->cfg.encoder_mode != SAEV_ENCODER_F32 &&
+    const bool predict_mode = fused_supported(c->cfg) && c->cfg.bound_mode == 1 && c->cfg.encoder_mode != SAEV_ENCODER_F32 &&
                               f16_ngroups(c) == 32;
     const bool one_launch_pre = fused_supported(c->cfg) && !predict_mode;
     if (c->follow_stream) {
@@ -219,12 +220,13 @@
                     HIPCHK(c, launch_refine_exact(sc, s));
                 }
                 sc.row_margin = nullptr; sc.tau_max = nullptr;
+                if (c->rho_step != 0) sc.kth_out = c->kth_val;
                 sc.cand_cnt = c->surv_cnt; sc.cand_val = c->surv_val; sc.cand_idx = c->surv_idx; sc.cand_cap = REFINE_CAP; sc.cand_stride = REFINE_CAP;
             }
             HIPCHK(c, launch_select_cand(sc, s));
             return SAEV_OK;
         };
-        const bool predict = c->cfg.bound_mode != 0 && ng == 32 && c->cfg.encoder_mode != SAEV_ENCODER_F32;
+        const bool predict = c->cfg.bound_mode == 1 && ng == 32 && c->cfg.encoder_mode != SAEV_ENCODER_F32;
         int32_t *bad1 = c->flags + 9, *run2 = c->flags + 10, *gate = c->flags + 11;
         if (predict) {
             HIPCHK(c, launch_heur_gate(c->heur_state, pre_flag, gate, s));
@@ -267,6 +269,8 @@
                 pe.amax_part = c->amax_part; pe.cmax_part = c->cmax_part; pe.n_img = ((n + 255) / 256) * (D_ / 32);
                 pe.upper = c->upper; pe.stats = c->stats; pe.stale = c->flags + 12; pe.stale_host = c->stale_dev;
                 pe.xside_keep = c->followers.empty() ? nullptr : c->xside_keep;
+                pe.rho_mode = c->rho_step; pe.rho_state = c->rho_state; pe.row_bound = c->row_bound; pe.tau_max = c->tau_max;
+                pe.rho_bad = bad1; pe.rho_gate = gate;
                 HIPCHK(c, launch_pre_encode2(pe, s));
                 if (c->train_fused) c->mu_serial++;
             } else
@@ -274,11 +278,27 @@
                                         c->wnorm_scratch, (S_ + 255) / 256, f16r_mode ? scl(c) : nullptr, const_cast<int32_t*>(pre_flag),
                                         c->wmax_prev, c->row_margin, c->flags + 1, s));
             timing_begin(c, s);
-            int rc = run_encoder(c, x, n, EPI_TOPK, nullptr, pre_flag, 0, s);
-            if (rc != SAEV_OK) return rc;
-            timing_end(c, s);
-            rc = select_stage(need_dense, 0, need_dense, nullptr, c->flags + 1, pre_flag);
-            if (rc != SAEV_OK) return rc;
+            if (c->stream_step && c->rho_step == 2) {
+                int32_t* const run_enc = c->flags + 14;
+                int rc = run_encoder(c, x, n, EPI_TOPK, nullptr, gate, 0, s, false, nullptr, true);
+                if (rc != SAEV_OK) return rc;
+                timing_end(c, s);
+                rc = select_stage(bad1, 0, bad1, c->tau_max, bad1, gate);
+                if (rc != SAEV_OK) return rc;
+                HIPCHK(c, launch_repeat_init(c->cand_cnt, n, c->gmax, ng * c->gmax_stride, bad1, pre_flag, run_enc, s));
+                rc = run_encoder(c, x, n, EPI_TOPK, nullptr, run_enc, 1, s);
+                if (rc != SAEV_OK) return rc;
+                HIPCHK(c, launch_overflow_check(c->cand_cnt, n, CAND_CAP, pre_flag, need_dense, c->flags + 2, c->flags + 3, s, need_dense,
+                                                run2, nullptr, bad1));
+                rc = select_stage(run2, 1, need_dense, nullptr, c->flags + 1, run2);
+                if (rc != SAEV_OK) return rc;
+            } else {
+                int rc = run_encoder(c, x, n, EPI_TOPK, nullptr, pre_flag, 0, s);
+                if (rc != SAEV_OK) return rc;
+                timing_end(c, s);
+                rc = select_stage(need_dense, 0, need_dense, nullptr, c->flags + 1, pre_flag);
+                if (rc != SAEV_OK) return rc;
+            }
         }
     } else {
         HIPCHK(c, launch_init_i32(need_dense, 1, 1, s));
@@ -310,6 +330,7 @@
     c->xprep_x = nullptr;
     c->stream_step = false;
     c->follow_stream = false;
+    c->rho_step = 0; c->rho_valid = false;
     return encode_topk_impl(c, x, n, idx_out, val_out, c->flags, s);
 }
 
@@ -527,6 +548,21 @@
     c->follow_stream = borrowed && c->borrow_streamed && c->stream_ok && c->wimg_fresh && c->wimg_mu_serial == c->leader->fwd_mu_serial &&
                        c->wenc_ready == nullptr && c->fwd_step && c->cfg.encoder_mode == SAEV_ENCODER_F16R;
     c->fwd_reused_wimg = c->stream_step || c->follow_stream;
+    {
+        const bool rho_mode = c->cfg.bound_mode == 2 && c->rho_state != nullptr && c->stream_step && !borrowed && !btk && training &&
+                              c->train_fused && c->P == 1 && c->followers.empty() && c->cfg.encoder_mode == SAEV_ENCODER_F16R &&
+                              fused_supported(c->cfg) && f16_ngroups(c) == 32;
+        if (rho_mode && c->stale_host != nullptr) {
+            const volatile int32_t* hw = c->stale_host + 4;
+            const int32_t serial = hw[0];
+            if (serial != c->rho_serial_seen) { c->rho_serial_seen = serial; c->rho_pause_left = hw[1]; }
+        }
+        const bool paused = rho_mode && c->rho_pause_left > 0;
+        if (paused) c->rho_pause_left--;
+        c->rho_step = rho_mode ? ((c->rho_valid && c->rho_n == n && !paused) ? 2 : 1) : 0;
+        c->rho_valid = rho_mode;
+        c->rho_n = n;
+    }
     if (c->gather_pool != nullptr && !c->stream_step)
         HIPCHK(c, launch_gather_rows(c->gather_pool, c->gather_rows, n, D, const_cast<float*>(x), s));
     if (c->stream_step) {
@@ -613,7 +649,7 @@
     }
     c->P_last = c->P;
     for (int p = 0; p < c->P; ++p) c->cuts_last[p] = c->cuts[p];
-    const bool lists = !btk && fused_supported(c->cfg) && !(c->cfg.bound_mode != 0 && c->cfg.encoder_mode != SAEV_ENCODER_F32 && f16_ngroups(c) == 32);
+    const bool lists = !btk && fused_supported(c->cfg) && !(c->cfg.bound_mode == 1 && c->cfg.encoder_mode != SAEV_ENCODER_F32 && f16_ngroups(c) == 32);
     c->stats_pending = false;
     if (c->train_fused && training) {
         c->stats_pending = true;
diff --git a/saev_amd/csrc/gemm_encode_f16x3.hip b/saev_amd/csrc/gemm_encode_f16x3.hip
--- a/saev_amd/csrc/gemm_encode_f16x3.hip
+++ b/saev_amd/csrc/gemm_encode_f16x3.hip
@@ -625,6 +625,14 @@
     if (st_begin < st_end) {
         stage_kstep(0, st_begin * HTS, kmap(0));
         if (nks > 1) stage_kstep(1, st_begin * HTS, kmap(1));
+    }
+    float tau_row[4] = {0.f, 0.f, 0.f, 0.f};
+    if constexpr (NG == 0) {
+#pragma unroll
+        for (int jb = 0; jb < 4; ++jb) {
+            const int b = b0 + wb * 64 + jb * 16 + l15;
+            tau_row[jb] = (b < B) ? fmaxf(a.row_bound[b], -3.0e38f) - a.row_margin[b] : 3.0e38f;
+        }
     }
 
     for (int st = st_begin; st < st_end; ++st) {
@@ -802,7 +810,7 @@
 #undef GPTR
                 __syncthreads();
             }
-        } else if (refresh) {
+        } else if (NG != 0 && refresh) {
 #pragma unroll
             for (int jb = 0; jb < 4; ++jb) {
                 const int bl_ = wb * 64 + jb * 16 + l15;
@@ -897,8 +905,13 @@
 #pragma unroll
         for (int jb = 0; jb < 4; ++jb) {
             const int b = b0 + wb * 64 + jb * 16 + l15;
-            float tau = fmaxf(key2f(sm.tau_key[wb * 64 + jb * 16 + l15]), -3.0e38f);
-            if (a.row_margin != nullptr) tau -= (b < B) ? a.row_margin[b] : 0.f;
+            float tau;
+            if constexpr (NG == 0) {
+                tau = tau_row[jb];
+            } else {
+                tau = fmaxf(key2f(sm.tau_key[wb * 64 + jb * 16 + l15]), -3.0e38f);
+                if (a.row_margin != nullptr) tau -= (b < B) ? a.row_margin[b] : 0.f;
+            }
             uint32_t m = 0;
 #pragma unroll
             for (int sb = 0; sb < 8; ++sb)
@@ -961,7 +974,8 @@
     const size_t smem = sizeof(HSmem);
     static bool attr_set = false;
     if (!attr_set) {
-        const void* fns[12] = {reinterpret_cast<const void*>(&encode_m16_kernel<1>),
+        const void* fns[13] = {reinterpret_cast<const void*>(&encode_m16_kernel<1>),
+                              reinterpret_cast<const void*>(&encode_m16_kernel<2, 0>),
                               reinterpret_cast<const void*>(&encode_m16_kernel<2>),
                               reinterpret_cast<const void*>(&encode_m16_kernel<1, 64>),
                               reinterpret_cast<const void*>(&encode_m16_kernel<2, 64>),
@@ -985,6 +999,9 @@
         if (a.arith == 1) LAUNCH_ENC(EPI_DENSE, 32, 1);
         else if (a.arith == 2) LAUNCH_ENC(EPI_DENSE, 32, 2);
         else LAUNCH_ENC(EPI_DENSE, 32, 0);
+    } else if (a.ngroups <= 32 && a.row_bound != nullptr) {
+        if (a.arith != 2 || a.row_margin == nullptr) return hipErrorInvalidValue;
+        LAUNCH_M16(2, 0);
     } else if (a.ngroups <= 32 && a.heur_z != nullptr) {
         if (a.arith == 1) LAUNCH_ENC(EPI_TOPK, 32, 1, true);
         else if (a.arith == 2) LAUNCH_ENC(EPI_TOPK, 32, 2, true);
diff --git a/saev_amd/csrc/kernels.h b/saev_amd/csrc/kernels.h
--- a/saev_amd/csrc/kernels.h
+++ b/saev_amd/csrc/kernels.h
@@ -46,6 +46,8 @@
     int walk_grid;
 };
 hipError_t launch_select_dense(const SelectDenseArgs& a, hipStream_t stream);
+hipError_t launch_repeat_init(int32_t* cand_cnt, int n_rows, int32_t* gmax, int n_gmax, const int32_t* bad, const int32_t* pre_flag,
+                              int32_t* run_enc, hipStream_t stream);
 
 struct SelectCandArgs {
     const int32_t* cand_cnt;
@@ -75,6 +77,7 @@
     const float* sum_bias;
     int sum_n;
     size_t sum_plane;
+    float* kth_out;
 };
 hipError_t launch_refine_exact(const SelectCandArgs& a, hipStream_t stream);
 constexpr int REFINE_CAP = 512;
@@ -324,9 +327,18 @@
     int32_t* dead_list;
 };
 hipError_t launch_dead_update(const DeadArgs& a, hipStream_t stream);
+struct RhoArgs {
+    const float* kth;
+    const float* xnorm;
+    float* state;
+    const int32_t* flags;
+    float* scratch;
+    int k;
+    int32_t* host;
+};
 hipError_t launch_stats_dead(const RowStats* rs, int n_rows, int D, int P, float alpha, const float* upper, const int32_t* n_overflow,
                              saev_step_stats* stats, double* scratch, const int32_t* cand_cnt, int cand_cap, const DeadArgs& d,
-                             hipStream_t stream);
+                             hipStream_t stream, const RhoArgs* rho = nullptr);
 hipError_t launch_absmax(const float* x, long n, float* out_zeroed, hipStream_t stream);
 hipError_t launch_gather_rows(const float* pool, const int64_t* rows, int n_rows, int D, float* out, hipStream_t stream);
 hipError_t launch_scatter_dense(const int32_t* idx, const float* val, int n_rows, int k, int stride, int S, float* f,
@@ -361,6 +373,7 @@
     int enable_when;
     const float* heur_z;
     int32_t* tau_max;
+    const float* row_bound;
     int refresh_first, refresh_every;
     int n_batches;
     int blk_imgs;
@@ -415,6 +428,7 @@
     int32_t* stale; int32_t* stale_host;
     float* xside_keep;
     saev_step_stats* stats;
+    int rho_mode; const float* rho_state; float* row_bound; int32_t* tau_max; int32_t* rho_bad; int32_t* rho_gate;
     int nb_rows;
 };
 hipError_t launch_pre_encode2(PreEncode2Args a, hipStream_t stream);
diff --git a/saev_amd/csrc/select.hip b/saev_amd/csrc/select.hip
--- a/saev_amd/csrc/select.hip
+++ b/saev_amd/csrc/select.hip
@@ -240,6 +240,7 @@
         }
         return;
     }
+    if (a.kth_out != nullptr && lane == 0) a.kth_out[row] = n >= a.k ? ukey2f(T) : __builtin_nanf("");
     int cgt = 0, ceq = 0;
 #pragma unroll
     for (int e = 0; e < EPL; ++e) { cgt += __popcll(__ballot(key[e] > T)); ceq += __popcll(__ballot(key[e] == T)); }
@@ -339,6 +340,7 @@
     }
     const uint32_t T = stream_kth_largest(cv, ci, n, k, lane);
     if (a.tau_max != nullptr && lane == 0 && (n < a.k || ukey2f(T) < key2f(a.tau_max[row]))) *a.invalid = 1;
+    if (a.kth_out != nullptr && lane == 0) a.kth_out[row] = n >= a.k ? ukey2f(T) : __builtin_nanf("");
     const int cgt = stream_count(cv, ci, n, 0u, 1, T, 0, lane), ceq = stream_count(cv, ci, n, 0u, 2, T, 0, lane);
     const int need = k - cgt;
     int32_t idx_cut = 0x7fffffff;
@@ -392,6 +394,10 @@
     if (a.tau_max != nullptr) {
         const float kth = ukey2f(__shfl(key, max(k - 1, 0), 64));
         if (lane == 0 && (n < a.k || kth < key2f(a.tau_max[row]))) *a.invalid = 1;
+    }
+    if (a.kth_out != nullptr) {
+        const float kth = ukey2f(__shfl(key, max(k - 1, 0), 64));
+        if (lane == 0) a.kth_out[row] = n >= a.k ? kth : __builtin_nanf("");
     }
     const bool win = lane < k;
     sort_by_idx_and_store(a, row, k, win ? idx : 0x7fffffff, win ? ukey2f(key) : 0.f, lane);
@@ -451,6 +457,17 @@
     if (i < n_gmax) gmax[i] = INT32_MIN;
     if (tau_max != nullptr && i < n_rows) tau_max[i] = INT32_MIN;
 }
+__global__ __launch_bounds__(256) void repeat_init_kernel(int32_t* cand_cnt, int n_rows, int32_t* gmax, int n_gmax, const int32_t* bad,
+                                                          const int32_t* pre_flag, int32_t* run_enc) {
+    const bool armed = *bad != 0;
+    if (blockIdx.x == 0 && threadIdx.x == 0) *run_enc = (armed && *pre_flag == 0) ? 1 : 0;
+    if (!armed) return;
+    const int n = max(n_rows, n_gmax);
+    for (int i = blockIdx.x * 256 + threadIdx.x; i < n; i += gridDim.x * 256) {
+        if (i < n_rows) cand_cnt[i] = 0;
+        if (i < n_gmax) gmax[i] = INT32_MIN;
+    }
+}
 __global__ void step_zero_kernel(saev_step_stats* stats, float* upper, int32_t* flag0) {
     if (threadIdx.x == 0) {
         *stats = saev_step_stats{};
@@ -735,6 +752,10 @@
     if (i >= n_rows) return;
     margin[i] = f16r_margin(xnorm[2 * i], xnorm[2 * i + 1], wmax, dwmax, bmax, D, scales[0]);
 }
+__device__ __forceinline__ bool rho_gate_closed(const float* st) {
+    const float c = st[0], rho = st[6];
+    return st[5] > 0.f || !(rho - rho == 0.f) || !(c > 0.f);
+}
 __global__ __launch_bounds__(256) void pre_encode2_kernel(PreEncode2Args a) {
     __shared__ float sh[5][4];
     const int i = blockIdx.x * 256 + threadIdx.x;
@@ -787,6 +808,11 @@
         *a.pre_flag = pre;
         *a.wmax_prev = wmax;
         a.flags1[0] = pre; a.flags1[1] = 0; a.flags1[2] = 0;
+        if (a.rho_mode != 0) {
+            const int g = a.rho_mode != 2 ? 2 : ((pre != 0 || rho_gate_closed(a.rho_state)) ? 1 : 0);
+            *a.rho_gate = g;
+            *a.rho_bad = g != 0 ? 1 : 0;
+        }
         *a.upper = amax;
         *a.stats = saev_step_stats{};
         const float xs_next = (cmax > 0.f && cmax < 3.0e38f) ? exp2f(13.0f - floorf(log2f(cmax))) : x_scale;
@@ -813,6 +839,11 @@
     const float xn = back * sqrtf(s2) * 1.000001f, xd = back * sqrtf(d2) * 1.000002f;
     if (a.xnorm != nullptr) { a.xnorm[2 * i] = xn; a.xnorm[2 * i + 1] = xd; }
     a.margin[i] = f16r_margin(xn, xd, wmax, dwmax, bmax, a.D, x_scale);
+    if (a.rho_mode == 2 && !rho_gate_closed(a.rho_state)) {
+        const float bound = a.rho_state[0] * a.rho_state[6] * xn;
+        a.row_bound[i] = bound;
+        a.tau_max[i] = f2key(bound);
+    }
 }
 __global__ void follower_scales_kernel(const float* xside, const float* wmax, float* scales, int32_t* pre_flag, int keep_w) {
     if (threadIdx.x != 0) return;
@@ -928,6 +959,13 @@
     return hipGetLastError();
 }
 
+hipError_t launch_repeat_init(int32_t* cand_cnt, int n_rows, int32_t* gmax, int n_gmax, const int32_t* bad, const int32_t* pre_flag,
+                              int32_t* run_enc, hipStream_t stream) {
+    const int n = std::max(n_rows, n_gmax);
+    hipLaunchKernelGGL(repeat_init_kernel, dim3(std::max(1, std::min((n + 255) / 256, 256))), dim3(256), 0, stream, cand_cnt, n_rows, gmax,
+                       n_gmax, bad, pre_flag, run_enc);
+    return hipGetLastError();
+}
 hipError_t launch_encoder_init(int32_t* cand_cnt, int n_rows, int32_t* gmax, int n_gmax, hipStream_t stream, int32_t* tau_max,
                                const int32_t* enable_flag, int enable_when) {
     const int n = n_rows > n_gmax ? n_rows : n_gmax;
diff --git a/saev_amd/csrc/tail.hip b/saev_amd/csrc/tail.hip
--- a/saev_amd/csrc/tail.hip
+++ b/saev_amd/csrc/tail.hip
@@ -568,7 +568,46 @@
     const RowStats* rs; int n_rows, D, P; float alpha; int with_aux; const float* upper; const int32_t* n_overflow;
     saev_step_stats* stats; const int32_t* n_dead_dev; double* scratch; const int32_t* cand_cnt; int cand_cap;
 };
-__device__ __forceinline__ void stats_reduce_body(const StatsArgs& A, int bid, int n_blocks) {
+__device__ __forceinline__ void rho_controller(const RhoArgs& R, float rho_min, float cand_mean) {
+    float* st = R.state;
+    const int gate = R.flags[11], bad = R.flags[9], dense = R.flags[1];
+    float c = st[0];
+    if (gate == 0) {
+        st[2] += 1.f;
+        if (bad != 0) {
+            c -= 0.05f;
+            st[1] += 1.f;
+        } else if (cand_mean > 3.f * (float)R.k) {
+            c += 0.0005f;
+        }
+        if (bad != 0 || cand_mean > fmaxf(12.f * (float)R.k, 256.f)) {
+            st[4] += 1.f;
+            st[8] = 0.f;
+            if (st[4] >= 3.f) {
+                st[4] = 0.f;
+                st[5] = 256.f * exp2f(2.f * st[7]);
+                st[7] = fminf(st[7] + 1.f, 4.f);
+                st[9] += 1.f;
+                if (R.host != nullptr) {
+                    R.host[1] = (int32_t)st[5];
+                    __threadfence_system();
+                    R.host[0] = (int32_t)st[9];
+                }
+                if (bad != 0) c = 0.85f;
+            }
+        } else {
+            st[4] = 0.f;
+            st[8] += 1.f;
+            if (st[8] >= 256.f) st[7] = 0.f;
+        }
+        st[0] = fminf(fmaxf(c, 0.5f), 0.95f);
+    } else if (st[5] > 0.f) {
+        st[5] -= 1.f;
+    }
+    st[3] = cand_mean;
+    st[6] = (dense == 0 && rho_min < 3.0e38f) ? rho_min : __builtin_nanf("");
+}
+__device__ __forceinline__ void stats_reduce_body(const StatsArgs& A, int bid, int n_blocks, const RhoArgs& R = RhoArgs{}) {
     const RowStats* rs = A.rs; const int n_rows = A.n_rows, D = A.D, P = A.P; const float alpha = A.alpha; const int with_aux = A.with_aux;
     const float* upper = A.upper; const int32_t* n_overflow = A.n_overflow; saev_step_stats* stats = A.stats;
     const int32_t* n_dead_dev = A.n_dead_dev; double* scratch = A.scratch; const int32_t* cand_cnt = A.cand_cnt; const int cand_cap = A.cand_cap;
@@ -579,7 +618,12 @@
     double s[NS] = {0, 0, 0, 0, 0, 0, 0, 0};
     const int per = (n_rows + n_blocks - 1) / n_blocks;
     const int r0 = bid * per, r1 = min(n_rows, r0 + per);
+    float rho_min = 3.4e38f;
     for (int r = r0 + threadIdx.x; r < r1; r += 1024) {
+        if (R.kth != nullptr) {
+            const float q = R.kth[r] / R.xnorm[2 * r];
+            if (q - q == 0.f) rho_min = fminf(rho_min, q);
+        }
         const RowStats v = rs[r];
         s[0] += v.sse_scaled; s[1] += v.l0; s[2] += v.l1; s[3] += with_aux ? v.aux_sse : 0.f;
         s[4] += v.sse64; s[5] += v.sumsq64;
@@ -593,10 +637,25 @@
     for (int i = 0; i < 7; ++i) s[i] = wave_sum_d(s[i]);
 #pragma unroll
     for (int o = 32; o > 0; o >>= 1) s[7] = fmax(s[7], __shfl_xor(s[7], o, 64));
+    __shared__ float sh_rho[16], sh_cnt[16];
+    if (R.kth != nullptr) {
+        float csum = 0.f;
+        if (cand_cnt != nullptr)
+            for (int r = r0 + threadIdx.x; r < r1; r += 1024) csum += (float)min(cand_cnt[r], cand_cap);
+#pragma unroll
+        for (int o = 32; o > 0; o >>= 1) { rho_min = fminf(rho_min, __shfl_xor(rho_min, o, 64)); csum += __shfl_xor(csum, o, 64); }
+        if ((threadIdx.x & 63) == 0) { sh_rho[threadIdx.x >> 6] = rho_min; sh_cnt[threadIdx.x >> 6] = csum; }
+    }
     if ((threadIdx.x & 63) == 0)
         for (int i = 0; i < NS; ++i) sh[threadIdx.x >> 6][i] = s[i];
     __syncthreads();
     int* ticket = reinterpret_cast<int*>(scratch + 16 * NS);
+    if (R.kth != nullptr && threadIdx.x == 64) {
+        float m = 3.4e38f, t = 0.f;
+        for (int w = 0; w < 16; ++w) { m = fminf(m, sh_rho[w]); t += sh_cnt[w]; }
+        __hip_atomic_store(&R.scratch[bid], m, __ATOMIC_RELAXED, __HIP_MEMORY_SCOPE_AGENT);
+        __hip_atomic_store(&R.scratch[16 + bid], t, __ATOMIC_RELAXED, __HIP_MEMORY_SCOPE_AGENT);
+    }
     if (threadIdx.x < NS) {
         const int i = threadIdx.x;
         double t = 0.0;
@@ -617,8 +676,18 @@
         const int b = threadIdx.x / NS, i = threadIdx.x % NS;
         part[b][i] = b < n_blocks ? __hip_atomic_load(&scratch[b * NS + i], __ATOMIC_RELAXED, __HIP_MEMORY_SCOPE_AGENT) : 0.0;
     }
+    __shared__ float rho_part[32];
+    if (R.kth != nullptr && threadIdx.x >= 128 && threadIdx.x < 160) {
+        const int j = threadIdx.x - 128;
+        rho_part[j] = (j & 15) < n_blocks ? __hip_atomic_load(&R.scratch[j], __ATOMIC_RELAXED, __HIP_MEMORY_SCOPE_AGENT) : (j < 16 ? 3.4e38f : 0.f);
+    }
     __syncthreads();
     if (threadIdx.x != 0) return;
+    if (R.kth != nullptr) {
+        float m = 3.4e38f, t = 0.f;
+        for (int b = 0; b < 16; ++b) { m = fminf(m, rho_part[b]); t += rho_part[16 + b]; }
+        rho_controller(R, m, t / (float)max(n_rows, 1));
+    }
     {
         double t[NS] = {0, 0, 0, 0, 0, 0, 0, 0};
         for (int b = 0; b < n_blocks; ++b) {
@@ -658,8 +727,8 @@
 }
 
 __global__ __launch_bounds__(1024) void stats_reduce_kernel(StatsArgs A) { stats_reduce_body(A, blockIdx.x, gridDim.x); }
-__global__ __launch_bounds__(1024) void stats_dead_kernel(StatsArgs A, int n_stat, DeadArgs d) {
-    if ((int)blockIdx.x < n_stat) stats_reduce_body(A, blockIdx.x, n_stat);
+__global__ __launch_bounds__(1024) void stats_dead_kernel(StatsArgs A, int n_stat, DeadArgs d, RhoArgs R) {
+    if ((int)blockIdx.x < n_stat) stats_reduce_body(A, blockIdx.x, n_stat, R);
     else dead_update_body(d, (int)blockIdx.x - n_stat, (int)gridDim.x - n_stat);
 }
 
@@ -757,9 +826,9 @@
 }
 hipError_t launch_stats_dead(const RowStats* rs, int n_rows, int D, int P, float alpha, const float* upper, const int32_t* n_overflow,
                              saev_step_stats* stats, double* scratch, const int32_t* cand_cnt, int cand_cap, const DeadArgs& d,
-                             hipStream_t stream) {
+                             hipStream_t stream, const RhoArgs* rho) {
     const int nb = std::max(1, std::min(16, (n_rows + 1023) / 1024));
     const StatsArgs A{rs, n_rows, D, P, alpha, 0, upper, n_overflow, stats, nullptr, scratch, cand_cnt, cand_cap};
-    hipLaunchKernelGGL(stats_dead_kernel, dim3(nb + (d.S + 1023) / 1024), dim3(1024), 0, stream, A, nb, d);
-    return hipGetLastError();
-}
+    hipLaunchKernelGGL(stats_dead_kernel, dim3(nb + (d.S + 1023) / 1024), dim3(1024), 0, stream, A, nb, d, rho != nullptr ? *rho : RhoArgs{});
+    return hipGetLastError();
+}
diff --git a/saev_amd/engine.py b/saev_amd/engine.py
--- a/saev_amd/engine.py
+++ b/saev_amd/engine.py
@@ -28,7 +28,7 @@
     aux_dead_cap: int = 0
     shard_world: int = 1
     max_backward_rows: int = 0
-    bounds: str = dataclasses.field(default_factory=lambda: os.environ.get("SAEV_AMD_BOUNDS", "guaranteed"))
+    bounds: str = dataclasses.field(default_factory=lambda: os.environ.get("SAEV_AMD_BOUNDS", "norm"))
     encoder: str = dataclasses.field(default_factory=lambda: os.environ.get("SAEV_AMD_ENCODER", DEFAULT_ENCODER))
     dw_route: str = dataclasses.field(default_factory=lambda: os.environ.get("SAEV_AMD_DW", "slices"))
     fwd_route: str = dataclasses.field(default_factory=lambda: os.environ.get("SAEV_AMD_FWD", "default"))
@@ -1453,8 +1453,8 @@
         self.chunk_a, self.chunk_b = lay.chunk_a, lay.chunk_b
         self.offsets = {"W_dec": lay.off_W_dec, "b_dec": lay.off_b_dec, "W_enc": lay.off_W_enc, "b_enc": lay.off_b_enc}
         self.shapes = {"W_dec": (S, D), "b_dec": (D,), "W_enc": (D, S), "b_enc": (S,)}
-        if cfg.bounds not in ("guaranteed", "predicted"):
-            raise ValueError(f"EngineConfig.bounds (SAEV_AMD_BOUNDS) must be 'guaranteed' or 'predicted', got {cfg.bounds!r}")
+        if cfg.bounds not in ("guaranteed", "predicted", "norm"):
+            raise ValueError(f"EngineConfig.bounds (SAEV_AMD_BOUNDS) must be 'guaranteed', 'predicted' or 'norm', got {cfg.bounds!r}")
         if cfg.encoder not in ("f32", "f16x3", "bf16", "f16r"):
             raise ValueError(f"EngineConfig.encoder (SAEV_AMD_ENCODER) must be one of f32, f16x3, bf16, f16r, got {cfg.encoder!r}")
         if cfg.activation not in ("topk", "relu", "batch_topk", "relu_train"):
@@ -1503,7 +1503,7 @@
             normalize_w_dec=int(cfg.normalize_w_dec), remove_parallel_grads=int(cfg.remove_parallel_grads),
             max_batch=cfg.max_batch, encoder_mode={"f32": 0, "f16x3": 1, "bf16": 2, "f16r": 3}[cfg.encoder],
             aux_dead_cap=cfg.aux_dead_cap, shard_world=cfg.shard_world,
-            bound_mode={"guaranteed": 0, "predicted": 1}[cfg.bounds], max_backward_rows=cfg.max_backward_rows,
+            bound_mode={"guaranteed": 0, "predicted": 1, "norm": 2}[cfg.bounds], max_backward_rows=cfg.max_backward_rows,
             activation={"topk": _lib.ACT_TOPK, "relu": _lib.ACT_RELU, "batch_topk": _lib.ACT_BATCHTOPK, "relu_train": _lib.ACT_RELU}[cfg.activation],
         )
         dbg = _lib.SaevDebugCfg(
@@ -2111,7 +2111,12 @@
         z, mc = C.c_float(), C.c_float()
         n, r = C.c_int64(), C.c_int64()
         self._chk(self.lib.saev_bound_state(self.ctx, C.byref(z), C.byref(n), C.byref(r), C.byref(mc), _stream()), "saev_bound_state")
-        return {"z": z.value, "launches": n.value, "repeats": r.value, "mean_candidates": mc.value}
+        out = {"z": z.value, "launches": n.value, "repeats": r.value, "mean_candidates": mc.value}
+        if self.cfg.bounds == "norm":
+            rho, left = C.c_float(), C.c_int64()
+            self._chk(self.lib.saev_bound_ratio(self.ctx, C.byref(rho), C.byref(left), _stream()), "saev_bound_ratio")
+            out.update(rho_lo=rho.value, pause_left=left.value)
+        return out
 
     def enable_kernel_timing(self, on: bool = True):
         self._chk(self.lib.saev_enable_kernel_timing(self.ctx, int(on)), "saev_enable_kernel_timing")
```

New measurement: 6.660 million, median of 6. 5.6% higher.
